# Cuberick-Orion/Candidate-Reranking-CIR

Hardware: AMD Instinct MI355X
Metric: query-candidate triplets scored/sec at K=100 (higher is better)
Workload: dtype f16; 1 GPU; CIRR-val-style K=100 re-rank from pixels (BASELINE configs[2]): ViT-B/16 224px (197 tokens), 32-token captions, 64 queries x (100 candidates + 5 subset members) per step per GPU, skip rate 0, random-init weights; k=100, subset=5, image_size=224, residual_stream=f16

## Files before the change

candidate_reranking_cir_amd/csrc/common.hpp:

```cpp
#pragma once
#include <hip/hip_runtime.h>
#include <stdint.h>

#include "cirrank.h"

namespace cir {

typedef __attribute__((ext_vector_type(8))) __bf16 bf16x8;
typedef __attribute__((ext_vector_type(4))) __bf16 bf16x4;
typedef __attribute__((ext_vector_type(8))) _Float16 f16x8;
typedef __attribute__((ext_vector_type(4))) _Float16 f16x4;
typedef __attribute__((ext_vector_type(4))) float f32x4;
typedef __attribute__((ext_vector_type(16))) float f32x16;
typedef __attribute__((ext_vector_type(4))) short s16x4;
typedef __attribute__((ext_vector_type(8))) short s16x8;
typedef __attribute__((ext_vector_type(4))) unsigned int u32x4;
typedef __attribute__((ext_vector_type(2))) unsigned int u32x2;

constexpr int kWave = 64;

template <typename T> struct Elem;
template <> struct Elem<__bf16> {
    using x8 = bf16x8;
    using x4 = bf16x4;
    static __device__ __forceinline__ f32x4 mfma16(x8 a, x8 b, f32x4 c) {
        return __builtin_amdgcn_mfma_f32_16x16x32_bf16(a, b, c, 0, 0, 0);
    }
    static __device__ __forceinline__ f32x16 mfma32(x8 a, x8 b, f32x16 c) {
        return __builtin_amdgcn_mfma_f32_32x32x16_bf16(a, b, c, 0, 0, 0);
    }
    static __device__ __forceinline__ void mfma16_acc(f32x4& c, x8 a, x8 b) {
        asm("v_mfma_f32_16x16x32_bf16 %0, %1, %2, %0" : "+v"(c) : "v"(a), "v"(b));
    }
};
template <> struct Elem<_Float16> {
    using x8 = f16x8;
    using x4 = f16x4;
    static __device__ __forceinline__ f32x4 mfma16(x8 a, x8 b, f32x4 c) {
        return __builtin_amdgcn_mfma_f32_16x16x32_f16(a, b, c, 0, 0, 0);
    }
    static __device__ __forceinline__ f32x16 mfma32(x8 a, x8 b, f32x16 c) {
        return __builtin_amdgcn_mfma_f32_32x32x16_f16(a, b, c, 0, 0, 0);
    }
    static __device__ __forceinline__ void mfma16_acc(f32x4& c, x8 a, x8 b) {
        asm("v_mfma_f32_16x16x32_f16 %0, %1, %2, %0" : "+v"(c) : "v"(a), "v"(b));
    }
};

template <typename T> __device__ __forceinline__ T from_f32(float x) { return static_cast<T>(x); }
template <typename T> __device__ __forceinline__ float to_f32(T x) { return static_cast<float>(x); }

template <typename T> __device__ __forceinline__ unsigned int pack2(float a, float b) {
    typedef __attribute__((ext_vector_type(2))) T t2;
    t2 v = {static_cast<T>(a), static_cast<T>(b)};
    return __builtin_bit_cast(unsigned int, v);
}

__device__ __forceinline__ float wave_sum(float v) {
#pragma unroll
    for (int o = 32; o > 0; o >>= 1) v += __shfl_xor(v, o, 64);
    return v;
}
__device__ __forceinline__ float wave_max(float v) {
#pragma unroll
    for (int o = 32; o > 0; o >>= 1) v = fmaxf(v, __shfl_xor(v, o, 64));
    return v;
}

__device__ __forceinline__ float fast_erf(float x) {
    const float ax = fabsf(x);
    const float t = __frcp_rn(fmaf(0.3275911f, ax, 1.0f));
    float p = fmaf(1.061405429f, t, -1.453152027f);
    p = fmaf(p, t, 1.421413741f);
    p = fmaf(p, t, -0.284496736f);
    p = fmaf(p, t, 0.254829592f);
    p *= t;
    const float e = 1.0f - p * __expf(-ax * ax);
    return copysignf(e, x);
}
__device__ __forceinline__ float gelu_erf_as(float x) { return 0.5f * x * (1.0f + fast_erf(x * 0.70710678118654752f)); }

__device__ __forceinline__ float gelu_erf(float x) {
    const float xc = __builtin_amdgcn_fmed3f(x, -5.5f, 5.5f);
    const float x2 = xc * xc;
    float p = fmaf(x2, -2.48362952e-05f, -7.36062896e-04f);
    p = fmaf(x2, p, 1.05982735e-01f);
    p = fmaf(x2, p, 2.30164715e+00f);
    const float e = __builtin_amdgcn_exp2f(-(xc * p));
    return x * __builtin_amdgcn_rcpf(1.0f + e);
}

typedef __attribute__((ext_vector_type(2))) float f32x2;
__device__ __forceinline__ f32x2 gelu_erf2(f32x2 x) {
    f32x2 xc;
    xc.x = __builtin_amdgcn_fmed3f(x.x, -5.5f, 5.5f);
    xc.y = __builtin_amdgcn_fmed3f(x.y, -5.5f, 5.5f);
    const f32x2 x2 = xc * xc;
    const f32x2 c3 = {-2.48362952e-05f, -2.48362952e-05f}, c2 = {-7.36062896e-04f, -7.36062896e-04f};
    const f32x2 c1 = {1.05982735e-01f, 1.05982735e-01f}, c0 = {2.30164715e+00f, 2.30164715e+00f};
    f32x2 p = __builtin_elementwise_fma(x2, c3, c2);
    p = __builtin_elementwise_fma(x2, p, c1);
    p = __builtin_elementwise_fma(x2, p, c0);
    const f32x2 q = xc * p;
    f32x2 e;
    e.x = __builtin_amdgcn_exp2f(-q.x);
    e.y = __builtin_amdgcn_exp2f(-q.y);
    const f32x2 d = e + 1.0f;
    f32x2 r;
    r.x = __builtin_amdgcn_rcpf(d.x);
    r.y = __builtin_amdgcn_rcpf(d.y);
    return x * r;
}

__device__ __forceinline__ void gelu_erf8(float (&v)[8]) {
    f32x2 x[4], xc[4], t[4], p[4];
#pragma unroll
    for (int j = 0; j < 4; ++j) x[j] = f32x2{v[2 * j], v[2 * j + 1]};
#pragma unroll
    for (int j = 0; j < 4; ++j) { xc[j].x = __builtin_amdgcn_fmed3f(x[j].x, -5.5f, 5.5f); xc[j].y = __builtin_amdgcn_fmed3f(x[j].y, -5.5f, 5.5f); }
    __builtin_amdgcn_sched_barrier(0);
#pragma unroll
    for (int j = 0; j < 4; ++j) t[j] = xc[j] * xc[j];
    __builtin_amdgcn_sched_barrier(0);
    const f32x2 c3 = {-2.48362952e-05f, -2.48362952e-05f}, c2 = {-7.36062896e-04f, -7.36062896e-04f};
    const f32x2 c1 = {1.05982735e-01f, 1.05982735e-01f}, c0 = {2.30164715e+00f, 2.30164715e+00f};
#pragma unroll
    for (int j = 0; j < 4; ++j) p[j] = __builtin_elementwise_fma(t[j], c3, c2);
    __builtin_amdgcn_sched_barrier(0);
#pragma unroll
    for (int j = 0; j < 4; ++j) p[j] = __builtin_elementwise_fma(t[j], p[j], c1);
    __builtin_amdgcn_sched_barrier(0);
#pragma unroll
    for (int j = 0; j < 4; ++j) p[j] = __builtin_elementwise_fma(t[j], p[j], c0);
    __builtin_amdgcn_sched_barrier(0);
#pragma unroll
    for (int j = 0; j < 4; ++j) t[j] = xc[j] * p[j];
    __builtin_amdgcn_sched_barrier(0);
#pragma unroll
    for (int j = 0; j < 4; ++j) { t[j].x = __builtin_amdgcn_exp2f(-t[j].x); t[j].y = __builtin_amdgcn_exp2f(-t[j].y); }
    __builtin_amdgcn_sched_barrier(0);
#pragma unroll
    for (int j = 0; j < 4; ++j) t[j] = t[j] + 1.0f;
    __builtin_amdgcn_sched_barrier(0);
#pragma unroll
    for (int j = 0; j < 4; ++j) { t[j].x = __builtin_amdgcn_rcpf(t[j].x); t[j].y = __builtin_amdgcn_rcpf(t[j].y); }
    __builtin_amdgcn_sched_barrier(0);
#pragma unroll
    for (int j = 0; j < 4; ++j) { const f32x2 y = x[j] * t[j]; v[2 * j] = y.x; v[2 * j + 1] = y.y; }
}

__device__ __forceinline__ void gelu_erf_as8(float (&v)[8]) {
    f32x2 x[4], t[4], p[4], q[4];
#pragma unroll
    for (int j = 0; j < 4; ++j) x[j] = f32x2{v[2 * j], v[2 * j + 1]};
#pragma unroll
    for (int j = 0; j < 4; ++j) { t[j].x = fmaf(fabsf(x[j].x), 0.3275911f * 0.70710678118654752f, 1.0f); t[j].y = fmaf(fabsf(x[j].y), 0.3275911f * 0.70710678118654752f, 1.0f); }
    __builtin_amdgcn_sched_barrier(0);
#pragma unroll
    for (int j = 0; j < 4; ++j) { t[j].x = __builtin_amdgcn_rcpf(t[j].x); t[j].y = __builtin_amdgcn_rcpf(t[j].y); }
#pragma unroll
    for (int j = 0; j < 4; ++j) q[j] = x[j] * x[j];
    __builtin_amdgcn_sched_barrier(0);
    const f32x2 a5 = {1.061405429f, 1.061405429f}, a4 = {-1.453152027f, -1.453152027f}, a3 = {1.421413741f, 1.421413741f};
    const f32x2 a2 = {-0.284496736f, -0.284496736f}, a1 = {0.254829592f, 0.254829592f};
#pragma unroll
    for (int j = 0; j < 4; ++j) p[j] = __builtin_elementwise_fma(a5, t[j], a4);
#pragma unroll
    for (int j = 0; j < 4; ++j) q[j] = q[j] * f32x2{-0.72134752044448170f, -0.72134752044448170f};
    __builtin_amdgcn_sched_barrier(0);
#pragma unroll
    for (int j = 0; j < 4; ++j) p[j] = __builtin_elementwise_fma(p[j], t[j], a3);
#pragma unroll
    for (int j = 0; j < 4; ++j) { q[j].x = __builtin_amdgcn_exp2f(q[j].x); q[j].y = __builtin_amdgcn_exp2f(q[j].y); }
    __builtin_amdgcn_sched_barrier(0);
#pragma unroll
    for (int j = 0; j < 4; ++j) p[j] = __builtin_elementwise_fma(p[j], t[j], a2);
    __builtin_amdgcn_sched_barrier(0);
#pragma unroll
    for (int j = 0; j < 4; ++j) p[j] = __builtin_elementwise_fma(p[j], t[j], a1);
    __builtin_amdgcn_sched_barrier(0);
#pragma unroll
    for (int j = 0; j < 4; ++j) t[j] = t[j] * q[j];
    __builtin_amdgcn_sched_barrier(0);
#pragma unroll
    for (int j = 0; j < 4; ++j) p[j] = __builtin_elementwise_fma(-p[j], t[j], f32x2{1.0f, 1.0f});
    __builtin_amdgcn_sched_barrier(0);
#pragma unroll
    for (int j = 0; j < 4; ++j) { p[j].x = fmaf(fabsf(x[j].x), p[j].x, x[j].x); p[j].y = fmaf(fabsf(x[j].y), p[j].y, x[j].y); }
    __builtin_amdgcn_sched_barrier(0);
#pragma unroll
    for (int j = 0; j < 4; ++j) { const f32x2 y = p[j] * f32x2{0.5f, 0.5f}; v[2 * j] = y.x; v[2 * j + 1] = y.y; }
}

constexpr float kSplitLoScale = 4096.0f;
constexpr int kSplitLoExp = 12;
__device__ __forceinline__ float clamp_e4m3(float x) { return __builtin_amdgcn_fmed3f(x, -448.0f, 448.0f); }
struct Split4 { unsigned h01, h23, lo8, hi8; };
__device__ __forceinline__ Split4 split8_x4(const float (&y)[4]) {
    float hf[4], lf[4];
    _Float16 hh[4];
#pragma unroll
    for (int j = 0; j < 4; ++j) {
        float v = y[j];
        asm volatile("" : "+v"(v));
        hh[j] = (_Float16)v;
        float f = (float)hh[j];
        asm volatile("" : "+v"(f));
        hf[j] = clamp_e4m3(f);
        lf[j] = clamp_e4m3((v - f) * kSplitLoScale);
    }
    typedef __attribute__((ext_vector_type(2))) _Float16 h2;
    Split4 r;
    r.h01 = __builtin_bit_cast(unsigned, h2{hh[0], hh[1]});
    r.h23 = __builtin_bit_cast(unsigned, h2{hh[2], hh[3]});
    unsigned l = 0, h = 0;
    l = __builtin_amdgcn_cvt_pk_fp8_f32(lf[0], lf[1], l, false);
    l = __builtin_amdgcn_cvt_pk_fp8_f32(lf[2], lf[3], l, true);
    h = __builtin_amdgcn_cvt_pk_fp8_f32(hf[0], hf[1], h, false);
    h = __builtin_amdgcn_cvt_pk_fp8_f32(hf[2], hf[3], h, true);
    r.lo8 = l;
    r.hi8 = h;
    return r;
}
typedef __attribute__((ext_vector_type(8))) int i32x8;
__device__ __forceinline__ void mfma_f8_acc(f32x4& c, i32x8 a, i32x8 b, int sa, int sb) {
    asm("v_mfma_scale_f32_16x16x128_f8f6f4 %0, %1, %2, %0, %3, %4 op_sel_hi:[0,0,0]" : "+v"(c) : "v"(a), "v"(b), "v"(sa), "v"(sb));
}

__device__ __forceinline__ uint32_t hash32(uint32_t x) {
    x ^= x >> 16; x *= 0x7feb352du; x ^= x >> 15; x *= 0x846ca68bu; x ^= x >> 16;
    return x;
}
constexpr uint32_t kDropWeyl = 0x9E3779B9u;
__device__ __forceinline__ uint32_t drop_threshold(float p) { return (uint32_t)(p * 65536.0f + 0.5f); }
__device__ __forceinline__ uint32_t drop_row_key(uint64_t seed, uint64_t row) {
    return (uint32_t)seed + (uint32_t)(seed >> 32) * 0x85EBCA6Bu + (uint32_t)row * kDropWeyl + (uint32_t)(row >> 32) * 0xC2B2AE35u;
}
__device__ __forceinline__ uint32_t drop_bits(uint32_t row_key, uint32_t col) { return hash32(row_key ^ (col >> 1)); }
__device__ __forceinline__ bool drop_kept(uint32_t bits, uint32_t col, uint32_t thr) { return ((col & 1u) ? (bits >> 16) : (bits & 0xffffu)) >= thr; }

__device__ __forceinline__ int xcd_remap(int bid, int nblk) {
    const int q = nblk >> 3, r = nblk & 7, x = bid & 7;
    const int base = (x < r) ? x * (q + 1) : r * (q + 1) + (x - r) * q;
    return base + (bid >> 3);
}

}

namespace cir {
extern int g_tune[3];

constexpr int kOrdRows = 256;
constexpr int kEmbChunk = 512;
struct OrderedDst { float* out[4]; int src[4]; int nout; };
int colsum_ordered_launch(const float* x, int64_t ld, int64_t rows, int seg, const OrderedDst& d, hipStream_t s);
}
#define CIR_CHECK_PTR(p) do { if ((p) == nullptr) return CIR_EINVAL; } while (0)
#define CIR_LAUNCH_RESULT() do { hipError_t e_ = hipGetLastError(); return e_ == hipSuccess ? CIR_OK : (int)e_; } while (0)
static inline bool cir_aligned16(const void* p) { return (reinterpret_cast<uintptr_t>(p) & 15u) == 0; }
```

candidate_reranking_cir_amd/csrc/misc.hip:

```cpp
#include "common.hpp"

namespace cir {

template <typename TI, typename TO>
__global__ __launch_bounds__(256) void patchify_kernel(const TI* img, TO* out, int B, int C, int H, int Wd, int p, int vec) {
    const int gw = Wd / p, gh = H / p;
    const int64_t total = (int64_t)B * gh * gw * C * p;
    const int64_t gid = (int64_t)blockIdx.x * blockDim.x + threadIdx.x;
    if (gid >= total) return;
    int64_t t = gid;
    const int px = (int)(t % gw); t /= gw;
    const int ky = (int)(t % p); t /= p;
    const int py = (int)(t % gh); t /= gh;
    const int c = (int)(t % C);
    const int64_t b = t / C;
    const TI* src = img + ((b * C + c) * H + (py * p + ky)) * (int64_t)Wd + px * p;
    TO* dst = out + ((b * gh + py) * gw + px) * (int64_t)(C * p * p) + (c * p + ky) * p;
    if (vec) {
        if constexpr (sizeof(TO) == 4) {
            const float4* s4 = reinterpret_cast<const float4*>(src);
            float4* d4 = reinterpret_cast<float4*>(dst);
            const float4 a0 = s4[0], a1 = s4[1], a2 = s4[2], a3 = s4[3];
            d4[0] = a0; d4[1] = a1; d4[2] = a2; d4[3] = a3;
        } else if constexpr (sizeof(TI) == 2) {
            const u32x4* s4 = reinterpret_cast<const u32x4*>(src);
            u32x4* d4 = reinterpret_cast<u32x4*>(dst);
            const u32x4 v0 = s4[0], v1 = s4[1];
            d4[0] = v0;
            d4[1] = v1;
        } else {
            const float4* s4 = reinterpret_cast<const float4*>(src);
            const float4 a0 = s4[0], a1 = s4[1], a2 = s4[2], a3 = s4[3];
            u32x4 o0, o1;
            o0.x = pack2<TO>(a0.x, a0.y); o0.y = pack2<TO>(a0.z, a0.w); o0.z = pack2<TO>(a1.x, a1.y); o0.w = pack2<TO>(a1.z, a1.w);
            o1.x = pack2<TO>(a2.x, a2.y); o1.y = pack2<TO>(a2.z, a2.w); o1.z = pack2<TO>(a3.x, a3.y); o1.w = pack2<TO>(a3.z, a3.w);
            u32x4* d4 = reinterpret_cast<u32x4*>(dst);
            d4[0] = o0;
            d4[1] = o1;
        }
        return;
    }
    for (int kx = 0; kx < p; ++kx) dst[kx] = static_cast<TO>(static_cast<float>(src[kx]));
}

template <typename S>
__global__ __launch_bounds__(256) void vit_assemble_kernel(const S* proj, const float* cls, const float* pos, S* x,
                                                           int B, int P, int D) {
    const int d4 = D / 4;
    const int64_t total = (int64_t)B * (P + 1) * d4;
    const int64_t gid = (int64_t)blockIdx.x * blockDim.x + threadIdx.x;
    if (gid >= total) return;
    const int c = (int)(gid % d4);
    const int64_t row = gid / d4;
    const int tok = (int)(row % (P + 1));
    const int64_t b = row / (P + 1);
    const float4 pe = reinterpret_cast<const float4*>(pos + (int64_t)tok * D)[c];
    float4 v;
    if (tok == 0) {
        v = reinterpret_cast<const float4*>(cls)[c];
    } else if constexpr (__is_same(S, float)) {
        v = reinterpret_cast<const float4*>(proj + (b * P + tok - 1) * D)[c];
    } else {
        const f16x4 h = reinterpret_cast<const f16x4*>(proj + (b * P + tok - 1) * D)[c];
        v = make_float4((float)h[0], (float)h[1], (float)h[2], (float)h[3]);
    }
    const float4 o = make_float4(v.x + pe.x, v.y + pe.y, v.z + pe.z, v.w + pe.w);
    if constexpr (__is_same(S, float)) {
        reinterpret_cast<float4*>(x + row * D)[c] = o;
    } else {
        u32x2 pk;
        pk.x = pack2<_Float16>(o.x, o.y);
        pk.y = pack2<_Float16>(o.z, o.w);
        reinterpret_cast<u32x2*>(x + row * D)[c] = pk;
    }
}

template <typename T>
__global__ __launch_bounds__(256) void small_linear_kernel(const T* x, int64_t ldx, const T* W, const float* bias, float* y,
                                                           int64_t M, int N, int K) {
    using X8 = typename Elem<T>::x8;
    const int lane = threadIdx.x & 63;
    const int64_t row = (int64_t)blockIdx.x * 4 + (threadIdx.x >> 6);
    if (row >= M) return;
    float acc[8];
#pragma unroll
    for (int n = 0; n < 8; ++n) acc[n] = 0.f;
    for (int k = lane * 8; k < K; k += 512) {
        const X8 xv = *reinterpret_cast<const X8*>(x + row * ldx + k);
#pragma unroll
        for (int n = 0; n < 8; ++n) {
            if (n < N) {
                const X8 wv = *reinterpret_cast<const X8*>(W + (int64_t)n * K + k);
#pragma unroll
                for (int j = 0; j < 8; ++j) acc[n] = fmaf(static_cast<float>(xv[j]), static_cast<float>(wv[j]), acc[n]);
            }
        }
    }
#pragma unroll
    for (int n = 0; n < 8; ++n) {
        if (n < N) {
            const float s = wave_sum(acc[n]);
            if (lane == 0) y[row * N + n] = s + (bias ? bias[n] : 0.f);
        }
    }
}


template <typename TI, typename TO>
__global__ __launch_bounds__(256) void gather_rows_kernel(const TI* src, const int64_t* index, TO* dst, int64_t n_rows,
                                                          int64_t row_elems, int64_t src_rows) {
    const int64_t vec_per_row = row_elems / 8;
    const int64_t gid = (int64_t)blockIdx.x * blockDim.x + threadIdx.x;
    if (gid >= n_rows * vec_per_row) return;
    const int64_t row = gid / vec_per_row, c = (gid - row * vec_per_row) * 8;
    int64_t sr = index ? index[row] : row;
    sr = sr < 0 ? 0 : (sr >= src_rows ? src_rows - 1 : sr);
    const TI* s = src + sr * row_elems + c;
    TO* d = dst + row * row_elems + c;
    float v[8];
    if constexpr (sizeof(TI) == 4) {
        const float4 a = reinterpret_cast<const float4*>(s)[0], b = reinterpret_cast<const float4*>(s)[1];
        v[0] = a.x; v[1] = a.y; v[2] = a.z; v[3] = a.w; v[4] = b.x; v[5] = b.y; v[6] = b.z; v[7] = b.w;
    } else {
        typedef __attribute__((ext_vector_type(8))) TI ti8;
        const ti8 a = *reinterpret_cast<const ti8*>(s);
#pragma unroll
        for (int j = 0; j < 8; ++j) v[j] = static_cast<float>(a[j]);
    }
    if constexpr (sizeof(TO) == 4) {
        reinterpret_cast<float4*>(d)[0] = make_float4(v[0], v[1], v[2], v[3]);
        reinterpret_cast<float4*>(d)[1] = make_float4(v[4], v[5], v[6], v[7]);
    } else {
        u32x4 o;
        o.x = pack2<TO>(v[0], v[1]); o.y = pack2<TO>(v[2], v[3]); o.z = pack2<TO>(v[4], v[5]); o.w = pack2<TO>(v[6], v[7]);
        *reinterpret_cast<u32x4*>(d) = o;
    }
}


__global__ __launch_bounds__(256) void linear_f32_kernel(const float* x, int64_t ldx, const float* W, const float* bias, float* y,
                                                        int64_t M, int N, int K, int mode) {
    __shared__ float As[16][65], Ws[16][65];
    const int tid = threadIdx.x, tx = tid & 15, ty = tid >> 4;
    const int64_t row0 = (int64_t)blockIdx.y * 64;
    const int col0 = blockIdx.x * 64;
    float acc[4][4];
#pragma unroll
    for (int i = 0; i < 4; ++i)
#pragma unroll
        for (int j = 0; j < 4; ++j) acc[i][j] = 0.f;
    for (int k0 = 0; k0 < K; k0 += 16) {
#pragma unroll
        for (int i = 0; i < 4; ++i) {
            const int e = tid + i * 256, r = e >> 4, kk = e & 15;
            As[kk][r] = (row0 + r < M && k0 + kk < K) ? x[(row0 + r) * ldx + k0 + kk] : 0.f;
            Ws[kk][r] = (col0 + r < N && k0 + kk < K) ? W[(int64_t)(col0 + r) * K + k0 + kk] : 0.f;
        }
        __syncthreads();
#pragma unroll
        for (int kk = 0; kk < 16; ++kk) {
            float av[4], wv[4];
#pragma unroll
            for (int i = 0; i < 4; ++i) { av[i] = As[kk][ty * 4 + i]; wv[i] = Ws[kk][tx * 4 + i]; }
#pragma unroll
            for (int i = 0; i < 4; ++i)
#pragma unroll
                for (int j = 0; j < 4; ++j) acc[i][j] = fmaf(av[i], wv[j], acc[i][j]);
        }
        __syncthreads();
    }
#pragma unroll
    for (int i = 0; i < 4; ++i) {
        const int64_t m = row0 + ty * 4 + i;
        if (m >= M) continue;
#pragma unroll
        for (int j = 0; j < 4; ++j) {
            const int n = col0 + tx * 4 + j;
            if (n >= N) continue;
            const float v = acc[i][j] + (bias ? bias[n] : 0.f);
            y[m * N + n] = mode == 1 ? 1.0f - v : (mode == 2 ? v - 1.0f : v);
        }
    }
}

__global__ __launch_bounds__(256) void l2_normalize_kernel(const float* x, float* y, int64_t rows, int cols) {
    const int lane = threadIdx.x & 63;
    const int64_t row = (int64_t)blockIdx.x * 4 + (threadIdx.x >> 6);
    if (row >= rows) return;
    float s = 0.f;
    for (int c = lane; c < cols; c += 64) { const float v = x[row * cols + c]; s = fmaf(v, v, s); }
    const float inv = 1.0f / fmaxf(sqrtf(wave_sum(s)), 1e-12f);
    for (int c = lane; c < cols; c += 64) y[row * cols + c] = x[row * cols + c] * inv;
}

__global__ __launch_bounds__(256) void topk_desc_kernel(const float* logits, int64_t* idx, int K, int n_pow2) {
    extern __shared__ __attribute__((aligned(16))) char dyn[];
    float* val = reinterpret_cast<float*>(dyn);
    int* ind = reinterpret_cast<int*>(dyn + (size_t)n_pow2 * 4);
    const float* row = logits + (int64_t)blockIdx.x * K;
    for (int i = threadIdx.x; i < n_pow2; i += blockDim.x) {
        float v = i < K ? row[i] : -INFINITY;
        if (v != v) v = -INFINITY;
        val[i] = v;
        ind[i] = i < K ? i : 0x7fffffff;
    }
    __syncthreads();
    for (int size = 2; size <= n_pow2; size <<= 1) {
        for (int stride = size >> 1; stride > 0; stride >>= 1) {
            for (int t = threadIdx.x; t < n_pow2 / 2; t += blockDim.x) {
                const int lo = 2 * t - (t & (stride - 1));
                const int hi = lo + stride;
                const bool asc_block = ((lo & size) != 0);
                const float va = val[lo], vb = val[hi];
                const int ia = ind[lo], ib = ind[hi];
                const bool a_first = (va > vb) || (va == vb && ia < ib);
                const bool swap = asc_block ? a_first : !a_first;
                if (swap) { val[lo] = vb; val[hi] = va; ind[lo] = ib; ind[hi] = ia; }
            }
            __syncthreads();
        }
    }
    for (int i = threadIdx.x; i < K; i += blockDim.x) idx[(int64_t)blockIdx.x * K + i] = ind[i];
}

}

extern "C" int cir_version(void) { return CIR_ABI_VERSION; }

namespace cir { int g_tune[3] = {0, 0, 0}; }

extern "C" int cir_set_tuning(int knob, int value) {
    switch (knob) {
        case CIR_TUNE_GEMM_TILE: if (value != 0 && value != 128 && value != 256) return CIR_EINVAL; break;
        case CIR_TUNE_GEMM_GROUP_W: if (value < 0 || value > 64) return CIR_EINVAL; break;
        case CIR_TUNE_ATTN_SHARED_MAX: if (value != 0 && value != -1 && value != -2 && (value < 32 || value > 608)) return CIR_EINVAL; break;
        default: return CIR_EINVAL;
    }
    cir::g_tune[knob] = value;
    return CIR_OK;
}

extern "C" const char* cir_strerror(int code) {
    switch (code) {
        case CIR_OK: return "ok";
        case CIR_EINVAL: return "invalid argument (null pointer or non-positive extent)";
        case CIR_ESHAPE: return "extent not supported by the gfx950 kernels";
        case CIR_EALIGN: return "pointer or stride not aligned for 16-byte vector access";
        case CIR_EDTYPE: return "dtype code not supported by this entry point";
        default: return code > 0 ? hipGetErrorString((hipError_t)code) : "unknown cirrank error";
    }
}

extern "C" int cir_patchify(const void* image, int img_dtype, void* patches, int dtype16, int B, int C, int H, int Wd,
                            int patch, void* stream) {
    using namespace cir;
    CIR_CHECK_PTR(image); CIR_CHECK_PTR(patches);
    if (B <= 0 || C <= 0 || H <= 0 || Wd <= 0 || patch <= 0) return CIR_EINVAL;
    if (H % patch || Wd % patch) return CIR_ESHAPE;
    if (dtype16 != CIR_BF16 && dtype16 != CIR_F16 && dtype16 != CIR_F32) return CIR_EDTYPE;
    if (img_dtype != CIR_F32 && img_dtype != dtype16) return CIR_EDTYPE;
    const int64_t total = (int64_t)B * C * H * (Wd / patch);
    dim3 grid((unsigned)((total + 255) / 256)), block(256);
    hipStream_t s = reinterpret_cast<hipStream_t>(stream);
    const int vec = patch == 16 && Wd % 16 == 0 && cir_aligned16(image) && cir_aligned16(patches);
    if (dtype16 == CIR_F32) {
        hipLaunchKernelGGL((patchify_kernel<float, float>), grid, block, 0, s, (const float*)image, (float*)patches, B, C, H, Wd, patch, vec);
        CIR_LAUNCH_RESULT();
    }
    if (dtype16 == CIR_BF16) {
        if (img_dtype == CIR_F32) hipLaunchKernelGGL((patchify_kernel<float, __bf16>), grid, block, 0, s, (const float*)image, (__bf16*)patches, B, C, H, Wd, patch, vec);
        else hipLaunchKernelGGL((patchify_kernel<__bf16, __bf16>), grid, block, 0, s, (const __bf16*)image, (__bf16*)patches, B, C, H, Wd, patch, vec);
    } else {
        if (img_dtype == CIR_F32) hipLaunchKernelGGL((patchify_kernel<float, _Float16>), grid, block, 0, s, (const float*)image, (_Float16*)patches, B, C, H, Wd, patch, vec);
        else hipLaunchKernelGGL((patchify_kernel<_Float16, _Float16>), grid, block, 0, s, (const _Float16*)image, (_Float16*)patches, B, C, H, Wd, patch, vec);
    }
    CIR_LAUNCH_RESULT();
}

extern "C" int cir_vit_assemble(const void* proj, const float* cls, const float* pos, void* x, int stream_dtype, int B, int P, int D,
                                void* stream) {
    CIR_CHECK_PTR(proj); CIR_CHECK_PTR(cls); CIR_CHECK_PTR(pos); CIR_CHECK_PTR(x);
    if (B <= 0 || P <= 0 || D <= 0) return CIR_EINVAL;
    if (D % 8) return CIR_ESHAPE;
    if (stream_dtype != CIR_F32 && stream_dtype != CIR_F16) return CIR_EDTYPE;
    if (!cir_aligned16(proj) || !cir_aligned16(cls) || !cir_aligned16(pos) || !cir_aligned16(x)) return CIR_EALIGN;
    const int64_t total = (int64_t)B * (P + 1) * (D / 4);
    dim3 grid((unsigned)((total + 255) / 256)), block(256);
    hipStream_t s = reinterpret_cast<hipStream_t>(stream);
    if (stream_dtype == CIR_F32)
        hipLaunchKernelGGL(cir::vit_assemble_kernel<float>, grid, block, 0, s, reinterpret_cast<const float*>(proj), cls, pos, reinterpret_cast<float*>(x), B, P, D);
    else
        hipLaunchKernelGGL(cir::vit_assemble_kernel<_Float16>, grid, block, 0, s, reinterpret_cast<const _Float16*>(proj), cls, pos, reinterpret_cast<_Float16*>(x), B, P, D);
    CIR_LAUNCH_RESULT();
}

extern "C" int cir_small_linear(const void* x, int64_t ldx, const void* W, const float* bias, float* y, int64_t M, int N,
                                int K, int dtype, void* stream) {
    using namespace cir;
    CIR_CHECK_PTR(x); CIR_CHECK_PTR(W); CIR_CHECK_PTR(y);
    if (M <= 0 || N <= 0 || K <= 0) return CIR_EINVAL;
    if (N > 8 || K % 8) return CIR_ESHAPE;
    if (dtype != CIR_BF16 && dtype != CIR_F16) return CIR_EDTYPE;
    if (!cir_aligned16(x) || !cir_aligned16(W) || ldx % 8) return CIR_EALIGN;
    if ((M + 3) / 4 > 0x7fffffffLL) return CIR_ESHAPE;
    dim3 grid((unsigned)((M + 3) / 4)), block(256);
    hipStream_t s = reinterpret_cast<hipStream_t>(stream);
    if (dtype == CIR_BF16) hipLaunchKernelGGL((small_linear_kernel<__bf16>), grid, block, 0, s, (const __bf16*)x, ldx, (const __bf16*)W, bias, y, M, N, K);
    else hipLaunchKernelGGL((small_linear_kernel<_Float16>), grid, block, 0, s, (const _Float16*)x, ldx, (const _Float16*)W, bias, y, M, N, K);
    CIR_LAUNCH_RESULT();
}

extern "C" int cir_topk_desc(const float* logits, int64_t* idx, int Q, int K, void* stream) {
    CIR_CHECK_PTR(logits); CIR_CHECK_PTR(idx);
    if (Q <= 0 || K <= 0) return CIR_EINVAL;
    if (K > 8192) return CIR_ESHAPE;
    int n = 2;
    while (n < K) n <<= 1;
    dim3 grid((unsigned)Q), block(256);
    hipLaunchKernelGGL(cir::topk_desc_kernel, grid, block, (size_t)n * 8, reinterpret_cast<hipStream_t>(stream), logits, idx, K, n);
    CIR_LAUNCH_RESULT();
}

namespace cir {
template <typename TI, typename TO>
static void launch_gather(const void* src, const int64_t* index, void* dst, int64_t n_rows, int64_t row_elems, int64_t src_rows, hipStream_t s) {
    const int64_t total = n_rows * (row_elems / 8);
    dim3 grid((unsigned)((total + 255) / 256)), block(256);
    hipLaunchKernelGGL((gather_rows_kernel<TI, TO>), grid, block, 0, s, (const TI*)src, index, (TO*)dst, n_rows, row_elems, src_rows);
}
}

extern "C" int cir_gather_rows(const void* src, int src_dtype, const int64_t* index, void* dst, int dst_dtype, int64_t n_rows,
                               int64_t row_elems, int64_t src_rows, void* stream) {
    using namespace cir;
    CIR_CHECK_PTR(src); CIR_CHECK_PTR(dst);
    if (n_rows <= 0 || row_elems <= 0 || src_rows <= 0) return CIR_EINVAL;
    if (row_elems % 8) return CIR_ESHAPE;
    if (!cir_aligned16(src) || !cir_aligned16(dst)) return CIR_EALIGN;
    if (n_rows * (row_elems / 8) > 0x7fffffffLL * 256) return CIR_ESHAPE;
    hipStream_t s = reinterpret_cast<hipStream_t>(stream);
#define CIR_G(SD, DD, TI, TO) if (src_dtype == SD && dst_dtype == DD) { launch_gather<TI, TO>(src, index, dst, n_rows, row_elems, src_rows, s); CIR_LAUNCH_RESULT(); }
    CIR_G(CIR_F32, CIR_F32, float, float)
    CIR_G(CIR_F32, CIR_BF16, float, __bf16)
    CIR_G(CIR_F32, CIR_F16, float, _Float16)
    CIR_G(CIR_BF16, CIR_BF16, __bf16, __bf16)
    CIR_G(CIR_F16, CIR_F16, _Float16, _Float16)
    CIR_G(CIR_BF16, CIR_F32, __bf16, float)
    CIR_G(CIR_F16, CIR_F32, _Float16, float)
    CIR_G(CIR_BF16, CIR_F16, __bf16, _Float16)
    CIR_G(CIR_F16, CIR_BF16, _Float16, __bf16)
#undef CIR_G
    return CIR_EDTYPE;
}

namespace cir {
template <int ACT>
__global__ __launch_bounds__(256) void split16_kernel(const float* __restrict__ x, int64_t ldx, _Float16* __restrict__ hi, _Float16* __restrict__ lo,
                                                      _Float16* __restrict__ hi2, int64_t ldo, int64_t rows, int cols) {
    const int64_t per_row = cols >> 3;
    const int64_t i = (int64_t)blockIdx.x * 256 + threadIdx.x;
    if (i >= rows * per_row) return;
    const int64_t r = i / per_row;
    const int c = (int)(i - r * per_row) * 8;
    const float4 v0 = *reinterpret_cast<const float4*>(x + r * ldx + c), v1 = *reinterpret_cast<const float4*>(x + r * ldx + c + 4);
    float v[8] = {v0.x, v0.y, v0.z, v0.w, v1.x, v1.y, v1.z, v1.w};
    f16x8 h, l;
#pragma unroll
    for (int j = 0; j < 8; ++j) {
        float y = v[j];
        if (ACT == CIR_ACT_GELU) y = 0.5f * y * (1.0f + erff(y * 0.70710678118654752f));
        else if (ACT == CIR_ACT_RELU) y = fmaxf(y, 0.f);
        asm volatile("" : "+v"(y));
        const _Float16 hj = (_Float16)y;
        float hf = (float)hj;
        asm volatile("" : "+v"(hf));
        h[j] = hj;
        l[j] = (_Float16)(y - hf);
    }
    *reinterpret_cast<f16x8*>(hi + r * ldo + c) = h;
    *reinterpret_cast<f16x8*>(lo + r * ldo + c) = l;
    if (hi2 != nullptr) *reinterpret_cast<f16x8*>(hi2 + r * ldo + c) = h;
}
template <int ACT>
__global__ __launch_bounds__(256) void split8_kernel(const float* __restrict__ x, int64_t ldx, char* __restrict__ out, int64_t ldo, int64_t rows, int cols) {
    const int64_t per_row = cols >> 3;
    const int64_t i = (int64_t)blockIdx.x * 256 + threadIdx.x;
    if (i >= rows * per_row) return;
    const int64_t r = i / per_row;
    const int c = (int)(i - r * per_row) * 8;
    const float4 v0 = *reinterpret_cast<const float4*>(x + r * ldx + c), v1 = *reinterpret_cast<const float4*>(x + r * ldx + c + 4);
    float v[8] = {v0.x, v0.y, v0.z, v0.w, v1.x, v1.y, v1.z, v1.w};
    if (ACT == CIR_ACT_GELU) gelu_erf_as8(v);
    else if (ACT == CIR_ACT_RELU) {
#pragma unroll
        for (int j = 0; j < 8; ++j) v[j] = fmaxf(v[j], 0.f);
    }
    const float a[4] = {v[0], v[1], v[2], v[3]}, b[4] = {v[4], v[5], v[6], v[7]};
    const Split4 sa = split8_x4(a), sb = split8_x4(b);
    const u32x4 h = {sa.h01, sa.h23, sb.h01, sb.h23};
    const u32x2 l8 = {sa.lo8, sb.lo8}, h8 = {sa.hi8, sb.hi8};
    char* row = out + r * ldo;
    *reinterpret_cast<u32x4*>(row + 2 * c) = h;
    *reinterpret_cast<u32x2*>(row + 2 * cols + c) = l8;
    *reinterpret_cast<u32x2*>(row + 3 * cols + c) = h8;
}
}


extern "C" int cir_split16(const float* x, int64_t ldx, void* hi, void* lo, void* hi2, int64_t ldo, int64_t rows, int cols, int act, void* stream) {
    using namespace cir;
    CIR_CHECK_PTR(x); CIR_CHECK_PTR(hi); CIR_CHECK_PTR(lo);
    if (rows <= 0 || cols <= 0) return CIR_EINVAL;
    if (cols % 8 || ldx % 4 || ldo % 8 || ldo < cols) return CIR_ESHAPE;
    if (act < CIR_ACT_NONE || act > CIR_ACT_RELU) return CIR_EINVAL;
    if (!cir_aligned16(x) || !cir_aligned16(hi) || !cir_aligned16(lo) || (hi2 && !cir_aligned16(hi2))) return CIR_EALIGN;
    const int64_t n = rows * (cols / 8);
    if (n > 0x7fffffffLL * 256) return CIR_ESHAPE;
    dim3 grid((unsigned)((n + 255) / 256)), block(256);
    hipStream_t s = reinterpret_cast<hipStream_t>(stream);
    _Float16* h = reinterpret_cast<_Float16*>(hi);
    _Float16* l = reinterpret_cast<_Float16*>(lo);
    _Float16* h2 = reinterpret_cast<_Float16*>(hi2);
    if (act == CIR_ACT_GELU) hipLaunchKernelGGL((split16_kernel<CIR_ACT_GELU>), grid, block, 0, s, x, ldx, h, l, h2, ldo, rows, cols);
    else if (act == CIR_ACT_RELU) hipLaunchKernelGGL((split16_kernel<CIR_ACT_RELU>), grid, block, 0, s, x, ldx, h, l, h2, ldo, rows, cols);
    else hipLaunchKernelGGL((split16_kernel<CIR_ACT_NONE>), grid, block, 0, s, x, ldx, h, l, h2, ldo, rows, cols);
    CIR_LAUNCH_RESULT();
}

extern "C" int cir_split8(const float* x, int64_t ldx, void* out, int64_t ldo_bytes, int64_t rows, int cols, int act, void* stream) {
    using namespace cir;
    CIR_CHECK_PTR(x); CIR_CHECK_PTR(out);
    if (rows <= 0 || cols <= 0) return CIR_EINVAL;
    if (cols % 8 || ldx % 4 || ldo_bytes % 16 || ldo_bytes < 4 * (int64_t)cols) return CIR_ESHAPE;
    if (act < CIR_ACT_NONE || act > CIR_ACT_RELU) return CIR_EINVAL;
    if (!cir_aligned16(x) || !cir_aligned16(out) || cols % 16) return CIR_EALIGN;
    const int64_t n = rows * (cols / 8);
    if (n > 0x7fffffffLL * 256) return CIR_ESHAPE;
    dim3 grid((unsigned)((n + 255) / 256)), block(256);
    hipStream_t s = reinterpret_cast<hipStream_t>(stream);
    char* o = reinterpret_cast<char*>(out);
    if (act == CIR_ACT_GELU) hipLaunchKernelGGL((split8_kernel<CIR_ACT_GELU>), grid, block, 0, s, x, ldx, o, ldo_bytes, rows, cols);
    else if (act == CIR_ACT_RELU) hipLaunchKernelGGL((split8_kernel<CIR_ACT_RELU>), grid, block, 0, s, x, ldx, o, ldo_bytes, rows, cols);
    else hipLaunchKernelGGL((split8_kernel<CIR_ACT_NONE>), grid, block, 0, s, x, ldx, o, ldo_bytes, rows, cols);
    CIR_LAUNCH_RESULT();
}

extern "C" int cir_linear_f32(const float* x, int64_t ldx, const float* W, const float* bias, float* y, int64_t M, int N, int K,
                              int mode, void* stream) {
    CIR_CHECK_PTR(x); CIR_CHECK_PTR(W); CIR_CHECK_PTR(y);
    if (M <= 0 || N <= 0 || K <= 0) return CIR_EINVAL;
    if (mode < 0 || mode > 2) return CIR_EINVAL;
    dim3 grid((unsigned)((N + 63) / 64), (unsigned)((M + 63) / 64)), block(256);
    if (grid.y > 65535u) return CIR_ESHAPE;
    hipLaunchKernelGGL(cir::linear_f32_kernel, grid, block, 0, reinterpret_cast<hipStream_t>(stream), x, ldx, W, bias, y, M, N, K, mode);
    CIR_LAUNCH_RESULT();
}

extern "C" int cir_l2_normalize(const float* x, float* y, int64_t rows, int cols, void* stream) {
    CIR_CHECK_PTR(x); CIR_CHECK_PTR(y);
    if (rows <= 0 || cols <= 0) return CIR_EINVAL;
    if ((rows + 3) / 4 > 0x7fffffffLL) return CIR_ESHAPE;
    dim3 grid((unsigned)((rows + 3) / 4)), block(256);
    hipLaunchKernelGGL(cir::l2_normalize_kernel, grid, block, 0, reinterpret_cast<hipStream_t>(stream), x, y, rows, cols);
    CIR_LAUNCH_RESULT();
}
```

candidate_reranking_cir_amd/csrc/xattn_fold.hip:

```cpp

#include "xattn_fold.hpp"

#ifndef FOLD_DBG
#define FOLD_DBG 0
#endif

namespace cir {

#if FOLD_DBG & 8
__device__ unsigned long long g_fold_stamps[8 * 64];
#define FOLD_STAMP(K)                                                                                          \
    do { if (blockIdx.x < 4 && (wave & 3) == 0 && lane == 0 && (K) < 64) {                                      \
             unsigned long long t_; __builtin_amdgcn_sched_barrier(0);                                         \
             asm volatile("s_memtime %0\n\ts_waitcnt lgkmcnt(0)" : "=s"(t_) :: "memory");                       \
             __builtin_amdgcn_sched_barrier(0);                                                                 \
             g_fold_stamps[(blockIdx.x * 2 + (wave >> 2)) * 64 + (K)] = t_; } } while (0)
#else
#define FOLD_STAMP(K) do {} while (0)
#endif

template <typename T, bool MASKED = false>
__global__ __launch_bounds__(512, 2) void xattn_fold_kernel(const FoldArgs a) {
    using X8 = typename Elem<T>::x8;
    extern __shared__ __attribute__((aligned(16))) char smem[];

    const int tid = threadIdx.x;
    const int lane = tid & 63;
    const int wave = __builtin_amdgcn_readfirstlane(tid >> 6);
    const int l16 = lane & 15, g = lane >> 4;
    const int b = (blockIdx.x >> 2) & 1;
    const int t = (blockIdx.x >> 3) * 4 + (blockIdx.x & 3);
    if (t >= a.T) return;

    const T* X = reinterpret_cast<const T*>(a.x) + (int64_t)t * a.x_s1;
    const T* Wk = reinterpret_cast<const T*>(a.wkt) + (int64_t)b * a.w_sb;
    const T* Wv = reinterpret_cast<const T*>(a.wvp) + (int64_t)b * a.w_sb;

    const int pair = wave >> 1, odd = wave & 1;
    const int hA = 3 * pair + 2 * odd, hC = 3 * pair + 1;
    int hq[3], tok[3];
    hq[0] = hA; hq[1] = hA; hq[2] = hC;
    tok[0] = l16; tok[1] = 16 + l16; tok[2] = 16 * odd + l16;
    char* const qs = smem + 2 * kFoldBuf;
    {
        const T* qb_ = reinterpret_cast<const T*>(a.q) + (int64_t)b * a.q_sb + (int64_t)t * a.L * a.q_rs;
#pragma unroll
        for (int i = 0; i < 6; ++i) {
            const int c = tid + i * 512;
            const int row = c / 96, ch = c - row * 96;
            X8 v;
#pragma unroll
            for (int j = 0; j < 8; ++j) v[j] = static_cast<T>(0.f);
            if (row < a.L) v = *reinterpret_cast<const X8*>(qb_ + (int64_t)row * a.q_rs + ch * 8);
            *reinterpret_cast<X8*>(qs + row * kStrideQ + ch * 16) = v;
        }
    }
    int qoff[3];
#pragma unroll
    for (int qb = 0; qb < 3; ++qb) qoff[qb] = tok[qb] * kStrideQ + (hq[qb] * 64 + 8 * g) * 2;

    int xoff1[4];
#pragma unroll
    for (int j = 0; j < 4; ++j) {
        const int s = (wave * 4 + j) * 64 + lane;
        const int row = s >> 3, c = (s & 7) ^ (row & 7);
        xoff1[j] = (min(row, a.N - 1) * kFoldD + c * 8) * 2;
    }
    const __amdgpu_buffer_rsrc_t rs_x = __builtin_amdgcn_make_buffer_rsrc(const_cast<T*>(X), 0, a.N * kFoldD * 2, 0x00020000);
    auto stage1 = [&](int chunk, int buf) {
        char* base = smem + buf * kFoldBuf + wave * 4 * 1024;
#pragma unroll
        for (int j = 0; j < 4; ++j) FOLD_DMA(rs_x, xoff1[j], chunk * 128, base + j * 1024);
    };

    f32x4 S[kFoldKB][3];
#pragma unroll
    for (int kb = 0; kb < kFoldKB; ++kb)
#pragma unroll
        for (int qb = 0; qb < 3; ++qb) S[kb][qb] = f32x4{0.f, 0.f, 0.f, 0.f};

    X8 w[2][2][2];
    const int wlane = lane * 16;
    const __amdgpu_buffer_rsrc_t rs_k = __builtin_amdgcn_make_buffer_rsrc(const_cast<T*>(Wk), 0, kFoldD * kFoldD * 2, 0x00020000);
    const __amdgpu_buffer_rsrc_t rs_v = __builtin_amdgcn_make_buffer_rsrc(const_cast<T*>(Wv), 0, kFoldD * kFoldD * 2, 0x00020000);
    auto load_wk = [&](int unit) {
#pragma unroll
        for (int fbh = 0; fbh < 2; ++fbh) {
#pragma unroll
            for (int ks = 0; ks < 2; ++ks) {
                w[fbh][ks][0] = wload<X8>(rs_k, wlane, (((unit * 2 + fbh) * 12 + hA) * 2 + ks) * 1024);
                w[fbh][ks][1] = wload<X8>(rs_k, wlane, (((unit * 2 + fbh) * 12 + hC) * 2 + ks) * 1024);
            }
        }
    };
    FOLD_STAMP(0);
    stage1(0, 0);
    load_wk(0);
    for (int kc = 0; kc < kFoldChunks; ++kc) {
        if (kc < 4) FOLD_STAMP(1 + 6 * kc);
        asm volatile("s_waitcnt vmcnt(0)" ::: "memory");
        if (kc < 4) FOLD_STAMP(2 + 6 * kc);
        if (!(FOLD_DBG & 4) || kc == 0) __syncthreads();
        if (kc < 4) FOLD_STAMP(3 + 6 * kc);
        const char* xs = smem + (kc & 1) * kFoldBuf;
#pragma unroll
        for (int half = 0; half < 2; ++half) {
            f32x4 a1[2][3];
#pragma unroll
            for (int fbh = 0; fbh < 2; ++fbh)
#pragma unroll
                for (int qb = 0; qb < 3; ++qb) a1[fbh][qb] = f32x4{0.f, 0.f, 0.f, 0.f};
#pragma unroll
            for (int ks = 0; ks < 2; ++ks) {
                X8 qf[3];
#pragma unroll
                for (int qb = 0; qb < 3; ++qb) qf[qb] = *reinterpret_cast<const X8*>(qs + qoff[qb] + 64 * ks);
#pragma unroll
                for (int fbh = 0; fbh < 2; ++fbh) {
                    a1[fbh][0] = Elem<T>::mfma16(w[fbh][ks][0], qf[0], a1[fbh][0]);
                    a1[fbh][1] = Elem<T>::mfma16(w[fbh][ks][0], qf[1], a1[fbh][1]);
                    a1[fbh][2] = Elem<T>::mfma16(w[fbh][ks][1], qf[2], a1[fbh][2]);
                }
            }
            X8 bq[3];
#pragma unroll
            for (int qb = 0; qb < 3; ++qb) bq[qb] = pack_acc2<T>(a1[0][qb], a1[1][qb]);
            if (kc < 4 && half == 0) FOLD_STAMP(4 + 6 * kc);
            __builtin_amdgcn_sched_barrier(0);
            const int nu = 2 * kc + half + 1;
            const bool more_w = nu < 2 * kFoldChunks && !(FOLD_DBG & 1), more_x = half == 0 && kc + 1 < kFoldChunks && !(FOLD_DBG & 4);
            auto mem_op = [&](int j) {
                if (j < 8) {
                    if (more_w) {
                        const int fbh = j >> 2, ks = (j >> 1) & 1, hc = j & 1;
                        w[fbh][ks][hc] = wload<X8>(rs_k, wlane, (((nu * 2 + fbh) * 12 + (hc ? hC : hA)) * 2 + ks) * 1024);
                    }
                } else if (j < 12) {
                    if (more_x) FOLD_DMA(rs_x, xoff1[j - 8], (kc + 1) * 128, smem + ((kc + 1) & 1) * kFoldBuf + (wave * 4 + j - 8) * 1024);
                }
            };
            const char* xr = xs + l16 * 128 + (((4 * half + g) ^ (l16 & 7)) << 4);
            auto rd = [&](int kb) { return *reinterpret_cast<const X8*>(xr + kb * 16 * 128); };
            X8 xa[3];
            xa[0] = rd(0);
            xa[1] = rd(1);
#pragma unroll
            for (int kb = 0; kb < kFoldKB; ++kb) {
                if (kb + 2 < kFoldKB && !(FOLD_DBG & 2)) xa[(kb + 2) % 3] = rd(kb + 2);
                mem_op(kb);
                __builtin_amdgcn_sched_barrier(0);
#pragma unroll
                for (int qb = 0; qb < 3; ++qb) S[kb][qb] = Elem<T>::mfma16(xa[kb % 3], bq[qb], S[kb][qb]);
                __builtin_amdgcn_sched_barrier(0);
            }
            if (kc < 4) FOLD_STAMP(5 + 6 * kc + half);
        }
    }
    FOLD_STAMP(25);

    const float sl = a.scale * 1.4426950408889634f;
    float rinv[3];
    X8 P[7][3];
#pragma unroll
    for (int qb = 0; qb < 3; ++qb) {
        float m = -INFINITY;
#pragma unroll
        for (int kb = 0; kb < kFoldKB; ++kb)
#pragma unroll
            for (int r = 0; r < 4; ++r) {
                const int key = 16 * kb + 4 * g + r;
                float v = key < a.N ? S[kb][qb][r] : -INFINITY;
                if constexpr (MASKED) {
                    const float mk = a.mask[(int64_t)t * a.m_st + min(key, a.N - 1)];
                    v = key < a.N ? fmaf(fmaxf(mk, -2.0e38f), 1.4426950408889634f, S[kb][qb][r] * sl) : -INFINITY;
                }
                S[kb][qb][r] = v;
                m = fmaxf(m, v);
            }
        m = fmaxf(m, __shfl_xor(m, 16, 64));
        m = fmaxf(m, __shfl_xor(m, 32, 64));
        const float ms = MASKED ? m : m * sl;
        float sum = 0.f;
#pragma unroll
        for (int kb = 0; kb < kFoldKB; ++kb)
#pragma unroll
            for (int r = 0; r < 4; ++r) {
                const float p = MASKED ? __builtin_amdgcn_exp2f(S[kb][qb][r] - ms) : __builtin_amdgcn_exp2f(fmaf(S[kb][qb][r], sl, -ms));
                S[kb][qb][r] = p;
                sum += p;
            }
        sum += __shfl_xor(sum, 16, 64);
        sum += __shfl_xor(sum, 32, 64);
        rinv[qb] = 1.0f / sum;
#pragma unroll
        for (int p = 0; p < 7; ++p) P[p][qb] = pack_acc2<T>(S[2 * p][qb], S[2 * p + 1][qb]);
    }

    f32x4 c4[4][3];
#pragma unroll
    for (int db = 0; db < 4; ++db)
#pragma unroll
        for (int qb = 0; qb < 3; ++qb) c4[db][qb] = f32x4{0.f, 0.f, 0.f, 0.f};
    X8 wv[4][2];
    int xoff2[5];
#pragma unroll
    for (int j = 0; j < 5; ++j) {
        const int s = (wave * 5 + j) * 64 + lane;
        const int row = min(s / 10, a.N - 1), c = min(s % 10, 7);
        xoff2[j] = (row * kFoldD + c * 8) * 2;
    }
    auto stage2 = [&](int chunk, int buf) {
        char* base = smem + buf * kFoldBuf + wave * 5 * 1024;
#pragma unroll
        for (int j = 0; j < 5; ++j) FOLD_DMA(rs_x, xoff2[j], chunk * 128, base + j * 1024);
    };
    FOLD_STAMP(26);
    __syncthreads();
    stage2(0, 0);
    const int troff = (4 * g + (l16 >> 2)) * kStride2 + (4 * (l16 & 3)) * 2;
    for (int nc = 0; nc < kFoldChunks; ++nc) {
        if (nc < 4) FOLD_STAMP(27 + 6 * nc);
        asm volatile("s_waitcnt vmcnt(0)" ::: "memory");
        if (nc < 4) FOLD_STAMP(28 + 6 * nc);
        if (!(FOLD_DBG & 4) || nc == 0) __syncthreads();
        if (nc < 4) FOLD_STAMP(29 + 6 * nc);
        const char* xs = smem + (nc & 1) * kFoldBuf + troff;
#pragma unroll
        for (int half = 0; half < 2; ++half) {
            f32x4 a3[2][3];
#pragma unroll
            for (int fbh = 0; fbh < 2; ++fbh)
#pragma unroll
                for (int qb = 0; qb < 3; ++qb) a3[fbh][qb] = f32x4{0.f, 0.f, 0.f, 0.f};
            const int cu = 2 * nc + half;
            const bool more_x = half == 0 && nc + 1 < kFoldChunks && !(FOLD_DBG & 4);
            auto mem_op = [&](int j) {
                if (j < 8) {
                    if (!(FOLD_DBG & 1) || cu == 0) {
                        const int db = j >> 1, hc = j & 1;
                        wv[db][hc] = wload<X8>(rs_v, wlane, ((cu * 4 + db) * 12 + (hc ? hC : hA)) * 1024);
                    }
                } else if (j < 13) {
                    if (more_x) FOLD_DMA(rs_x, xoff2[j - 8], (nc + 1) * 128, smem + ((nc + 1) & 1) * kFoldBuf + (wave * 5 + j - 8) * 1024);
                }
            };
            const unsigned xaddr = (unsigned)(size_t)(lptr_t)(xs) + (32 * half) * 2;
            u32x2 lo[3], hi[3];
#define FOLD_TR(SLOT, I)                                                                                                        \
            asm volatile("ds_read_b64_tr_b16 %0, %2 offset:%3\n\tds_read_b64_tr_b16 %1, %2 offset:%4"                             \
                         : "=&v"(lo[SLOT]), "=&v"(hi[SLOT]) : "v"(xaddr), "n"((32 * ((I) >> 1)) * kStride2 + (16 * ((I) & 1)) * 2),  \
                           "n"((32 * ((I) >> 1) + 16) * kStride2 + (16 * ((I) & 1)) * 2) : "memory")
            FOLD_TR(0, 0);
            FOLD_TR(1, 1);
#pragma unroll
            for (int i = 0; i < 14; ++i) {
                if (i + 2 < 14 && !(FOLD_DBG & 2)) {
                    switch (i + 2) {
                        case 2: FOLD_TR(2, 2); break; case 3: FOLD_TR(0, 3); break; case 4: FOLD_TR(1, 4); break; case 5: FOLD_TR(2, 5); break;
                        case 6: FOLD_TR(0, 6); break; case 7: FOLD_TR(1, 7); break; case 8: FOLD_TR(2, 8); break; case 9: FOLD_TR(0, 9); break;
                        case 10: FOLD_TR(1, 10); break; case 11: FOLD_TR(2, 11); break; case 12: FOLD_TR(0, 12); break; default: FOLD_TR(1, 13); break;
                    }
                }
                mem_op(i);
                if (FOLD_DBG & 2) asm volatile("s_waitcnt lgkmcnt(0)" : "+v"(lo[i % 3]), "+v"(hi[i % 3]));
                else if (i + 2 < 14) asm volatile("s_waitcnt lgkmcnt(4)" : "+v"(lo[i % 3]), "+v"(hi[i % 3]));
                else if (i + 1 < 14) asm volatile("s_waitcnt lgkmcnt(2)" : "+v"(lo[i % 3]), "+v"(hi[i % 3]));
                else asm volatile("s_waitcnt lgkmcnt(0)" : "+v"(lo[i % 3]), "+v"(hi[i % 3]));
                __builtin_amdgcn_sched_barrier(0);
                const u32x4 both = {lo[i % 3].x, lo[i % 3].y, hi[i % 3].x, hi[i % 3].y};
                const X8 xa = __builtin_bit_cast(X8, both);
#pragma unroll
                for (int qb = 0; qb < 3; ++qb) a3[i & 1][qb] = Elem<T>::mfma16(xa, P[i >> 1][qb], a3[i & 1][qb]);
                __builtin_amdgcn_sched_barrier(0);
            }
#undef FOLD_TR
            if (nc < 4 && half == 0) FOLD_STAMP(30 + 6 * nc);
            X8 bq[3];
#pragma unroll
            for (int qb = 0; qb < 3; ++qb) bq[qb] = pack_acc2<T>(a3[0][qb], a3[1][qb]);
#pragma unroll
            for (int db = 0; db < 4; ++db) {
                c4[db][0] = Elem<T>::mfma16(wv[db][0], bq[0], c4[db][0]);
                c4[db][1] = Elem<T>::mfma16(wv[db][0], bq[1], c4[db][1]);
                c4[db][2] = Elem<T>::mfma16(wv[db][1], bq[2], c4[db][2]);
            }
            __builtin_amdgcn_sched_barrier(0);
            if (nc < 4) FOLD_STAMP(31 + 6 * nc + half);
        }
    }

    FOLD_STAMP(51);
    T* ob = reinterpret_cast<T*>(a.out) + (int64_t)t * a.o_st + (int64_t)b * a.o_sb;
    const float* bvb = a.bv + b * kFoldD;
#pragma unroll
    for (int qb = 0; qb < 3; ++qb) {
        if (tok[qb] >= a.L) continue;
        T* orow = ob + (int64_t)tok[qb] * a.o_sr + hq[qb] * 64 + 4 * g;
        const float* brow = bvb + hq[qb] * 64 + 4 * g;
#pragma unroll
        for (int db = 0; db < 4; ++db) {
            const float4 b4 = *reinterpret_cast<const float4*>(brow + 16 * db);
            u32x2 o;
            o.x = pack2<T>(fmaf(c4[db][qb][0], rinv[qb], b4.x), fmaf(c4[db][qb][1], rinv[qb], b4.y));
            o.y = pack2<T>(fmaf(c4[db][qb][2], rinv[qb], b4.z), fmaf(c4[db][qb][3], rinv[qb], b4.w));
            *reinterpret_cast<u32x2*>(orow + 16 * db) = o;
        }
    }
}

}

extern "C" int cir_cross_attention_folded(const void* q, int64_t q_sb, int64_t q_rs, const void* x, int64_t x_s1, const void* wkt, const void* wvp,
                                          int64_t w_sb, const float* bv, const float* key_mask, int64_t mask_stride, void* out, int64_t o_st, int64_t o_sr,
                                          int64_t o_sb, int T, int L, int N, int D, int H, float scale, int dtype, void* stream) {
    using namespace cir;
    FoldArgs a;
    const int rc = fold_args(a, q, q_sb, q_rs, x, x_s1, wkt, wvp, w_sb, bv, key_mask, mask_stride, out, o_st, o_sr, o_sb, T, L, N, D, H, scale, dtype,
                             32, 608, (int64_t)T * 2);
    if (rc != CIR_OK) return rc;
    hipStream_t s = reinterpret_cast<hipStream_t>(stream);
    if (N > 16 * kFoldKB) return launch_fold16(a, dtype, s);
    const FoldKernel k = dtype == CIR_BF16 ? (key_mask ? xattn_fold_kernel<__bf16, true> : xattn_fold_kernel<__bf16, false>)
                                           : (key_mask ? xattn_fold_kernel<_Float16, true> : xattn_fold_kernel<_Float16, false>);
    return fold_launch(k, dim3((unsigned)(8 * ((T + 3) / 4))), dim3(512), 2 * kFoldBuf + 32 * kStrideQ, s, a);
}

#if FOLD_DBG & 8
extern "C" int cir_debug_fold_stamps(unsigned long long* host) {
    return (int)hipMemcpyFromSymbol(host, HIP_SYMBOL(cir::g_fold_stamps), sizeof(unsigned long long) * 8 * 64);
}
#endif
```

candidate_reranking_cir_amd/csrc/xattn_fold.hpp:

```cpp
#pragma once
#include "common.hpp"
#include "gemm_args.hpp"

namespace cir {

struct FoldArgs {
    const void* q; int64_t q_sb, q_rs;
    const void* x; int64_t x_s1;
    const void* wkt; const void* wvp; int64_t w_sb;
    const float* bv;
    void* out; int64_t o_st, o_sr, o_sb;
    int T, L, N;
    float scale;
    const float* mask = nullptr; int64_t m_st = 0;
};

typedef __attribute__((address_space(3))) s16x4* lds_s16x4_ptr_f;
constexpr int kFoldD = 768, kFoldChunks = 12, kFoldKB = 14;
constexpr int kFoldBuf = 2560 * 16;
constexpr int kStride2 = 160;
constexpr int kStrideQ = 1568;

#define FOLD_DMA(RS, VOFF, SOFF, LDS_DST) __builtin_amdgcn_raw_ptr_buffer_load_lds(RS, (lptr_t)(LDS_DST), 16, VOFF, SOFF, 0, 0)

template <typename X8>
__device__ __forceinline__ X8 wload(__amdgpu_buffer_rsrc_t rs, int voff, int soff) {
    return __builtin_bit_cast(X8, __builtin_amdgcn_raw_buffer_load_b128(rs, voff, soff, 0));
}

template <typename T>
__device__ __forceinline__ typename Elem<T>::x8 pack_acc2(const f32x4& lo, const f32x4& hi) {
    typename Elem<T>::x8 r;
#pragma unroll
    for (int j = 0; j < 4; ++j) { r[j] = static_cast<T>(lo[j]); r[4 + j] = static_cast<T>(hi[j]); }
    return r;
}


inline int fold_args(FoldArgs& a, const void* q, int64_t q_sb, int64_t q_rs, const void* x, int64_t x_s1, const void* wkt, const void* wvp, int64_t w_sb,
                     const float* bv, const float* key_mask, int64_t mask_stride, void* out, int64_t o_st, int64_t o_sr, int64_t o_sb, int T, int L, int N,
                     int D, int H, float scale, int dtype, int max_l, int max_n, int64_t grid_bound, int min_l = 1, int min_n = 1) {
    CIR_CHECK_PTR(q); CIR_CHECK_PTR(x); CIR_CHECK_PTR(wkt); CIR_CHECK_PTR(wvp); CIR_CHECK_PTR(bv); CIR_CHECK_PTR(out);
    if (T <= 0 || L <= 0 || N <= 0) return CIR_EINVAL;
    if (D != kFoldD || H != 12 || L > max_l || N > max_n || L < min_l || N < min_n) return CIR_ESHAPE;
    if (dtype != CIR_BF16 && dtype != CIR_F16) return CIR_EDTYPE;
    if (!cir_aligned16(q) || !cir_aligned16(x) || !cir_aligned16(wkt) || !cir_aligned16(wvp) || !cir_aligned16(bv) || (reinterpret_cast<uintptr_t>(out) & 7) ||
        q_sb % 8 || q_rs % 8 || x_s1 % 8 || w_sb % 8 || o_st % 4 || o_sr % 4 || o_sb % 4)
        return CIR_EALIGN;
    if (grid_bound > 0x7fffffff) return CIR_ESHAPE;
    if (key_mask && mask_stride < N) return CIR_ESHAPE;
    a.q = q; a.q_sb = q_sb; a.q_rs = q_rs; a.x = x; a.x_s1 = x_s1; a.wkt = wkt; a.wvp = wvp; a.w_sb = w_sb; a.bv = bv;
    a.out = out; a.o_st = o_st; a.o_sr = o_sr; a.o_sb = o_sb; a.T = T; a.L = L; a.N = N; a.scale = scale;
    a.mask = key_mask; a.m_st = mask_stride;
    return CIR_OK;
}

using FoldKernel = void (*)(const FoldArgs);
inline int fold_launch(FoldKernel kernel, dim3 grid, dim3 block, size_t lds, hipStream_t s, const FoldArgs& a) {
    const hipError_t e = hipFuncSetAttribute(reinterpret_cast<const void*>(kernel), hipFuncAttributeMaxDynamicSharedMemorySize, (int)lds);
    if (e != hipSuccess) return (int)e;
    hipLaunchKernelGGL(kernel, grid, block, lds, s, a);
    CIR_LAUNCH_RESULT();
}

int launch_fold16(const FoldArgs& a, int dtype, hipStream_t s);

}
```

candidate_reranking_cir_amd/engine.py:

```python
from __future__ import annotations

import warnings
import weakref
from typing import Dict, NamedTuple, Optional, Tuple

import torch

from . import ops
from .config import BertGeometry, VitGeometry

SD = Dict[str, torch.Tensor]

LN_FOLD_DEFAULT = 1


def _w16(t: torch.Tensor, dtype, device) -> torch.Tensor:
    return t.detach().to(device=device, dtype=torch.float32).to(dtype).contiguous()


def _f32(t: torch.Tensor, device) -> torch.Tensor:
    return t.detach().to(device=device, dtype=torch.float32).contiguous()


def _mark_split(mode: int, layers, *extra):
    mark = ops.split_weight8 if mode == 8 else ops.split_weight
    for ly in layers:
        for k, v in ly.items():
            if k.startswith("w") and torch.is_tensor(v) and v.dtype == torch.float32 and v.dim() >= 2:
                mark(v)
    for w in extra:
        mark(w)


def _split_mode(split3, dtype, geo=None) -> int:
    if dtype != torch.float32 or not split3:
        return 0
    if split3 == 8 and geo is not None and (geo.hidden_size % 256 or geo.intermediate_size % 256):
        return 3
    return 8 if split3 == 8 else 3


def _auto_stream(dtype: torch.dtype, stream_dtype: Optional[torch.dtype]) -> torch.dtype:
    return stream_dtype if stream_dtype is not None else torch.float16


def _ln(x, gamma, beta, eps, dt, sdt, residual=None, need_stream=True, split8=False):
    if split8:
        return ops.layernorm_split8(x, gamma, beta, eps, residual=residual)
    if (dt == sdt and need_stream) or dt == torch.float32:
        y, _ = ops.layernorm(x, gamma, beta, eps, residual=residual, want32=True, dtype16=None, stream_dtype=sdt)
        return y, y
    return ops.layernorm(x, gamma, beta, eps, residual=residual, want32=need_stream, dtype16=dt, stream_dtype=sdt)


def _attend(q, k, v, scale, mask, dt, split8, lead):
    if split8:
        return ops.attention_split8(q, k, v, scale, mask).view(*lead)
    ctx = torch.empty(q.shape, dtype=dt, device=q.device)
    ops.attention(q, k, v, ctx, scale, mask)
    return ctx.view(*lead, q.shape[-1])


def additive_self_mask(attention_mask: torch.Tensor) -> torch.Tensor:
    return ((1.0 - attention_mask.to(torch.float32)) * -10000.0).contiguous()


def additive_encoder_mask(attention_mask: torch.Tensor) -> torch.Tensor:
    return ((1.0 - attention_mask.to(torch.float32)) * torch.finfo(torch.float32).min).contiguous()


class VitEngine:

    def __init__(self, sd: SD, geo: VitGeometry, dtype: torch.dtype, device, prefix: str = "visual_encoder.",
                 stream_dtype: Optional[torch.dtype] = None):
        geo.validate()
        self.geo, self.dtype, self.device, self.stream_dtype = geo, dtype, device, _auto_stream(dtype, stream_dtype)
        d = geo.width
        p = prefix
        self.w_patch = _w16(sd[p + "patch_embed.proj.weight"].reshape(d, -1), dtype, device)
        self.b_patch = _f32(sd[p + "patch_embed.proj.bias"], device)
        self.cls = _f32(sd[p + "cls_token"].reshape(d), device)
        self.pos = _f32(sd[p + "pos_embed"].reshape(-1, d), device)
        self.blocks = []
        for i in range(geo.depth):
            b = f"{p}blocks.{i}."
            self.blocks.append(dict(
                g1=_f32(sd[b + "norm1.weight"], device), b1=_f32(sd[b + "norm1.bias"], device),
                wqkv=_w16(sd[b + "attn.qkv.weight"], dtype, device), bqkv=_f32(sd[b + "attn.qkv.bias"], device),
                wo=_w16(sd[b + "attn.proj.weight"], dtype, device), bo=_f32(sd[b + "attn.proj.bias"], device),
                g2=_f32(sd[b + "norm2.weight"], device), b2=_f32(sd[b + "norm2.bias"], device),
                w1=_w16(sd[b + "mlp.fc1.weight"], dtype, device), c1=_f32(sd[b + "mlp.fc1.bias"], device),
                w2=_w16(sd[b + "mlp.fc2.weight"], dtype, device), c2=_f32(sd[b + "mlp.fc2.bias"], device)))
        self.gf, self.bf = _f32(sd[p + "norm.weight"], device), _f32(sd[p + "norm.bias"], device)
        self.ln_fold = 0
        if dtype == torch.float16 and self.stream_dtype == torch.float16 and d % 128 == 0:
            self.ln_fold = LN_FOLD_DEFAULT
            for i, blk in enumerate(self.blocks):
                b = f"{p}blocks.{i}."
                blk["qkv_f"] = ops.ln_fold_pack(sd[b + "attn.qkv.weight"].to(device), sd[b + "attn.qkv.bias"].to(device), blk["g1"], blk["b1"])
                if self.ln_fold >= 2:
                    blk["fc1_f"] = ops.ln_fold_pack(sd[b + "mlp.fc1.weight"].to(device), sd[b + "mlp.fc1.bias"].to(device), blk["g2"], blk["b2"])

    def forward(self, image: torch.Tensor, want32: bool = False, chunk: int = 4096, out32: Optional[torch.Tensor] = None,
                out16: Optional[torch.Tensor] = None):
        geo, dt = self.geo, self.dtype
        bsz, d, n = image.shape[0], geo.width, geo.num_tokens
        if bsz > chunk:
            n_parts = -(-bsz // chunk)
            size = -(-bsz // n_parts)
            y16 = torch.empty((bsz, n, d), dtype=dt, device=image.device) if out16 is None else out16
            if dt == torch.float32 and want32 and out32 is None:
                y32 = y16
            else:
                y32 = (torch.empty((bsz, n, d), dtype=torch.float32, device=image.device) if out32 is None else out32) if want32 else None
            for i in range(0, bsz, size):
                self.forward(image[i:i + size], want32, chunk, out32=None if y32 is None else y32[i:i + size], out16=y16[i:i + size])
            return y32, y16
        if image.shape[-1] != geo.image_size or image.shape[-2] != geo.image_size:
            raise ValueError(f"image size {tuple(image.shape[-2:])} != model image_size {geo.image_size}")
        if image.dtype not in (torch.float32, dt):
            image = image.float()
        scale = 64 ** -0.5
        sdt = self.stream_dtype
        patches = ops.patchify(image, geo.patch_size, dt)
        proj = ops.gemm(patches, self.w_patch, self.b_patch, out_dtype=sdt)
        x = ops.vit_assemble(proj, self.cls, self.pos, bsz).view(bsz * n, d)
        ctx = torch.empty((bsz, n, d), dtype=dt, device=x.device)
        for blk in self.blocks:
            if self.ln_fold >= 1:
                qkv = ops.gemm_ln(x, *blk["qkv_f"], geo.layer_norm_eps).view(bsz, n, 3, d)
            else:
                _, xb = _ln(x, blk["g1"], blk["b1"], geo.layer_norm_eps, dt, sdt, need_stream=False)
                qkv = ops.gemm(xb, blk["wqkv"], blk["bqkv"]).view(bsz, n, 3, d)
            ops.attention(qkv[:, :, 0].unsqueeze(1), qkv[:, :, 1].unsqueeze(1), qkv[:, :, 2].unsqueeze(1),
                          ctx.unsqueeze(1), scale)
            ops.gemm(ctx.view(bsz * n, d), blk["wo"], blk["bo"], residual=x, out_dtype=sdt, out=x)
            if self.ln_fold >= 2 and "fc1_f" in blk:
                f = ops.gemm_ln(x, *blk["fc1_f"], geo.layer_norm_eps, act=ops.ACT_GELU)
            else:
                _, xb = _ln(x, blk["g2"], blk["b2"], geo.layer_norm_eps, dt, sdt, need_stream=False)
                f = ops.gemm(xb, blk["w1"], blk["c1"], act=ops.ACT_GELU)
            ops.gemm(f, blk["w2"], blk["c2"], residual=x, out_dtype=sdt, out=x)
        if dt == torch.float32:
            o = out16 if out16 is not None else out32
            y32, _ = ops.layernorm(x, self.gf, self.bf, geo.layer_norm_eps, want32=True, dtype16=None, stream_dtype=torch.float32,
                                   out32=None if o is None else o.view(bsz * n, d))
            if out16 is not None and out32 is not None and out32.data_ptr() != out16.data_ptr():
                out32.copy_(out16)
            return (y32.view(bsz, n, d) if want32 else None), y32.view(bsz, n, d)
        y32, y16 = ops.layernorm(x, self.gf, self.bf, geo.layer_norm_eps, want32=want32, dtype16=dt, stream_dtype=torch.float32,
                                 out32=None if (out32 is None or not want32) else out32.view(bsz * n, d),
                                 out16=None if out16 is None else out16.view(bsz * n, d))
        return (y32.view(bsz, n, d) if want32 else None), y16.view(bsz, n, d)


    @torch.no_grad()
    def forward_drop_path(self, image: torch.Tensor, scales: torch.Tensor) -> torch.Tensor:
        from . import train_ops as T
        geo, dt = self.geo, self.dtype
        if dt == torch.float32:
            raise RuntimeError("DropPath embeds run on 16-bit operands: leave the exact mode for training")
        bsz, d, n = image.shape[0], geo.width, geo.num_tokens
        assert tuple(scales.shape) == (geo.depth, 2, bsz) and scales.dtype == torch.float32
        if image.dtype not in (torch.float32, dt):
            image = image.float()
        f32 = torch.float32
        patches = ops.patchify(image.contiguous(), geo.patch_size, dt)
        x = ops.vit_assemble(ops.gemm(patches, self.w_patch, self.b_patch, out_dtype=f32), self.cls, self.pos, bsz).view(bsz * n, d)
        ctx = torch.empty((bsz, n, d), dtype=dt, device=x.device)
        for i, blk in enumerate(self.blocks):
            _, xb = ops.layernorm(x, blk["g1"], blk["b1"], geo.layer_norm_eps, want32=False, dtype16=dt, stream_dtype=f32)
            qkv = ops.gemm(xb, blk["wqkv"], blk["bqkv"]).view(bsz, n, 3, d)
            ops.attention(qkv[:, :, 0].unsqueeze(1), qkv[:, :, 1].unsqueeze(1), qkv[:, :, 2].unsqueeze(1), ctx.unsqueeze(1), 64 ** -0.5)
            x = T.rows_scale_add(x, ops.gemm(ctx.view(bsz * n, d), blk["wo"], blk["bo"], out_dtype=f32), scales[i, 0].contiguous(), n)
            _, xb = ops.layernorm(x, blk["g2"], blk["b2"], geo.layer_norm_eps, want32=False, dtype16=dt, stream_dtype=f32)
            f = ops.gemm(xb, blk["w1"], blk["c1"], act=ops.ACT_GELU)
            x = T.rows_scale_add(x, ops.gemm(f, blk["w2"], blk["c2"], out_dtype=f32), scales[i, 1].contiguous(), n)
        y32, _ = ops.layernorm(x, self.gf, self.bf, geo.layer_norm_eps, want32=True, dtype16=None, stream_dtype=f32)
        return y32.view(bsz, n, d)


class KVBank(list):
    tokens: Optional[torch.Tensor] = None
    engine = None


def _cat(sd: SD, keys, suffix: str) -> torch.Tensor:
    return torch.cat([sd[k + suffix].detach().float() for k in keys], dim=0)


class MedEngine:

    def __init__(self, sd: SD, geo: BertGeometry, dtype: torch.dtype, device, prefix: str = "text_encoder.",
                 stream_dtype: Optional[torch.dtype] = None, cross_dtype: Optional[torch.dtype] = None, split3: bool = False):
        geo.validate()
        self.geo, self.dtype, self.device, self.stream_dtype = geo, dtype, device, _auto_stream(dtype, stream_dtype)
        self.split = _split_mode(split3, dtype, geo)
        self.split3 = self.split != 0
        self.xdtype = xdt = cross_dtype or dtype
        e = prefix + "embeddings."
        self.word, self.posemb = _f32(sd[e + "word_embeddings.weight"], device), _f32(sd[e + "position_embeddings.weight"], device)
        self.ge, self.be = _f32(sd[e + "LayerNorm.weight"], device), _f32(sd[e + "LayerNorm.bias"], device)
        self.layers = []
        for i in range(geo.num_hidden_layers):
            p = f"{prefix}encoder.layer.{i}."
            sa, ca = p + "attention.self.", p + "crossattention.self."
            self.layers.append(dict(
                wqkv=_w16(_cat(sd, [sa + "query", sa + "key", sa + "value"], ".weight"), dtype, device),
                bqkv=_f32(_cat(sd, [sa + "query", sa + "key", sa + "value"], ".bias"), device),
                wo=_w16(sd[p + "attention.output.dense.weight"], dtype, device), bo=_f32(sd[p + "attention.output.dense.bias"], device),
                g1=_f32(sd[p + "attention.output.LayerNorm.weight"], device), b1=_f32(sd[p + "attention.output.LayerNorm.bias"], device),
                wq=_w16(sd[ca + "query.weight"], xdt, device), bq=_f32(sd[ca + "query.bias"], device),
                wkv=_w16(_cat(sd, [ca + "key", ca + "value"], ".weight"), xdt, device),
                bkv=_f32(_cat(sd, [ca + "key", ca + "value"], ".bias"), device),
                wco=_w16(sd[p + "crossattention.output.dense.weight"], xdt, device), bco=_f32(sd[p + "crossattention.output.dense.bias"], device),
                g2=_f32(sd[p + "crossattention.output.LayerNorm.weight"], device), b2=_f32(sd[p + "crossattention.output.LayerNorm.bias"], device),
                w1=_w16(sd[p + "intermediate.dense.weight"], dtype, device), c1=_f32(sd[p + "intermediate.dense.bias"], device),
                w2=_w16(sd[p + "output.dense.weight"], dtype, device), c2=_f32(sd[p + "output.dense.bias"], device),
                g3=_f32(sd[p + "output.LayerNorm.weight"], device), b3=_f32(sd[p + "output.LayerNorm.bias"], device)))
        if self.split:
            _mark_split(self.split, self.layers)

    def forward(self, input_ids: torch.Tensor, attention_mask: torch.Tensor, enc16: torch.Tensor,
                enc_mask: Optional[torch.Tensor] = None):
        geo, dt, sdt, xdt = self.geo, self.dtype, self.stream_dtype, self.xdtype
        q_n, l = input_ids.shape
        d, n = geo.hidden_size, enc16.shape[1]
        r = q_n * l
        eps, scale = geo.layer_norm_eps, 64 ** -0.5
        hs, h16 = ops.embed_layernorm(input_ids, self.word, self.posemb, self.ge, self.be, eps, dt, stream_dtype=sdt)
        hs, h16 = hs.view(r, d), h16.view(r, d)
        smask = additive_self_mask(attention_mask).view(q_n, 1, l)
        emask = additive_encoder_mask(enc_mask).view(q_n, 1, n) if enc_mask is not None else None
        enc2 = enc16.reshape(q_n * n, enc16.shape[2])
        s8 = self.split == 8
        ctx_x = torch.empty((q_n, 1, l, d), dtype=xdt, device=hs.device)
        for ly in self.layers:
            qkv = ops.gemm(h16, ly["wqkv"], ly["bqkv"]).view(q_n, 1, l, 3 * d)
            ctx_op = _attend(qkv[..., :d], qkv[..., d:2 * d], qkv[..., 2 * d:], scale, smask, dt, s8, (r,))
            t = ops.gemm(ctx_op, ly["wo"], ly["bo"], residual=hs, out_dtype=sdt)
            a_s, a16 = _ln(t, ly["g1"], ly["b1"], eps, xdt, sdt)
            qc = ops.gemm(a16, ly["wq"], ly["bq"]).view(q_n, 1, l, d)
            kv = ops.gemm(enc2, ly["wkv"], ly["bkv"]).view(q_n, 1, n, 2 * d)
            ops.attention(qc, kv[..., :d], kv[..., d:], ctx_x, scale, emask)
            t = ops.gemm(ctx_x.view(r, d), ly["wco"], ly["bco"], residual=a_s, out_dtype=sdt)
            c_s, c16 = _ln(t, ly["g2"], ly["b2"], eps, dt, sdt, split8=s8)
            f = ops.gemm(c16, ly["w1"], ly["c1"], act=ops.ACT_GELU)
            t = ops.gemm(f, ly["w2"], ly["c2"], residual=c_s, out_dtype=sdt)
            hs, h16 = _ln(t, ly["g3"], ly["b3"], eps, dt, sdt, split8=s8)
        if s8:
            h16 = hs
        h32 = hs if hs.dtype == torch.float32 else ops.gather_rows(hs, None, torch.float32)
        return h32.view(q_n, l, d), h16.view(q_n, l, d)


class LayerPlan(NamedTuple):
    cls_only: bool
    cross: str
    sdt: torch.dtype
    sdt_out: torch.dtype


class Plan(NamedTuple):
    layers: Tuple[LayerPlan, ...]
    kv_chunk: int
    fallback: bool


SCALE = 64 ** -0.5


class NlvrEngine:

    def __init__(self, sd: SD, geo: BertGeometry, dtype: torch.dtype, device, prefix: str = "text_encoder.", fold_merge: bool = True,
                 stream_dtype: Optional[torch.dtype] = None, cross_dtype: Optional[torch.dtype] = None, split3: bool = False):
        geo.validate()
        self.geo, self.dtype, self.device, self.fold_merge, self.stream_dtype = geo, dtype, device, fold_merge, _auto_stream(dtype, stream_dtype)
        self.split = _split_mode(split3, dtype, geo)
        self.split3 = self.split != 0
        self.xdtype = xdt = cross_dtype or dtype
        self.trim_last = True
        self.kv_chunk = 0
        self.fold_cls_kv = xdt != torch.float32
        self.fold_cross_kv = xdt != torch.float32 and geo.hidden_size == 768 and geo.encoder_width == 768 and geo.num_attention_heads == 12
        self.fold_fallbacks = 0
        self.fold_long = False
        self.fold_short = False
        self.fold_long_wide = False
        self.stream32_from = None
        self._graphs = {}
        e = prefix + "embeddings."
        self.word, self.posemb = _f32(sd[e + "word_embeddings.weight"], device), _f32(sd[e + "position_embeddings.weight"], device)
        self.ge, self.be = _f32(sd[e + "LayerNorm.weight"], device), _f32(sd[e + "LayerNorm.bias"], device)
        d = geo.hidden_size
        self.layers = []
        for i in range(geo.num_hidden_layers):
            p = f"{prefix}encoder.layer.{i}."
            ly = {}
            sa = [p + f"attention.self{b}." for b in (0, 1)]
            ca = [p + f"crossattention.self{b}." for b in (0, 1)]
            ly["wqkv"] = _w16(torch.stack([_cat(sd, [s + "query", s + "key", s + "value"], ".weight") for s in sa]), dtype, device)
            ly["bqkv"] = _f32(torch.stack([_cat(sd, [s + "query", s + "key", s + "value"], ".bias") for s in sa]), device)
            ly["wo"] = _w16(torch.stack([sd[p + f"attention.output.dense{b}.weight"].float() for b in (0, 1)]), dtype, device)
            ly["bo"] = _f32(torch.stack([sd[p + f"attention.output.dense{b}.bias"].float() for b in (0, 1)]), device)
            ly["g1"] = _f32(torch.stack([sd[p + f"attention.output.LayerNorm{c}.weight"] for c in "AB"]), device)
            ly["b1"] = _f32(torch.stack([sd[p + f"attention.output.LayerNorm{c}.bias"] for c in "AB"]), device)
            ly["wq"] = _w16(torch.stack([sd[c + "query.weight"].float() for c in ca]), xdt, device)
            ly["bq"] = _f32(torch.stack([sd[c + "query.bias"].float() for c in ca]), device)
            kv_keys = [ca[0] + "key", ca[0] + "value", ca[1] + "key", ca[1] + "value"]
            ly["wkv"] = _w16(_cat(sd, kv_keys, ".weight"), xdt, device)
            ly["bkv"] = _f32(_cat(sd, kv_keys, ".bias"), device)
            if self.fold_cross_kv:
                ly["wkt"] = ops.fold_pack_key(_w16(torch.stack([sd[c + "key.weight"].detach().float() for c in ca]), xdt, device))
                ly["wvp"] = ops.fold_pack_value(_w16(torch.stack([sd[c + "value.weight"].detach().float() for c in ca]), xdt, device))
                ly["bvf"] = _f32(torch.stack([sd[c + "value.bias"].detach().float() for c in ca]), device)
            w0 = sd[p + "crossattention.output.dense0.weight"].detach().cpu().double()
            w1 = sd[p + "crossattention.output.dense1.weight"].detach().cpu().double()
            c0 = sd[p + "crossattention.output.dense0.bias"].detach().cpu().double()
            c1 = sd[p + "crossattention.output.dense1.bias"].detach().cpu().double()
            mk = p + "crossattention.output.merge_layer"
            if mk + ".weight" in sd:
                wm, bm = sd[mk + ".weight"].detach().cpu().double(), sd[mk + ".bias"].detach().cpu().double()
                if fold_merge:
                    ly["wm"] = _w16(torch.cat([wm[:, :d] @ w0, wm[:, d:] @ w1], dim=1).float(), xdt, device)
                    ly["bm"] = _f32((wm[:, :d] @ c0 + wm[:, d:] @ c1 + bm).float(), device)
                else:
                    ly["wd"] = _w16(torch.stack([w0, w1]).float(), xdt, device)
                    ly["bd"] = _f32(torch.stack([c0, c1]).float(), device)
                    ly["wm"] = _w16(wm.float(), xdt, device)
                    ly["bm"] = _f32(bm.float(), device)
            else:
                ly["wm"] = _w16(torch.cat([0.5 * w0, 0.5 * w1], dim=1).float(), xdt, device)
                ly["bm"] = _f32((0.5 * (c0 + c1)).float(), device)
            ly["g2"] = _f32(torch.stack([sd[p + f"crossattention.output.LayerNorm{c}.weight"] for c in "AB"]), device)
            ly["b2"] = _f32(torch.stack([sd[p + f"crossattention.output.LayerNorm{c}.bias"] for c in "AB"]), device)
            ly["w1"] = _w16(sd[p + "intermediate.dense.weight"], dtype, device)
            ly["c1"] = _f32(sd[p + "intermediate.dense.bias"], device)
            ly["w2"] = _w16(sd[p + "output.dense.weight"], dtype, device)
            ly["c2"] = _f32(sd[p + "output.dense.bias"], device)
            ly["g3"] = _f32(sd[p + "output.LayerNorm.weight"], device)
            ly["b3"] = _f32(sd[p + "output.LayerNorm.bias"], device)
            self.layers.append(ly)
        h_n, dv = geo.num_attention_heads, geo.encoder_width
        self.cls_fold = None
        if geo.num_hidden_layers > 1 and 2 * h_n <= 32 and dv % 128 == 0 and dv <= 768 and d == h_n * 64:
            p = f"{prefix}encoder.layer.{geo.num_hidden_layers - 1}.crossattention."
            wk = [sd[p + f"self{b}.key.weight"].detach().float() for b in (0, 1)]
            wv = [sd[p + f"self{b}.value.weight"].detach().float() for b in (0, 1)]
            bv = [sd[p + f"self{b}.value.bias"].detach().float() for b in (0, 1)]
            self.cls_fold = dict(
                wkt=[_w16(w.view(h_n, 64, dv).transpose(1, 2).contiguous(), xdt, device) for w in wk],
                wv=_w16(torch.cat(wv).view(2 * h_n, 64, dv), xdt, device),
                bv=_f32(torch.cat(bv).view(2 * h_n, 64), device), qp={})
        self.wc0, self.bc0 = _w16(sd["cls_head.0.weight"], dtype, device), _f32(sd["cls_head.0.bias"], device)
        self.wc2, self.bc2 = _w16(sd["cls_head.2.weight"], dtype, device), _f32(sd["cls_head.2.bias"], device)
        if self.split:
            _mark_split(self.split, self.layers, self.wc0)

    def plan(self, l: int, n: int, dv: int, masked: bool, bank: Optional[Tuple[bool, ...]] = None) -> Plan:
        d, dt, s32, last = self.geo.hidden_size, self.dtype, self.stream32_from, len(self.layers) - 1
        sd = lambda i: torch.float32 if (s32 is not None and i >= s32 and dt != torch.float32) else self.stream_dtype
        layers = []
        for i, ly in enumerate(self.layers):
            cls_only = self.trim_last and i == last and i > 0
            no_kv = bank is not None and bank[i]
            foldable = bank is None and self.fold_cross_kv and "wkt" in ly and not cls_only and dv == d
            if cls_only and not masked and self.cls_fold is not None and self.fold_cls_kv and (bank is None or no_kv):
                cross = "cls_fold"
            elif no_kv:
                raise ValueError("this K/V bank was built with the last layer folded (no K|V of that layer): rebuild it with fold_cls_kv = False")
            elif foldable and self.fold_short and l <= 16 and n <= 608:
                cross = "fold_short"
            elif foldable and l <= 32 and n <= 608:
                cross = "fold32"
            elif foldable and self.fold_long and 33 <= l <= 64 and n <= 224:
                cross = "fold_long"
            elif foldable and self.fold_long_wide and 33 <= l <= 64 and 225 <= n <= 608:
                cross = "fold_long_wide"
            else:
                cross = "projected" if bank is None else "bank"
            layers.append(LayerPlan(cls_only, cross, sd(i), sd(i + 1)))
        fallback = last >= 1 and layers[1].cross == "projected" and self.fold_cross_kv and "wkt" in self.layers[1] and l > 32
        return Plan(tuple(layers), self.kv_chunk, fallback)

    def graph_key(self, ids_shape, cand_shape, cand_dtype) -> tuple:
        return (tuple(ids_shape), tuple(cand_shape), cand_dtype, self.plan(ids_shape[1], cand_shape[1], cand_shape[2], False))

    @torch.no_grad()
    def build_kv_bank(self, bank16: torch.Tensor, chunk: int = 512) -> list:
        n_idx, n, dv = bank16.shape
        d = self.geo.hidden_size
        out = KVBank()
        out.tokens = bank16
        out.engine = weakref.ref(self)
        last = len(self.layers) - 1
        for i, ly in enumerate(self.layers):
            if i == last and self.trim_last and last > 0 and self.cls_fold is not None and self.fold_cls_kv:
                out.append(None)
                continue
            kv = torch.empty((n_idx, n, 4 * d), dtype=self.xdtype, device=bank16.device)
            for i0 in range(0, n_idx, chunk):
                rows = bank16[i0:i0 + chunk].reshape(-1, dv)
                ops.gemm(rows, ly["wkv"], ly["bkv"], out=kv[i0:i0 + chunk].view(-1, 4 * d))
            out.append(kv)
        return out

    def forward_graphed(self, input_ids, attention_mask, z_t32, cand16, qidx) -> torch.Tensor:
        if ops.PROFILE_GEMM is not None or ops.PROFILE_ATTN is not None:
            return self.forward(input_ids, attention_mask, z_t32, cand16, qidx)
        graphs = self._graphs
        z_t32 = z_t32.float().contiguous()
        key = self.graph_key(input_ids.shape, cand16.shape, cand16.dtype)
        g = graphs.pop(key, None)
        if g is None:
            if len(graphs) >= 8:
                graphs.pop(next(iter(graphs)))
            g = ScoreGraph(self, input_ids.contiguous(), attention_mask.contiguous(), z_t32, cand16.contiguous(), qidx.contiguous())
        graphs[key] = g
        return g(input_ids, attention_mask, z_t32, cand16, qidx)

    def _self_block(self, ly, h32, h16, items, l, smask, sdt, lq=None):
        d, eps, lq = self.geo.hidden_size, self.geo.layer_norm_eps, lq or l
        qkv = ops.gemm(h16, ly["wqkv"], ly["bqkv"]).view(2, items, l, 3 * d)
        ctx_op = _attend(qkv[:, :, :lq, :d], qkv[..., d:2 * d], qkv[..., 2 * d:], SCALE, smask.unsqueeze(0).expand(2, items, l), self.dtype,
                         self.split == 8, (2, items * lq))
        t = ops.gemm(ctx_op, ly["wo"], ly["bo"], residual=h32 if lq == l else h32.view(2, items, l, d)[:, :, 0, :], out_dtype=sdt)
        return _ln(t, ly["g1"], ly["b1"], eps, self.xdtype, sdt)

    def _query_block(self, input_ids, attention_mask, z_t32, qidx, t_n, sdt):
        geo, dt, xdt = self.geo, self.dtype, self.xdtype
        (q_n, l), d = input_ids.shape, geo.hidden_size
        emb32, _ = ops.embed_layernorm(input_ids, self.word, self.posemb, self.ge, self.be, geo.layer_norm_eps, dt)
        if tuple(z_t32.shape) != tuple(emb32.shape):
            raise AssertionError("left and right inputs shall be the same shape")
        hq32 = torch.stack([z_t32.reshape(q_n * l, d).float(), emb32.view(q_n * l, d)])
        hq_s = hq32 if sdt == torch.float32 else ops.gather_rows(hq32.view(2 * q_n * l, d), None, sdt).view(2, q_n * l, d)
        hq16 = hq_s if dt == sdt else ops.gather_rows(hq32.view(2 * q_n * l, d), None, dt).view(2, q_n * l, d)
        smask_q = additive_self_mask(attention_mask)
        a_sq, a16q = self._self_block(self.layers[0], hq_s, hq16, q_n, l, smask_q, sdt)
        both = torch.cat([qidx, qidx + q_n])
        a32 = ops.gather_rows(a_sq.view(2 * q_n, l * d), both, sdt).view(2, t_n * l, d)
        a16 = a32 if xdt == sdt else ops.gather_rows(a16q.view(2 * q_n, l * d), both, xdt).view(2, t_n * l, d)
        return a32, a16, ops.gather_rows(_pad8(smask_q), qidx, torch.float32)[:, :l]

    def _cross_block(self, ly, lp: LayerPlan, a16, cc, tok, emask2d, rows, kv, kv_chunk):
        d, (t_n, l), n = self.geo.hidden_size, cc.shape[:2], tok.shape[1]
        qraw = ops.gemm(a16, ly["wq"], ly["bq"])
        qc = qraw.view(2, t_n, -1, d).permute(1, 0, 2, 3)
        ccl = cc if not lp.cls_only else torch.empty((t_n, 1, 2, d), dtype=self.xdtype, device=cc.device)
        emask = None if emask2d is None else emask2d.view(t_n, 1, n).expand(t_n, 2, n)
        if lp.cross == "cls_fold":
            self._cross_cls_fold(qc, ccl, tok, rows)
        elif lp.cross in ("fold_short", "fold32", "fold_long", "fold_long_wide"):
            fold = getattr(ops, {"fold_short": "cross_attention_folded_short", "fold32": "cross_attention_folded", "fold_long": "cross_attention_folded_long",
                                 "fold_long_wide": "cross_attention_folded_long_wide"}[lp.cross])
            fold(qraw, tok, ly["wkt"], ly["wvp"], ly["bvf"], ccl, l, SCALE, heads=self.geo.num_attention_heads, mask=emask2d)
        elif lp.cross == "projected":
            self._cross_projected(ly, qc, ccl, tok, emask, kv_chunk)
        else:
            kv = kv.view(-1, n, 4, d)
            ops.attention(qc, kv[:, :, 0::2].permute(0, 2, 1, 3), kv[:, :, 1::2].permute(0, 2, 1, 3), ccl.permute(0, 2, 1, 3), SCALE, emask,
                          kv_index=rows)
        return ccl

    def _cross_cls_fold(self, qc, ccl, tok, rows):
        f, h_n, t_n, dv = self.cls_fold, self.geo.num_attention_heads, ccl.shape[0], tok.shape[2]
        qp = f["qp"].get(t_n)
        if qp is None:
            qp = f["qp"][t_n] = torch.zeros((t_n, 32, dv), dtype=self.xdtype, device=ccl.device)
        q2 = qc.permute(1, 0, 2, 3).reshape(2, t_n, h_n, 64)
        for b in (0, 1):
            ops.gemm(q2[b].permute(1, 0, 2), f["wkt"][b], None, out=qp[:, b * h_n:(b + 1) * h_n, :].permute(1, 0, 2))
        o = ops.cls_cross_attention(tok, qp, SCALE, x_index=rows)
        ops.gemm(o[:, :2 * h_n, :].permute(1, 0, 2), f["wv"], f["bv"], out=ccl.view(t_n, 2 * h_n, 64).permute(1, 0, 2))

    def _cross_projected(self, ly, qc, ccl, tok, emask, kv_chunk):
        d, (t_n, n, dv) = self.geo.hidden_size, tok.shape
        cand2 = tok.reshape(t_n * n, dv)
        step_c = kv_chunk if kv_chunk > 0 else t_n
        for c0 in range(0, t_n, step_c):
            c1 = min(c0 + step_c, t_n)
            kv = ops.gemm(cand2[c0 * n:c1 * n], ly["wkv"], ly["bkv"]).view(c1 - c0, n, 4, d)
            ops.attention(qc[c0:c1], kv[:, :, 0::2].permute(0, 2, 1, 3), kv[:, :, 1::2].permute(0, 2, 1, 3),
                          ccl[c0:c1].permute(0, 2, 1, 3), SCALE, None if emask is None else emask[c0:c1])

    def _merge_ffn(self, ly, lp: LayerPlan, ccl, a32, rq):
        d, dt, eps, xdt, s8 = self.geo.hidden_size, self.dtype, self.geo.layer_norm_eps, self.xdtype, self.split == 8
        if "wd" in ly:
            dd = torch.empty((rq, 2, d), dtype=xdt, device=ccl.device)
            ops.gemm(ccl.view(rq, 2, d).permute(1, 0, 2), ly["wd"], ly["bd"], out=dd.permute(1, 0, 2))
            m = ops.gemm(dd.view(rq, 2 * d), ly["wm"], ly["bm"], out_dtype=lp.sdt)
        else:
            m = ops.gemm(ccl.view(rq, 2 * d), ly["wm"], ly["bm"], out_dtype=lp.sdt)
        x32, x16 = _ln(m, ly["g2"], ly["b2"], eps, dt, lp.sdt, residual=a32, split8=s8)
        f = ops.gemm(x16.view(2 * rq, d) if not s8 else x16.view(2 * rq), ly["w1"], ly["c1"], act=ops.ACT_GELU)
        t = ops.gemm(f, ly["w2"], ly["c2"], residual=x32.view(2 * rq, d), out_dtype=lp.sdt)
        h32, h16 = _ln(t, ly["g3"], ly["b3"], eps, dt, lp.sdt_out, split8=s8)
        return h32.view(2, rq, d), (h16.view(2, rq, d) if not s8 else h16.view(2, rq))

    def forward(self, input_ids: torch.Tensor, attention_mask: torch.Tensor, z_t32: torch.Tensor, cand16: Optional[torch.Tensor],
                qidx: torch.Tensor, cand_mask: Optional[torch.Tensor] = None, taps: Optional[list] = None,
                kv_bank: Optional[list] = None, cand_rows: Optional[torch.Tensor] = None) -> torch.Tensor:
        d, l = self.geo.hidden_size, input_ids.shape[1]
        if kv_bank is not None:
            if getattr(kv_bank, "engine", None) is None or kv_bank.engine() is not self:
                raise RuntimeError("kv_bank was not built by this engine: the model's parameters were written (or its precision changed) since "
                                   "build_kv_bank - its K/V are projections of the old weights; build the bank again")
            bank, tok, cand_rows = tuple(kv is None for kv in kv_bank), kv_bank.tokens, cand_rows.to(torch.int64).contiguous()
            t_n, n = cand_rows.shape[0], kv_bank[0].shape[1]
        else:
            bank, tok, cand_rows, (t_n, n), kv_bank = None, cand16, None, cand16.shape[:2], [None] * len(self.layers)
        plan = self.plan(l, n, tok.shape[2], cand_mask is not None, bank)
        a32, a16, smask = self._query_block(input_ids, attention_mask, z_t32, qidx, t_n, plan.layers[0].sdt)
        self.fold_fallbacks += plan.fallback
        if plan.fallback and self.fold_fallbacks == 1:
            warnings.warn(f"captions of {l} tokens (> 32): the cross-attention runs the projected K|V path for this batch (~8 % of a step slower than "
                          "the query-side fold at 224 px); NlvrEngine.fold_fallbacks counts such calls; 33-64 tokens against <= 224 keys can take the "
                          "long-caption fold instead: BLIP_NLVR.set_long_caption_fold(); against 225-608 keys (384 px) its key-split form: "
                          "BLIP_NLVR.set_long_caption_fold_wide()", stacklevel=3)
        emask2d = additive_encoder_mask(cand_mask).view(t_n, n) if cand_mask is not None else None
        cc = torch.empty((t_n, l, 2, d), dtype=self.xdtype, device=z_t32.device)
        h32 = h16 = None
        for ly, lp, kv in zip(self.layers, plan.layers, kv_bank):
            lq = 1 if lp.cls_only else l
            if h32 is not None:
                a32, a16 = self._self_block(ly, h32, h16, t_n, l, smask, lp.sdt, lq)
            ccl = self._cross_block(ly, lp, a16, cc, tok, emask2d, cand_rows, kv, plan.kv_chunk)
            h32, h16 = self._merge_ffn(ly, lp, ccl, a32, t_n * lq)
            if taps is not None:
                hv = h32.view(2, t_n, lq, d)
                taps.append((hv[0, :, 0, :8].float(), hv[1, :, 0, :8].float()))
        lq = 1 if plan.layers[-1].cls_only else l
        hcls = h32 if self.split == 8 else h16
        hid = hcls.view(2, t_n, lq, d)[:, :, 0, :].permute(1, 0, 2).reshape(t_n, 2 * d)
        y = ops.gemm(hid, self.wc0, self.bc0, act=ops.ACT_RELU)
        return ops.small_linear(y, self.wc2, self.bc2)


class ScoreGraph:

    def __init__(self, eng: "NlvrEngine", ids, mask, z32, cand16, qidx):
        self.ids, self.mask, self.z, self.cand, self.qidx = (t.clone() for t in (ids, mask, z32, cand16, qidx))
        side = torch.cuda.Stream()
        side.wait_stream(torch.cuda.current_stream())
        with torch.cuda.stream(side):
            for _ in range(2):
                eng.forward(self.ids, self.mask, self.z, self.cand, self.qidx)
        torch.cuda.current_stream().wait_stream(side)
        self.graph = torch.cuda.CUDAGraph()
        with torch.cuda.graph(self.graph):
            self.out = eng.forward(self.ids, self.mask, self.z, self.cand, self.qidx)

    def __call__(self, ids, mask, z32, cand16, qidx) -> torch.Tensor:
        self.ids.copy_(ids); self.mask.copy_(mask); self.z.copy_(z32); self.cand.copy_(cand16); self.qidx.copy_(qidx)
        self.graph.replay()
        return self.out.clone()


def _pad8(m: torch.Tensor) -> torch.Tensor:
    pad = (-m.shape[1]) % 8
    if pad == 0:
        return m.contiguous()
    return torch.cat([m, m.new_zeros((m.shape[0], pad))], dim=1).contiguous()
```

candidate_reranking_cir_amd/lib.py:

```python
from __future__ import annotations

import ctypes
import os
from ctypes import c_uint64, c_char_p, c_float, c_int, c_int64, c_void_p

_HERE = os.path.dirname(os.path.abspath(__file__))
LIB_PATH = os.environ.get("CIR_LIB", os.path.join(_HERE, "libcirrank.so"))

CIR_BF16, CIR_F16, CIR_F32 = 0, 1, 2
TUNE_GEMM_TILE, TUNE_GEMM_GROUP_W, TUNE_ATTN_SHARED_MAX = 0, 1, 2
ACT_NONE, ACT_GELU, ACT_RELU = 0, 1, 2

class WgradDesc(ctypes.Structure):
    _fields_ = [("dy", c_void_p), ("ldy", c_int64), ("x", c_void_p), ("ldx", c_int64), ("dw", c_void_p), ("ldw", c_int64), ("rows", c_int64),
                ("N", c_int), ("K", c_int), ("splits", c_int)]


SIGNATURES = {
    "cir_version": (c_int, []),
    "cir_strerror": (c_char_p, [c_int]),
    "cir_set_tuning": (c_int, [c_int, c_int]),
    "cir_gemm_bias_act": (c_int, [c_void_p, c_int64, c_int64, c_void_p, c_int64, c_int64, c_void_p, c_int64,
                                  c_void_p, c_int, c_int64, c_int64, c_void_p, c_int64, c_int64,
                                  c_int64, c_int, c_int, c_int, c_int, c_int, c_int, c_void_p]),
    "cir_gemm_ln_bias_act": (c_int, [c_void_p, c_int64, c_void_p, c_int64, c_void_p, c_void_p, c_void_p, c_int64,
                                     c_int64, c_int, c_int, c_float, c_int, c_int, c_void_p]),
    "cir_split16": (c_int, [c_void_p, c_int64, c_void_p, c_void_p, c_void_p, c_int64, c_int64, c_int, c_int, c_void_p]),
    "cir_split8": (c_int, [c_void_p, c_int64, c_void_p, c_int64, c_int64, c_int, c_int, c_void_p]),
    "cir_gemm_split8": (c_int, [c_void_p, c_int64, c_int64, c_void_p, c_int64, c_int64, c_void_p, c_int64, c_void_p, c_int64, c_int64,
                                c_void_p, c_int64, c_int64, c_int64, c_int, c_int, c_int, c_int, c_int, c_int, c_int, c_void_p]),
    "cir_layernorm_split8": (c_int, [c_void_p, c_int64, c_void_p, c_int64, c_void_p, c_void_p, c_int64, c_void_p, c_int64, c_void_p, c_int64, c_int64,
                                     c_int64, c_int, c_int, c_float, c_void_p]),
    "cir_layernorm": (c_int, [c_void_p, c_int, c_int64, c_void_p, c_int64, c_void_p, c_void_p, c_int64, c_void_p, c_int, c_void_p,
                              c_int64, c_int64, c_int, c_int, c_float, c_int, c_void_p]),
    "cir_attention": (c_int, [c_void_p, c_int64, c_int64, c_int64, c_void_p, c_int64, c_int64, c_int64,
                              c_void_p, c_int64, c_int64, c_int64, c_void_p, c_int64, c_int64, c_void_p,
                              c_void_p, c_int64, c_int64, c_int64,
                              c_int, c_int, c_int, c_int, c_int, c_float, c_int, c_void_p]),
    "cir_attention_split8": (c_int, [c_void_p, c_int64, c_int64, c_int64, c_void_p, c_int64, c_int64, c_int64, c_void_p, c_int64, c_int64, c_int64,
                                     c_void_p, c_int64, c_int64, c_void_p, c_int64, c_int64, c_int64, c_int, c_int, c_int, c_int, c_int, c_float, c_void_p]),
    "cir_cls_cross_attention": (c_int, [c_void_p, c_int64, c_void_p, c_void_p, c_void_p, c_int, c_int, c_int, c_float, c_int, c_void_p]),
    "cir_cross_attention_folded": (c_int, [c_void_p, c_int64, c_int64, c_void_p, c_int64, c_void_p, c_void_p, c_int64, c_void_p, c_void_p, c_int64, c_void_p, c_int64, c_int64,
                                           c_int64, c_int, c_int, c_int, c_int, c_int, c_float, c_int, c_void_p]),
    "cir_cross_attention_folded_long": (c_int, [c_void_p, c_int64, c_int64, c_void_p, c_int64, c_void_p, c_void_p, c_int64, c_void_p, c_void_p, c_int64, c_void_p, c_int64,
                                                c_int64, c_int64, c_int, c_int, c_int, c_int, c_int, c_float, c_int, c_void_p]),
    "cir_cross_attention_folded_short": (c_int, [c_void_p, c_int64, c_int64, c_void_p, c_int64, c_void_p, c_void_p, c_int64, c_void_p, c_void_p, c_int64, c_void_p, c_int64,
                                                 c_int64, c_int64, c_int, c_int, c_int, c_int, c_int, c_float, c_int, c_void_p]),
    "cir_cross_attention_folded_long_wide": (c_int, [c_void_p, c_int64, c_int64, c_void_p, c_int64, c_void_p, c_void_p, c_int64, c_void_p, c_void_p, c_int64, c_void_p,
                                                     c_int64, c_int64, c_int64, c_int, c_int, c_int, c_int, c_int, c_float, c_int, c_void_p]),
    "cir_embed_layernorm": (c_int, [c_void_p, c_void_p, c_void_p, c_void_p, c_void_p, c_void_p, c_int, c_void_p,
                                    c_int64, c_int, c_int, c_int, c_float, c_int, c_void_p]),
    "cir_patchify": (c_int, [c_void_p, c_int, c_void_p, c_int, c_int, c_int, c_int, c_int, c_int, c_void_p]),
    "cir_vit_assemble": (c_int, [c_void_p, c_void_p, c_void_p, c_void_p, c_int, c_int, c_int, c_int, c_void_p]),
    "cir_small_linear": (c_int, [c_void_p, c_int64, c_void_p, c_void_p, c_void_p, c_int64, c_int, c_int, c_int, c_void_p]),
    "cir_gather_rows": (c_int, [c_void_p, c_int, c_void_p, c_void_p, c_int, c_int64, c_int64, c_int64, c_void_p]),
    "cir_topk_desc": (c_int, [c_void_p, c_void_p, c_int, c_int, c_void_p]),
    "cir_topk_select_workspace": (c_int64, [c_int, c_int, c_int]),
    "cir_topk_select": (c_int, [c_void_p, c_int64, c_void_p, c_void_p, c_void_p, c_int, c_int, c_int, c_void_p, c_int64, c_void_p]),
    "cir_rank_of": (c_int, [c_void_p, c_int64, c_void_p, c_void_p, c_void_p, c_int, c_int, c_int, c_void_p]),
    "cir_linear_f32": (c_int, [c_void_p, c_int64, c_void_p, c_void_p, c_void_p, c_int64, c_int, c_int, c_int, c_void_p]),
    "cir_l2_normalize": (c_int, [c_void_p, c_void_p, c_int64, c_int, c_void_p]),
    "cir_transpose16": (c_int, [c_void_p, c_void_p, c_int, c_int, c_int64, c_int64, c_int, c_int64, c_int64, c_int, c_void_p]),
    "cir_bmm": (c_int, [c_void_p, c_void_p, c_void_p, c_int, c_int, c_int, c_int64, c_int64, c_int64, c_int, c_int, c_int, c_int,
                        c_int64, c_int64, c_int64, c_int64, c_int64, c_int64, c_float, c_int, c_int, c_int, c_void_p]),
    "cir_softmax_dropout": (c_int, [c_void_p, c_int64, c_void_p, c_int64, c_int64, c_void_p, c_void_p, c_int64, c_int64, c_int, c_float, c_float,
                                    c_uint64, c_int, c_void_p]),
    "cir_softmax_dropout_bwd": (c_int, [c_void_p, c_int64, c_void_p, c_int64, c_void_p, c_int64, c_int64, c_int, c_float, c_float, c_uint64, c_int,
                                        c_void_p]),
    "cir_attention_train_fwd": (c_int, [c_void_p, c_int64, c_int64, c_int64, c_void_p, c_int64, c_int64, c_int64, c_void_p, c_int64, c_int64, c_int64,
                                        c_void_p, c_void_p, c_int64, c_int64, c_int64, c_void_p, c_void_p, c_int, c_int, c_int, c_int, c_float, c_float, c_uint64,
                                        c_int, c_void_p]),
    "cir_attention_train_bwd": (c_int, [c_void_p, c_int64, c_int64, c_int64, c_void_p, c_int64, c_int64, c_int64, c_void_p, c_int64, c_int64, c_int64,
                                        c_void_p, c_void_p, c_void_p, c_int64, c_int64, c_int64, c_void_p, c_void_p, c_void_p,
                                        c_void_p, c_int64, c_int64, c_int64, c_void_p, c_int64, c_int64, c_int64, c_void_p, c_int64, c_int64, c_int64,
                                        c_int, c_int, c_int, c_int, c_int, c_float, c_float, c_uint64, c_int, c_void_p]),
    "cir_residual_layernorm_train": (c_int, [c_void_p, c_void_p, c_void_p, c_void_p, c_void_p, c_void_p, c_void_p, c_void_p, c_int64, c_int, c_float,
                                             c_float, c_float, c_uint64, c_int, c_void_p]),
    "cir_layernorm_bwd_fused": (c_int, [c_void_p, c_void_p, c_void_p, c_void_p, c_void_p, c_void_p, c_void_p, c_void_p, c_void_p, c_void_p, c_int64,
                                        c_int, c_float, c_float, c_float, c_uint64, c_int, c_void_p]),
    "cir_rows16_colsum": (c_int, [c_void_p, c_int64, c_void_p, c_int64, c_void_p, c_int64, c_void_p, c_int64, c_int, c_int, c_int, c_void_p]),
    "cir_transpose16_multi": (c_int, [c_void_p, c_void_p, c_void_p, c_int, c_int64, c_int, c_void_p]),
    "cir_wgrad_grouped": (c_int, [c_void_p, c_int, c_int, c_void_p]),
    "cir_wgrad": (c_int, [c_void_p, c_int64, c_void_p, c_int64, c_void_p, c_int64, c_int64, c_int, c_int, c_int, c_int, c_void_p]),
    "cir_rows_scale_add": (c_int, [c_void_p, c_void_p, c_void_p, c_void_p, c_int64, c_int, c_int64, c_int, c_void_p]),
    "cir_layernorm_bwd": (c_int, [c_void_p, c_void_p, c_void_p, c_void_p, c_void_p, c_void_p, c_int64, c_int, c_float, c_void_p]),
    "cir_eltwise": (c_int, [c_void_p, c_int, c_void_p, c_void_p, c_int, c_int64, c_int, c_float, c_uint64, c_void_p]),
    "cir_colsum": (c_int, [c_void_p, c_int64, c_void_p, c_int64, c_int, c_void_p]),
    "cir_embed_bwd": (c_int, [c_void_p, c_void_p, c_void_p, c_void_p, c_int64, c_int, c_int, c_void_p]),
    "cir_colsum_ordered": (c_int, [c_void_p, c_int64, c_void_p, c_int64, c_int, c_void_p, c_int64, c_void_p]),
    "cir_layernorm_bwd_ordered": (c_int, [c_void_p, c_void_p, c_void_p, c_void_p, c_void_p, c_void_p, c_int64, c_int, c_float, c_void_p, c_int64, c_void_p]),
    "cir_layernorm_bwd_fused_ordered": (c_int, [c_void_p, c_void_p, c_void_p, c_void_p, c_void_p, c_void_p, c_void_p, c_void_p, c_void_p, c_void_p, c_int64,
                                                c_int, c_float, c_float, c_float, c_uint64, c_int, c_void_p, c_int64, c_void_p]),
    "cir_rows16_colsum_ordered": (c_int, [c_void_p, c_int64, c_void_p, c_int64, c_void_p, c_int64, c_void_p, c_int64, c_int, c_int, c_int, c_void_p, c_int64,
                                          c_void_p]),
    "cir_embed_bwd_ordered": (c_int, [c_void_p, c_void_p, c_void_p, c_void_p, c_int64, c_int, c_int, c_int64, c_void_p, c_int64, c_void_p, c_int64, c_void_p]),
    "cir_adamw_step": (c_int, [c_void_p, c_void_p, c_void_p, c_void_p, c_int64, c_float, c_float, c_float, c_float, c_float, c_int, c_void_p]),
    "cir_grads_check": (c_int, [c_void_p, c_int64, c_float, c_void_p, c_void_p]),
    "cir_adamw_begin": (c_int, [c_void_p, c_float, c_float, c_void_p]),
    "cir_adamw_step_dev": (c_int, [c_void_p, c_void_p, c_void_p, c_void_p, c_int64, c_float, c_float, c_float, c_float, c_float, c_void_p, c_void_p, c_int, c_void_p]),
    "cir_contrastive_fwd": (c_int, [c_void_p, c_void_p, c_void_p, c_void_p, c_void_p, c_void_p, c_int, c_int, c_int, c_int, c_void_p]),
    "cir_contrastive_bwd": (c_int, [c_void_p, c_void_p, c_void_p, c_void_p, c_void_p, c_void_p, c_void_p, c_void_p, c_void_p, c_int64, c_void_p,
                                    c_void_p, c_int64, c_void_p, c_void_p, c_int, c_int, c_int, c_int, c_int, c_void_p]),
}

_lib = None
TUNING = {}
PARAM_EPOCH = [0]


class CirrankError(RuntimeError):
    pass


def load() -> ctypes.CDLL:
    global _lib
    if _lib is not None:
        return _lib
    if not os.path.exists(LIB_PATH):
        raise ImportError(
            f"{LIB_PATH} is missing: build the gfx950 kernels first "
            f"(`python -c 'import __graft_entry__ as g; g.build()'` or `make -C candidate_reranking_cir_amd/csrc`). "
            f"There is no CPU/PyTorch fallback for this path.")
    import torch
    lib = ctypes.CDLL(LIB_PATH)
    for name, (restype, argtypes) in SIGNATURES.items():
        fn = getattr(lib, name)
        fn.restype = restype
        fn.argtypes = argtypes
    from . import ABI_VERSION
    if lib.cir_version() != ABI_VERSION:
        raise ImportError(f"libcirrank.so ABI {lib.cir_version()} != expected {ABI_VERSION}: rebuild")
    _lib = lib
    return lib


def set_tuning(knob: int, value: int):
    check(load().cir_set_tuning(knob, value), "cir_set_tuning")
    TUNING[knob] = value


def check(code: int, what: str):
    if code != 0:
        msg = load().cir_strerror(code).decode()
        raise CirrankError(f"{what} failed: {msg} (code {code})")
```

candidate_reranking_cir_amd/ops.py:

```python
from __future__ import annotations

from typing import Optional

import torch

from . import lib as _lib
from .lib import ACT_GELU, ACT_NONE, ACT_RELU, CIR_BF16, CIR_F16, CIR_F32

_DT = {torch.bfloat16: CIR_BF16, torch.float16: CIR_F16, torch.float32: CIR_F32}


PROFILE_GEMM = None
PROFILE_ATTN = None


def gemm_kernel_name(m: int, n: int, k: int, nb: int, has_residual: bool, act: int, out_dtype, in_dtype: torch.dtype, tile: int = 0,
                     res_dtype=None, lda: int = 0, ldw: int = 0, form: str = "gemm") -> str:
    if form == "ln":
        return f"cir::gemm256_kernel<_Float16,false,false,float,{act},true>"
    split8 = form == "split8"
    if in_dtype == torch.float32 and not split8:
        return "cir::gemm_kernel<float,1>"
    if isinstance(out_dtype, bool):
        out_dtype = torch.float32 if out_dtype else in_dtype
    t = "__bf16" if in_dtype == torch.bfloat16 else "_Float16"
    stream16 = out_dtype == torch.float16 and (in_dtype != torch.float16 or (has_residual and res_dtype == torch.float16))
    kind = 1 if out_dtype == torch.float32 else (2 if stream16 else 0)
    nblk256 = -(-m // 256) * -(-n // 256) * nb
    use256 = n >= 256 and nblk256 >= 192
    can256 = split8 or (not (has_residual and (act != ACT_NONE or kind == 0)) and k % 128 == 0)
    if tile == 128:
        use256 = False
    elif tile == 256:
        use256 = True
    if not (use256 and can256 and lda < (1 << 21) and ldw < (1 << 21)):
        return "cir::gemm_split8_kernel" if split8 else f"cir::gemm_kernel<{t},{kind}>"
    if split8:
        return "cir::gemm256_kernel<split8%s>" % (",split8-out" if out_dtype == torch.uint8 else (",residual" if has_residual else ""))
    name = f"cir::gemm256_kernel<{t},{'true' if kind == 1 else 'false'},{'true' if has_residual else 'false'}"
    if kind == 2:
        return name + (",_Float16,0>" if act == ACT_NONE else ",_Float16>")
    if kind == 0 and act in (ACT_NONE, ACT_GELU):
        return name + f",float,{act}>"
    return name + ">"


def _events():
    e0, e1 = torch.cuda.Event(enable_timing=True), torch.cuda.Event(enable_timing=True)
    e0.record()
    return e0, e1


def _stream() -> int:
    return torch._C._cuda_getCurrentRawStream(torch._C._cuda_getDevice())


def _need_cuda(*tensors):
    for t in tensors:
        if t is not None and not t.is_cuda:
            raise _lib.CirrankError("cirrank ops need device tensors (no CPU fallback exists)")


def _ptr(t: Optional[torch.Tensor]) -> Optional[int]:
    return None if t is None else t.data_ptr()


def _rows2d(x: torch.Tensor) -> torch.Tensor:
    k = x.shape[-1]
    if x.dim() == 2:
        return x
    if x.is_contiguous():
        return x.reshape(-1, k)
    if x.dim() == 3 and x.stride(0) == x.shape[1] * x.stride(1):
        return x.as_strided((x.shape[0] * x.shape[1], k), (x.stride(1), 1))
    return x.contiguous().view(-1, k)


def _gemm_views(a: torch.Tensor, w: torch.Tensor, bias, residual, out, out_dtype: torch.dtype, out_per_n: int = 1):
    batched = a.dim() == 3
    a3 = a if batched else a.unsqueeze(0)
    w3 = w if w.dim() == 3 else w.unsqueeze(0)
    nb, m, kk = a3.shape
    wb, n, wk = w3.shape
    out_cols = n * out_per_n
    assert wb == nb and wk == kk and a3.stride(2) == 1 and w3.stride(2) == 1
    if out is None:
        out = torch.empty((nb, m, out_cols) if batched else (m, out_cols), dtype=out_dtype, device=a.device)
    o3 = out if out.dim() == 3 else out.unsqueeze(0)
    assert o3.shape == (nb, m, out_cols) and o3.stride(2) == 1 and o3.dtype == out_dtype
    sb = 0
    if bias is not None:
        assert bias.dtype == torch.float32 and bias.stride(-1) == 1
        sb = bias.stride(0) if bias.dim() == 2 else 0
    ldr = sr = 0
    if residual is not None:
        r3 = residual if residual.dim() == 3 else residual.unsqueeze(0)
        assert r3.shape == (nb, m, n) and r3.stride(2) == 1
        ldr, sr = r3.stride(1), r3.stride(0)
    return a3, w3, out, o3, nb, m, n, kk, sb, ldr, sr


class SplitOperand:
    dtype = torch.float32

    def __init__(self, cat: torch.Tensor, k: int):
        self.cat, self.k, self.shape, self.device = cat, k, cat.shape[:-1] + (k,), cat.device

    @property
    def hi(self):
        return self.cat[..., :self.k]

    @property
    def lo(self):
        return self.cat[..., self.k:2 * self.k]

    def dim(self):
        return self.cat.dim()


def split16(x: torch.Tensor, act: int = ACT_NONE) -> SplitOperand:
    _need_cuda(x)
    assert x.dtype == torch.float32 and x.stride(-1) == 1
    k = x.shape[-1]
    x2 = _rows2d(x)
    cat = torch.empty(x.shape[:-1] + (3 * k,), dtype=torch.float16, device=x.device)
    p = cat.data_ptr()
    _lib.check(_lib.load().cir_split16(x2.data_ptr(), x2.stride(0), p, p + 2 * k, p + 4 * k, 3 * k, x2.shape[0], k, act, _stream()), "cir_split16")
    return SplitOperand(cat, k)


def split_weight(w32: torch.Tensor) -> torch.Tensor:
    hi = w32.to(torch.float16)
    lo = (w32 - hi.float()).to(torch.float16)
    w32._split3 = torch.cat([hi, hi, lo], dim=-1).contiguous()
    return w32


def _gemm_split3(a, w_cat, bias, residual, act, out):
    sa = a if isinstance(a, SplitOperand) else split16(a)
    assert act == ACT_NONE or residual is None, "activation and residual do not meet on this path"
    n_rec = len(PROFILE_GEMM) if PROFILE_GEMM is not None else 0
    s_ = gemm(sa.cat, w_cat, bias, residual=residual, out_dtype=torch.float32, out=out)
    if PROFILE_GEMM is not None and len(PROFILE_GEMM) > n_rec:
        fl, e0, e1, nbytes, name = PROFILE_GEMM[-1]
        PROFILE_GEMM[-1] = (fl / 3.0, e0, e1, nbytes, name.replace("cir::", "cir::split3:"))
    if act == ACT_GELU:
        return split16(s_, ACT_GELU)
    if act == ACT_RELU:
        s_.relu_()
    return s_


class Split8Operand:
    dtype = torch.float32

    def __init__(self, rows: torch.Tensor, k: int):
        assert rows.dtype == torch.uint8 and rows.shape[-1] == 4 * k and rows.stride(-1) == 1
        self.rows, self.k, self.shape, self.device = rows, k, rows.shape[:-1] + (k,), rows.device

    def dim(self):
        return self.rows.dim()

    def view(self, *lead) -> "Split8Operand":
        return Split8Operand(self.rows.view(*lead, 4 * self.k), self.k)

    def float(self) -> torch.Tensor:
        k = self.k
        hi = self.rows[..., :2 * k].contiguous().view(torch.float16).float()
        lo = self.rows[..., 2 * k:3 * k].contiguous().view(torch.float8_e4m3fn).float() * 2.0 ** -12
        return hi + lo


def split8(x: torch.Tensor, act: int = ACT_NONE, out: Optional[torch.Tensor] = None) -> Split8Operand:
    _need_cuda(x, out)
    assert x.dtype == torch.float32 and x.stride(-1) == 1
    k = x.shape[-1]
    x2 = _rows2d(x)
    if out is None:
        out = torch.empty(x.shape[:-1] + (4 * k,), dtype=torch.uint8, device=x.device)
    assert out.is_contiguous() and out.dtype == torch.uint8 and out.numel() == x2.shape[0] * 4 * k
    _lib.check(_lib.load().cir_split8(x2.data_ptr(), x2.stride(0), out.data_ptr(), 4 * k, x2.shape[0], k, act, _stream()), "cir_split8")
    return Split8Operand(out, k)


def _e4m3(x: torch.Tensor) -> torch.Tensor:
    x = x.clamp(-448.0, 448.0)
    try:
        return x.to(torch.float8_e4m3fn).view(torch.uint8)
    except (RuntimeError, TypeError):
        return x.cpu().to(torch.float8_e4m3fn).view(torch.uint8).to(x.device)


def split_weight8(w32: torch.Tensor) -> torch.Tensor:
    import math
    hi = w32.to(torch.float16)
    lo = w32 - hi.float()
    e1 = int(math.floor(math.log2(224.0 / max(float(hi.float().abs().max()), 1e-30))))
    e2 = int(math.floor(math.log2(224.0 / max(float(lo.abs().max()), 1e-30))))
    e1, e2 = max(min(e1, 60), -60), max(min(e2, 60), -60)
    rows = torch.cat([hi.contiguous().view(torch.uint8), _e4m3(hi.float() * 2.0 ** e1), _e4m3(lo * 2.0 ** e2)], dim=-1).contiguous()
    w32._split8 = (rows, e1, e2)
    return w32


def _gemm_split8(a, wpack, bias, residual, act, out):
    rows_w, e1, e2 = wpack
    sa = a if isinstance(a, Split8Operand) else split8(a)
    _need_cuda(sa.rows, rows_w, bias, residual, out)
    assert act == ACT_NONE or residual is None, "activation and residual do not meet on this path"
    assert residual is None or residual.dtype == torch.float32
    out_split = act == ACT_GELU
    assert out is None or not out_split
    k = sa.k
    a3, w3, res, o3, nb, m, n, _, sb, ldr, sr = _gemm_views(sa.rows, rows_w, bias, residual, out, *((torch.uint8, 4) if out_split else (torch.float32, 1)))
    ev = _events() if PROFILE_GEMM is not None else None
    code = _lib.load().cir_gemm_split8(a3.data_ptr(), a3.stride(1), a3.stride(0), w3.data_ptr(), w3.stride(1), w3.stride(0), _ptr(bias), sb,
                                       _ptr(residual), ldr, sr, o3.data_ptr(), o3.stride(1), o3.stride(0), m, n, k, nb, act, int(out_split),
                                       e1, e2, _stream())
    if ev is not None:
        ev[1].record()
        alg_bytes = nb * ((m * k + n * k) * 4 + m * n * 4 + (m * n * 4 if residual is not None else 0) + (n * 4 if bias is not None else 0))
        PROFILE_GEMM.append((2.0 * nb * m * n * k, *ev, float(alg_bytes),
                             gemm_kernel_name(m, n, k, nb, residual is not None, act, o3.dtype, torch.float32, _lib.TUNING.get(_lib.TUNE_GEMM_TILE, 0),
                                              lda=a3.stride(1) // 2, ldw=w3.stride(1) // 2, form="split8")))
    _lib.check(code, "cir_gemm_split8")
    return Split8Operand(res, n) if out_split else res


def gemm(a: torch.Tensor, w: torch.Tensor, bias: Optional[torch.Tensor] = None, residual: Optional[torch.Tensor] = None,
         act: int = ACT_NONE, out_dtype: Optional[torch.dtype] = None, out: Optional[torch.Tensor] = None) -> torch.Tensor:
    if isinstance(a, Split8Operand) or (not isinstance(a, SplitOperand) and a.dtype == torch.float32 and getattr(w, "_split8", None) is not None):
        assert out_dtype in (None, torch.float32) and getattr(w, "_split8", None) is not None
        return _gemm_split8(a, w._split8, bias, residual, act, out)
    if isinstance(a, SplitOperand) or (a.dtype == torch.float32 and getattr(w, "_split3", None) is not None):
        assert out_dtype in (None, torch.float32) and getattr(w, "_split3", None) is not None
        return _gemm_split3(a, w._split3, bias, residual, act, out)
    _need_cuda(a, w, bias, residual, out)
    assert w.dtype == a.dtype, "operands of one type (16-bit, or fp32 for the exact mode)"
    out_dtype = out_dtype or a.dtype
    if residual is not None:
        assert residual.dtype == torch.float32 or (residual.dtype == torch.float16 and out_dtype == torch.float16), \
            "residual: fp32, or fp16 with an fp16 out"
        assert not (out_dtype == torch.float16 and a.dtype != torch.float16 and residual.dtype != torch.float16), \
            "an fp16 out from bf16 operands (residual stream) takes an fp16 residual"
    a3, w3, out, o3, nb, m, n, k, sb, ldr, sr = _gemm_views(a, w, bias, residual, out, out_dtype)
    ev = _events() if PROFILE_GEMM is not None else None
    code = _lib.load().cir_gemm_bias_act(
        a3.data_ptr(), a3.stride(1), a3.stride(0), w3.data_ptr(), w3.stride(1), w3.stride(0),
        _ptr(bias), sb, _ptr(residual), _DT[residual.dtype] if residual is not None else CIR_F32, ldr, sr,
        o3.data_ptr(), o3.stride(1), o3.stride(0), m, n, k, nb, act, _DT[a.dtype], _DT[out_dtype], _stream())
    if ev is not None:
        ev[1].record()
        alg_bytes = nb * ((m * k + n * k) * a.element_size() + m * n * o3.element_size()
                          + (m * n * residual.element_size() if residual is not None else 0) + (n * 4 if bias is not None else 0))
        PROFILE_GEMM.append((2.0 * nb * m * n * k, *ev, float(alg_bytes),
                             gemm_kernel_name(m, n, k, nb, residual is not None, act, out_dtype, a.dtype, _lib.TUNING.get(_lib.TUNE_GEMM_TILE, 0),
                                              residual.dtype if residual is not None else None, a3.stride(1), w3.stride(1))))
    _lib.check(code, "cir_gemm_bias_act")
    return out


def ln_fold_pack(w: torch.Tensor, b: torch.Tensor, gamma: torch.Tensor, beta: torch.Tensor, dtype=torch.float16):
    w32, g32 = w.detach().float(), gamma.detach().float()
    wg = (w32 * g32[None, :]).to(dtype).contiguous()
    colsum = wg.double().sum(dim=1).float().contiguous()
    bias = (b.detach().double() + w32.double() @ beta.detach().double()).float().contiguous()
    return wg, colsum, bias


def gemm_ln(x: torch.Tensor, wg: torch.Tensor, colsum: torch.Tensor, bias: torch.Tensor, eps: float, act: int = ACT_NONE,
            out: Optional[torch.Tensor] = None) -> torch.Tensor:
    _need_cuda(x, wg, colsum, bias, out)
    m, k = x.shape
    n = wg.shape[0]
    assert x.dtype == torch.float16 and wg.dtype == torch.float16 and x.stride(1) == 1 and wg.stride(1) == 1 and wg.shape[1] == k
    assert colsum.dtype == torch.float32 and bias.dtype == torch.float32 and colsum.shape == (n,) and bias.shape == (n,)
    if out is None:
        out = torch.empty((m, n), dtype=torch.float16, device=x.device)
    assert out.shape == (m, n) and out.dtype == torch.float16 and out.stride(1) == 1
    ev = _events() if PROFILE_GEMM is not None else None
    code = _lib.load().cir_gemm_ln_bias_act(x.data_ptr(), x.stride(0), wg.data_ptr(), wg.stride(0), colsum.data_ptr(), bias.data_ptr(),
                                            out.data_ptr(), out.stride(0), m, n, k, float(eps), act, CIR_F16, _stream())
    if ev is not None:
        ev[1].record()
        PROFILE_GEMM.append((2.0 * m * n * k, *ev, float((m * k + n * k + m * n) * 2 + n * 8),
                             gemm_kernel_name(m, n, k, 1, False, act, torch.float16, torch.float16, form="ln")))
    _lib.check(code, "cir_gemm_ln_bias_act")
    return out


def _ln_views(x: torch.Tensor, gamma: torch.Tensor, residual: Optional[torch.Tensor], dtypes):
    x3 = x if x.dim() == 3 else x.unsqueeze(0)
    nb = max(x3.shape[0], gamma.shape[0] if gamma.dim() == 2 else 1, (residual.shape[0] if residual is not None and residual.dim() == 3 else 1))
    rows, cols = x3.shape[1], x3.shape[2]
    assert x3.dtype in dtypes and x3.stride(2) == 1 and x3.stride(1) == cols
    sx = x3.stride(0) if x3.shape[0] > 1 else 0
    sr = 0
    if residual is not None:
        r3 = residual if residual.dim() == 3 else residual.unsqueeze(0)
        assert r3.dtype == x3.dtype and r3.stride(2) == 1 and r3.stride(1) == cols
        sr = r3.stride(0) if r3.shape[0] > 1 else 0
    sg = gamma.stride(0) if gamma.dim() == 2 else 0
    return x3, nb, rows, cols, ((nb, rows) if (x.dim() == 3 or nb > 1) else (rows,)), sx, sr, sg


def layernorm(x: torch.Tensor, gamma: torch.Tensor, beta: torch.Tensor, eps: float, residual: Optional[torch.Tensor] = None,
              out32: Optional[torch.Tensor] = None, out16: Optional[torch.Tensor] = None, want32: bool = True,
              dtype16: Optional[torch.dtype] = torch.bfloat16, stream_dtype: Optional[torch.dtype] = None):
    _need_cuda(x, gamma, beta, residual)
    x3, nb, rows, cols, lead, sx, sr, sg = _ln_views(x, gamma, residual, (torch.float32, torch.float16))
    stream_dtype = stream_dtype or (out32.dtype if out32 is not None else x3.dtype)
    assert stream_dtype in (torch.float32, torch.float16)
    if out32 is None and want32:
        out32 = torch.empty(lead + (cols,), dtype=stream_dtype, device=x.device)
    if out16 is None and dtype16 is not None:
        out16 = torch.empty(lead + (cols,), dtype=dtype16, device=x.device)
    d16 = _DT[out16.dtype] if out16 is not None else CIR_BF16
    code = _lib.load().cir_layernorm(x3.data_ptr(), _DT[x3.dtype], sx, _ptr(residual), sr, gamma.data_ptr(), beta.data_ptr(), sg,
                                     _ptr(out32), _DT[out32.dtype] if out32 is not None else CIR_F32, _ptr(out16), rows * cols, rows, cols, nb,
                                     float(eps), d16, _stream())
    _lib.check(code, "cir_layernorm")
    return out32, out16


def layernorm_split8(x: torch.Tensor, gamma: torch.Tensor, beta: torch.Tensor, eps: float, residual: Optional[torch.Tensor] = None,
                     want_stream: bool = True):
    _need_cuda(x, gamma, beta, residual)
    x3, nb, rows, cols, lead, sx, sr, sg = _ln_views(x, gamma, residual, (torch.float32,))
    ys = torch.empty(lead + (cols,), dtype=torch.float32, device=x.device) if want_stream else None
    sp = torch.empty(lead + (4 * cols,), dtype=torch.uint8, device=x.device)
    code = _lib.load().cir_layernorm_split8(x3.data_ptr(), sx, _ptr(residual), sr, gamma.data_ptr(), beta.data_ptr(), sg, _ptr(ys), rows * cols,
                                            sp.data_ptr(), 4 * cols, rows * 4 * cols, rows, cols, nb, float(eps), _stream())
    _lib.check(code, "cir_layernorm_split8")
    return ys, Split8Operand(sp, cols)


def attention_split8(q: torch.Tensor, k: torch.Tensor, v: torch.Tensor, scale: float, mask: Optional[torch.Tensor] = None) -> Split8Operand:
    _need_cuda(q, k, v, mask)
    b1, b0, lq, d = q.shape
    lk = k.shape[2]
    assert k.shape == (b1, b0, lk, d) and v.shape == k.shape and d % 64 == 0
    assert q.dtype == k.dtype == v.dtype == torch.float32 and q.stride(3) == 1 and k.stride(3) == 1 and v.stride(3) == 1
    out = torch.empty((b1, b0, lq, 4 * d), dtype=torch.uint8, device=q.device)
    _attention_launch("cir_attention_split8", q, k, v, mask, (), out, (float(scale),))
    return Split8Operand(out, d)


def _attention_launch(entry: str, q: torch.Tensor, k: torch.Tensor, v: torch.Tensor, mask: Optional[torch.Tensor], extra: tuple, out: torch.Tensor,
                      tail: tuple):
    b1, b0, lq, d = q.shape
    lk = k.shape[2]
    ms1 = ms0 = 0
    if mask is not None:
        assert mask.dtype == torch.float32 and mask.shape == (b1, b0, lk) and mask.stride(2) == 1
        ms1, ms0 = mask.stride(0), mask.stride(1)
    ev = _events() if PROFILE_ATTN is not None else None
    code = getattr(_lib.load(), entry)(
        q.data_ptr(), q.stride(0), q.stride(1), q.stride(2), k.data_ptr(), k.stride(0), k.stride(1), k.stride(2),
        v.data_ptr(), v.stride(0), v.stride(1), v.stride(2), _ptr(mask), ms1, ms0, *extra,
        out.data_ptr(), out.stride(0), out.stride(1), out.stride(2), b1, b0, d // 64, lq, lk, *tail, _stream())
    if ev is not None:
        ev[1].record()
        PROFILE_ATTN.append((4.0 * b1 * b0 * lq * lk * d, *ev, (lq, lk)))
    _lib.check(code, entry)


def attention(q: torch.Tensor, k: torch.Tensor, v: torch.Tensor, out: torch.Tensor, scale: float,
              mask: Optional[torch.Tensor] = None, kv_index: Optional[torch.Tensor] = None) -> torch.Tensor:
    _need_cuda(q, k, v, out, mask, kv_index)
    b1, b0, lq, d = q.shape
    lk = k.shape[2]
    if kv_index is None:
        assert k.shape == (b1, b0, lk, d)
    else:
        assert kv_index.dtype == torch.int64 and kv_index.shape == (b1,) and kv_index.is_contiguous() and k.shape[1:] == (b0, lk, d)
    assert d % 64 == 0 and v.shape == k.shape and out.shape == q.shape
    assert q.stride(3) == 1 and k.stride(3) == 1 and v.stride(3) == 1 and out.stride(3) == 1
    assert q.dtype == k.dtype == v.dtype == out.dtype
    _attention_launch("cir_attention", q, k, v, mask, (_ptr(kv_index),), out, (float(scale), _DT[q.dtype]))
    return out


def cls_cross_attention(x: torch.Tensor, qp: torch.Tensor, scale: float, out: Optional[torch.Tensor] = None,
                        x_index: Optional[torch.Tensor] = None) -> torch.Tensor:
    _need_cuda(x, qp, out, x_index)
    lk, d = x.shape[1], x.shape[2]
    t_n = qp.shape[0]
    assert x_index is not None or x.shape[0] == t_n
    assert x_index is None or (x_index.dtype == torch.int64 and x_index.shape == (t_n,) and x_index.is_contiguous())
    assert x.stride(2) == 1 and x.stride(1) == d and qp.shape == (t_n, 32, d) and qp.is_contiguous() and qp.dtype == x.dtype
    if out is None:
        out = torch.empty((t_n, 32, d), dtype=x.dtype, device=x.device)
    assert out.shape == (t_n, 32, d) and out.is_contiguous() and out.dtype == x.dtype
    _lib.check(_lib.load().cir_cls_cross_attention(x.data_ptr(), x.stride(0), _ptr(x_index), qp.data_ptr(), out.data_ptr(), t_n, lk, d,
                                                   float(scale), _DT[x.dtype], _stream()), "cir_cls_cross_attention")
    return out


def fold_pack_key(wk: torch.Tensor) -> torch.Tensor:
    b, d, _ = wk.shape
    h = d // 64
    w = wk.view(b, h, 2, 4, 8, d // 32, 4, 2, 4)
    return w.permute(0, 5, 7, 1, 2, 3, 6, 8, 4).contiguous().view(b, d, d)


def fold_pack_value(wv: torch.Tensor) -> torch.Tensor:
    b, d, _ = wv.shape
    h = d // 64
    w = wv.view(b, h, 4, 16, d // 32, 2, 4, 4)
    return w.permute(0, 4, 2, 1, 6, 3, 5, 7).contiguous().view(b, d, d)


def _cross_attention_folded(entry: str, q: torch.Tensor, x: torch.Tensor, wkt: torch.Tensor, wvp: torch.Tensor, bv: torch.Tensor, out: torch.Tensor, l: int,
                            scale: float, heads: int, mask: Optional[torch.Tensor]) -> torch.Tensor:
    _need_cuda(q, x, wkt, wvp, bv, out)
    t_n, n, d = x.shape
    assert q.shape == (2, t_n * l, d) and q.stride(2) == 1 and x.stride(2) == 1 and x.stride(1) == d
    assert wkt.shape == (2, d, d) and wvp.shape == (2, d, d) and wkt.is_contiguous() and wvp.is_contiguous() and bv.shape == (2, d) and bv.is_contiguous()
    assert out.shape == (t_n, l, 2, d) and out.stride(3) == 1 and q.dtype == x.dtype == wkt.dtype == wvp.dtype == out.dtype and bv.dtype == torch.float32
    if mask is not None:
        _need_cuda(mask)
        assert mask.dtype == torch.float32 and mask.shape == (t_n, n) and mask.stride(1) == 1
    ev = _events() if PROFILE_ATTN is not None else None
    code = getattr(_lib.load(), entry)(q.data_ptr(), q.stride(0), q.stride(1), x.data_ptr(), x.stride(0), wkt.data_ptr(), wvp.data_ptr(), d * d,
                                       bv.data_ptr(), _ptr(mask), mask.stride(0) if mask is not None else 0,
                                       out.data_ptr(), out.stride(0), out.stride(1), out.stride(2), t_n, l, n, d, heads,
                                       float(scale), _DT[x.dtype], _stream())
    if ev is not None:
        ev[1].record()
        PROFILE_ATTN.append((2.0 * t_n * 2 * (2 * heads * l * 64 * d + 2 * heads * l * d * n), *ev, ("folded", l, n)))
    _lib.check(code, entry)
    return out


def cross_attention_folded(q: torch.Tensor, x: torch.Tensor, wkt: torch.Tensor, wvp: torch.Tensor, bv: torch.Tensor, out: torch.Tensor, l: int,
                           scale: float, heads: int = 12, mask: Optional[torch.Tensor] = None) -> torch.Tensor:
    return _cross_attention_folded("cir_cross_attention_folded", q, x, wkt, wvp, bv, out, l, scale, heads, mask)


def cross_attention_folded_long(q: torch.Tensor, x: torch.Tensor, wkt: torch.Tensor, wvp: torch.Tensor, bv: torch.Tensor, out: torch.Tensor, l: int,
                                scale: float, heads: int = 12, mask: Optional[torch.Tensor] = None) -> torch.Tensor:
    return _cross_attention_folded("cir_cross_attention_folded_long", q, x, wkt, wvp, bv, out, l, scale, heads, mask)


def cross_attention_folded_short(q: torch.Tensor, x: torch.Tensor, wkt: torch.Tensor, wvp: torch.Tensor, bv: torch.Tensor, out: torch.Tensor, l: int,
                                 scale: float, heads: int = 12, mask: Optional[torch.Tensor] = None) -> torch.Tensor:
    return _cross_attention_folded("cir_cross_attention_folded_short", q, x, wkt, wvp, bv, out, l, scale, heads, mask)


def cross_attention_folded_long_wide(q: torch.Tensor, x: torch.Tensor, wkt: torch.Tensor, wvp: torch.Tensor, bv: torch.Tensor, out: torch.Tensor, l: int,
                                     scale: float, heads: int = 12, mask: Optional[torch.Tensor] = None) -> torch.Tensor:
    return _cross_attention_folded("cir_cross_attention_folded_long_wide", q, x, wkt, wvp, bv, out, l, scale, heads, mask)


def embed_layernorm(ids: torch.Tensor, word: torch.Tensor, pos: torch.Tensor, gamma: torch.Tensor, beta: torch.Tensor,
                    eps: float, dtype16: torch.dtype = torch.bfloat16, stream_dtype: torch.dtype = torch.float32):
    _need_cuda(ids, word, pos, gamma, beta)
    r, l = ids.shape
    cols = word.shape[1]
    if l > pos.shape[0]:
        raise IndexError(f"caption of {l} tokens exceeds the {pos.shape[0]}-row position-embedding table")
    ids = ids.contiguous()
    y32 = torch.empty((r, l, cols), dtype=stream_dtype, device=ids.device)
    if dtype16 == torch.float32:
        assert stream_dtype == torch.float32
        y16 = None
    else:
        y16 = torch.empty((r, l, cols), dtype=dtype16, device=ids.device)
    code = _lib.load().cir_embed_layernorm(ids.data_ptr(), word.data_ptr(), pos.data_ptr(), gamma.data_ptr(), beta.data_ptr(),
                                           y32.data_ptr(), _DT[stream_dtype], _ptr(y16), r * l, l, cols, word.shape[0], float(eps),
                                           CIR_F16 if y16 is None else _DT[dtype16], _stream())
    _lib.check(code, "cir_embed_layernorm")
    return y32, (y32 if y16 is None else y16)


def patchify(image: torch.Tensor, patch: int, dtype16: torch.dtype = torch.bfloat16) -> torch.Tensor:
    _need_cuda(image)
    image = image.contiguous()
    b, c, h, w = image.shape
    out = torch.empty((b * (h // patch) * (w // patch), c * patch * patch), dtype=dtype16, device=image.device)
    code = _lib.load().cir_patchify(image.data_ptr(), _DT[image.dtype], out.data_ptr(), _DT[dtype16], b, c, h, w, patch, _stream())
    _lib.check(code, "cir_patchify")
    return out


def vit_assemble(proj: torch.Tensor, cls: torch.Tensor, pos: torch.Tensor, batch: int) -> torch.Tensor:
    _need_cuda(proj, cls, pos)
    assert proj.dtype in (torch.float32, torch.float16) and proj.is_contiguous()
    p = proj.shape[0] // batch
    d = proj.shape[1]
    x = torch.empty((batch, p + 1, d), dtype=proj.dtype, device=proj.device)
    code = _lib.load().cir_vit_assemble(proj.data_ptr(), cls.data_ptr(), pos.data_ptr(), x.data_ptr(), _DT[proj.dtype], batch, p, d, _stream())
    _lib.check(code, "cir_vit_assemble")
    return x


def small_linear(x: torch.Tensor, w: torch.Tensor, bias: Optional[torch.Tensor]) -> torch.Tensor:
    _need_cuda(x, w, bias)
    if x.dtype == torch.float32:
        return linear_f32(x, w, bias)
    m, k = x.shape
    n = w.shape[0]
    assert x.stride(1) == 1 and w.is_contiguous()
    y = torch.empty((m, n), dtype=torch.float32, device=x.device)
    code = _lib.load().cir_small_linear(x.data_ptr(), x.stride(0), w.data_ptr(), _ptr(bias), y.data_ptr(), m, n, k, _DT[x.dtype], _stream())
    _lib.check(code, "cir_small_linear")
    return y


def argsort_desc(logits: torch.Tensor) -> torch.Tensor:
    _need_cuda(logits)
    logits = logits.contiguous()
    q, k = logits.shape
    idx = torch.empty((q, k), dtype=torch.int64, device=logits.device)
    code = _lib.load().cir_topk_desc(logits.data_ptr(), idx.data_ptr(), q, k, _stream())
    _lib.check(code, "cir_topk_desc")
    return idx


def _rank_rows(values: torch.Tensor, exclude: Optional[torch.Tensor]):
    _need_cuda(values, exclude)
    assert values.dim() == 2 and values.dtype == torch.float32 and values.shape[0] < 2 ** 31 and values.shape[1] < 2 ** 31
    if values.stride(1) != 1 or values.stride(0) < values.shape[1]:
        values = values.contiguous()
    if exclude is not None:
        exclude = exclude.to(torch.int64).contiguous()
        assert exclude.shape == (values.shape[0],)
    return values, exclude


def topk_desc(values: torch.Tensor, k: int, exclude: Optional[torch.Tensor] = None, return_values: bool = False):
    values, exclude = _rank_rows(values, exclude)
    q, n = values.shape
    c = _lib.load()
    need = c.cir_topk_select_workspace(q, n, k)
    if need < 0:
        _lib.check(int(need), "cir_topk_select_workspace")
    work = torch.empty(need, dtype=torch.uint8, device=values.device)
    idx = torch.empty((q, k), dtype=torch.int64, device=values.device)
    val = torch.empty((q, k), dtype=torch.float32, device=values.device) if return_values else None
    code = c.cir_topk_select(values.data_ptr(), values.stride(0), _ptr(exclude), idx.data_ptr(), _ptr(val), q, n, k, work.data_ptr(), need, _stream())
    _lib.check(code, "cir_topk_select")
    return (idx, val) if return_values else idx


def rank_of(values: torch.Tensor, cols: torch.Tensor, exclude: Optional[torch.Tensor] = None) -> torch.Tensor:
    values, exclude = _rank_rows(values, exclude)
    _need_cuda(cols)
    cols = cols.to(torch.int64).contiguous()
    q, n = values.shape
    assert cols.dim() == 2 and cols.shape[0] == q
    rank = torch.empty_like(cols)
    code = _lib.load().cir_rank_of(values.data_ptr(), values.stride(0), cols.data_ptr(), _ptr(exclude), rank.data_ptr(), q, n, cols.shape[1], _stream())
    _lib.check(code, "cir_rank_of")
    return rank


def gather_rows(src: torch.Tensor, index: Optional[torch.Tensor], dtype: Optional[torch.dtype] = None) -> torch.Tensor:
    _need_cuda(src, index)
    src = src.contiguous()
    dtype = dtype or src.dtype
    row_elems = src[0].numel()
    n = src.shape[0] if index is None else index.numel()
    dst = torch.empty((n,) + tuple(src.shape[1:]), dtype=dtype, device=src.device)
    if index is not None:
        index = index.to(torch.int64).contiguous()
    code = _lib.load().cir_gather_rows(src.data_ptr(), _DT[src.dtype], _ptr(index), dst.data_ptr(), _DT[dtype], n, row_elems,
                                       src.shape[0], _stream())
    _lib.check(code, "cir_gather_rows")
    return dst


def linear_f32(x: torch.Tensor, w: torch.Tensor, bias: Optional[torch.Tensor] = None, mode: int = 0) -> torch.Tensor:
    _need_cuda(x, w, bias)
    assert x.dtype == torch.float32 and w.dtype == torch.float32 and x.stride(1) == 1 and w.is_contiguous()
    m, k = x.shape
    n = w.shape[0]
    y = torch.empty((m, n), dtype=torch.float32, device=x.device)
    code = _lib.load().cir_linear_f32(x.data_ptr(), x.stride(0), w.data_ptr(), _ptr(bias), y.data_ptr(), m, n, k, mode, _stream())
    _lib.check(code, "cir_linear_f32")
    return y


def l2_normalize(x: torch.Tensor) -> torch.Tensor:
    _need_cuda(x)
    x = x.contiguous()
    y = torch.empty_like(x)
    code = _lib.load().cir_l2_normalize(x.data_ptr(), y.data_ptr(), x.shape[0], x.shape[1], _stream())
    _lib.check(code, "cir_l2_normalize")
    return y
```

include/cirrank.h:

```cpp
#ifndef CIRRANK_H
#define CIRRANK_H

#include <stdint.h>

#ifdef __cplusplus
extern "C" {
#endif

#define CIR_ABI_VERSION 15

enum { CIR_BF16 = 0, CIR_F16 = 1, CIR_F32 = 2 };
enum { CIR_ACT_NONE = 0, CIR_ACT_GELU = 1, CIR_ACT_RELU = 2 };
enum {
    CIR_OK = 0,
    CIR_EINVAL = -1,
    CIR_ESHAPE = -2,
    CIR_EALIGN = -3,
    CIR_EDTYPE = -4
};

int cir_version(void);
const char* cir_strerror(int code);

enum { CIR_TUNE_GEMM_TILE = 0, CIR_TUNE_GEMM_GROUP_W = 1, CIR_TUNE_ATTN_SHARED_MAX = 2 };
int cir_set_tuning(int knob, int value);

int cir_gemm_bias_act(const void* A, int64_t lda, int64_t strideA,
                      const void* W, int64_t ldw, int64_t strideW,
                      const float* bias, int64_t strideBias,
                      const void* residual, int res_dtype, int64_t ldr, int64_t strideR,
                      void* C, int64_t ldc, int64_t strideC,
                      int64_t M, int N, int K, int batch,
                      int act, int in_dtype, int out_dtype, void* stream);

int cir_gemm_ln_bias_act(const void* X, int64_t ldx, const void* Wg, int64_t ldw, const float* colsum, const float* bias,
                         void* C, int64_t ldc, int64_t M, int N, int K, float eps, int act, int dtype, void* stream);

int cir_split16(const float* x, int64_t ldx, void* hi, void* lo, void* hi2, int64_t ldo, int64_t rows, int cols, int act, void* stream);

int cir_split8(const float* x, int64_t ldx, void* out, int64_t ldo_bytes, int64_t rows, int cols, int act, void* stream);

int cir_attention_split8(const float* q, int64_t q_s1, int64_t q_s0, int64_t q_rs, const float* k, int64_t k_s1, int64_t k_s0, int64_t k_rs,
                         const float* v, int64_t v_s1, int64_t v_s0, int64_t v_rs, const float* mask, int64_t m_s1, int64_t m_s0,
                         void* out, int64_t o_s1_bytes, int64_t o_s0_bytes, int64_t o_rs_bytes, int B1, int B0, int H, int Lq, int Lk,
                         float scale, void* stream);

int cir_layernorm_split8(const float* x, int64_t strideX, const float* residual, int64_t strideR, const float* gamma, const float* beta,
                         int64_t strideG, float* y_stream, int64_t strideY, void* y_split, int64_t ld_split_bytes, int64_t stride_split_bytes,
                         int64_t rows, int cols, int batch, float eps, void* stream);

int cir_gemm_split8(const void* A, int64_t lda_bytes, int64_t strideA_bytes, const void* W, int64_t ldw_bytes, int64_t strideW_bytes,
                    const float* bias, int64_t strideBias, const float* residual, int64_t ldr, int64_t strideR,
                    void* C, int64_t ldc, int64_t strideC, int64_t M, int N, int K, int batch, int act, int out_split,
                    int w_exp_hi, int w_exp_lo, void* stream);

int cir_layernorm(const void* x, int x_dtype, int64_t strideX, const void* residual, int64_t strideR,
                  const float* gamma, const float* beta, int64_t strideG,
                  void* y_stream, int y_stream_dtype, void* y16, int64_t strideY,
                  int64_t rows, int cols, int batch, float eps, int dtype16, void* stream);

int cir_attention(const void* q, int64_t q_s1, int64_t q_s0, int64_t q_rs,
                  const void* k, int64_t k_s1, int64_t k_s0, int64_t k_rs,
                  const void* v, int64_t v_s1, int64_t v_s0, int64_t v_rs,
                  const float* mask, int64_t m_s1, int64_t m_s0, const int64_t* kv_index,
                  void* out, int64_t o_s1, int64_t o_s0, int64_t o_rs,
                  int B1, int B0, int H, int Lq, int Lk, float scale, int dtype, void* stream);

int cir_cls_cross_attention(const void* x, int64_t x_s1, const int64_t* x_index, const void* qp, void* out, int T, int Lk, int D,
                            float scale, int dtype, void* stream);

int cir_cross_attention_folded(const void* q, int64_t q_sb, int64_t q_rs, const void* x, int64_t x_s1, const void* wkt, const void* wvp, int64_t w_sb,
                               const float* bv, const float* key_mask, int64_t mask_stride, void* out, int64_t o_st, int64_t o_sr, int64_t o_sb,
                               int T, int L, int N, int D, int H, float scale, int dtype, void* stream);

int cir_cross_attention_folded_long(const void* q, int64_t q_sb, int64_t q_rs, const void* x, int64_t x_s1, const void* wkt, const void* wvp, int64_t w_sb,
                                    const float* bv, const float* key_mask, int64_t mask_stride, void* out, int64_t o_st, int64_t o_sr, int64_t o_sb,
                                    int T, int L, int N, int D, int H, float scale, int dtype, void* stream);

int cir_cross_attention_folded_short(const void* q, int64_t q_sb, int64_t q_rs, const void* x, int64_t x_s1, const void* wkt, const void* wvp, int64_t w_sb,
                                     const float* bv, const float* key_mask, int64_t mask_stride, void* out, int64_t o_st, int64_t o_sr, int64_t o_sb,
                                     int T, int L, int N, int D, int H, float scale, int dtype, void* stream);

int cir_cross_attention_folded_long_wide(const void* q, int64_t q_sb, int64_t q_rs, const void* x, int64_t x_s1, const void* wkt, const void* wvp, int64_t w_sb,
                                         const float* bv, const float* key_mask, int64_t mask_stride, void* out, int64_t o_st, int64_t o_sr, int64_t o_sb,
                                         int T, int L, int N, int D, int H, float scale, int dtype, void* stream);

int cir_embed_layernorm(const int64_t* ids, const float* word, const float* pos,
                        const float* gamma, const float* beta, void* y_stream, int y_stream_dtype, void* y16,
                        int64_t rows, int L, int cols, int vocab, float eps, int dtype16, void* stream);

int cir_patchify(const void* image, int img_dtype, void* patches, int dtype16,
                 int B, int C, int H, int Wd, int patch, void* stream);

int cir_vit_assemble(const void* proj, const float* cls, const float* pos, void* x, int stream_dtype,
                     int B, int P, int D, void* stream);

int cir_small_linear(const void* x, int64_t ldx, const void* W, const float* bias, float* y,
                     int64_t M, int N, int K, int dtype, void* stream);

int cir_gather_rows(const void* src, int src_dtype, const int64_t* index, void* dst, int dst_dtype,
                    int64_t n_rows, int64_t row_elems, int64_t src_rows, void* stream);

int cir_topk_desc(const float* logits, int64_t* idx, int Q, int K, void* stream);

int64_t cir_topk_select_workspace(int Q, int n, int k);
int cir_topk_select(const float* values, int64_t ld, const int64_t* exclude, int64_t* idx, float* val, int Q, int n, int k,
                    void* workspace, int64_t workspace_bytes, void* stream);
int cir_rank_of(const float* values, int64_t ld, const int64_t* cols, const int64_t* exclude, int64_t* rank, int Q, int n, int m, void* stream);

int cir_linear_f32(const float* x, int64_t ldx, const float* W, const float* bias, float* y,
                   int64_t M, int N, int K, int mode, void* stream);

int cir_l2_normalize(const float* x, float* y, int64_t rows, int cols, void* stream);


int cir_transpose16(const void* src, void* dst, int rows, int cols, int64_t ld_src, int64_t ld_dst, int batch, int64_t s_src, int64_t s_dst,
                    int dtype, void* stream);
int cir_transpose16_multi(const void* src, void* dst, const int64_t* table, int count, int64_t total_tiles, int dtype, void* stream);
int cir_bmm(const void* A, const void* B, void* C, int M, int N, int K, int64_t lda, int64_t ldb, int64_t ldc, int trans_a, int trans_b,
            int nb1, int nb2, int64_t sA1, int64_t sA2, int64_t sB1, int64_t sB2, int64_t sC1, int64_t sC2, float alpha, int accumulate,
            int in_dtype, int out_dtype, void* stream);
int cir_wgrad(const void* dy, int64_t ldy, const void* x, int64_t ldx, float* dw, int64_t ldw, int64_t rows, int N, int K, int splits, int in_dtype,
              void* stream);
typedef struct { const void* dy; int64_t ldy; const void* x; int64_t ldx; float* dw; int64_t ldw; int64_t rows; int N, K, splits; } cir_wgrad_desc;
int cir_wgrad_grouped(const cir_wgrad_desc* problems, int count, int in_dtype, void* stream);
int cir_softmax_dropout(const float* S, int64_t ld_s, const float* mask, int64_t rows_per_mask, int64_t ld_mask, void* P, void* Pd, int64_t ld_p,
                        int64_t rows, int cols, float scale, float p_drop, uint64_t seed, int dtype, void* stream);
int cir_softmax_dropout_bwd(const void* P, int64_t ld_p, const float* dPd, int64_t ld_d, void* dS, int64_t ld_ds, int64_t rows, int cols,
                            float scale, float p_drop, uint64_t seed, int dtype, void* stream);
int cir_attention_train_fwd(const void* q, int64_t q_sg, int64_t q_sh, int64_t q_sr, const void* k, int64_t k_sg, int64_t k_sh, int64_t k_sr,
                            const void* v, int64_t v_sg, int64_t v_sh, int64_t v_sr, const float* mask, void* out, int64_t o_sg, int64_t o_sh,
                            int64_t o_sr, float* out32, float* lse, int G, int H, int Lq, int Lk, float scale, float p_drop, uint64_t seed,
                            int dtype, void* stream);
int cir_attention_train_bwd(const void* q, int64_t q_sg, int64_t q_sh, int64_t q_sr, const void* k, int64_t k_sg, int64_t k_sh, int64_t k_sr,
                            const void* v, int64_t v_sg, int64_t v_sh, int64_t v_sr, const float* mask, const void* out, const void* d_out,
                            int64_t o_sg, int64_t o_sh, int64_t o_sr, const float* out32, const float* lse,
                            float* dsum_scratch, void* dq, int64_t dq_sg,
                            int64_t dq_sh, int64_t dq_sr, void* dk, int64_t dk_sg, int64_t dk_sh, int64_t dk_sr, void* dv, int64_t dv_sg,
                            int64_t dv_sh, int64_t dv_sr, int grad_dtype, int G, int H, int Lq, int Lk, float scale, float p_drop, uint64_t seed,
                            int dtype, void* stream);
int cir_layernorm_bwd(const float* x, const float* gamma, const float* dy, float* dx, float* dgamma, float* dbeta, int64_t rows, int cols,
                      float eps, void* stream);
int cir_residual_layernorm_train(const float* t0, const float* t1, const float* residual, const float* gamma, const float* beta, float* pre,
                                 float* y32, void* y16, int64_t rows, int cols, float eps, float alpha, float p_drop, uint64_t seed, int dtype16,
                                 void* stream);
int cir_layernorm_bwd_fused(const float* x, const float* gamma, const float* dy, float* dx, float* dgamma, float* dbeta, const float* t_add,
                            void* dt16, float* dbias, float* dbias2, int64_t rows, int cols, float eps, float alpha, float p_drop, uint64_t seed,
                            int dtype16, void* stream);
int cir_rows16_colsum(const void* a, int64_t lda, const void* z, int64_t ldz, void* out, int64_t ldo, float* sums, int64_t rows, int cols, int mode,
                      int dtype, void* stream);
int cir_rows_scale_add(const float* a, const float* b, const float* scale, void* out, int64_t rows, int cols, int64_t rows_per_group, int out_dtype,
                       void* stream);
int cir_eltwise(const void* z, int z_dtype, const float* dy, void* out, int out_dtype, int64_t n, int mode, float p_drop, uint64_t seed, void* stream);
int cir_colsum(const float* x, int64_t ld, float* out, int64_t rows, int cols, void* stream);
int cir_embed_bwd(const int64_t* ids, const float* dy, float* dword, float* dpos, int64_t rows, int L, int cols, void* stream);
int cir_colsum_ordered(const float* x, int64_t ld, float* out, int64_t rows, int cols, float* partials, int64_t partial_elems, void* stream);
int cir_layernorm_bwd_ordered(const float* x, const float* gamma, const float* dy, float* dx, float* dgamma, float* dbeta, int64_t rows, int cols,
                              float eps, float* partials, int64_t partial_elems, void* stream);
int cir_layernorm_bwd_fused_ordered(const float* x, const float* gamma, const float* dy, float* dx, float* dgamma, float* dbeta, const float* t_add,
                                    void* dt16, float* dbias, float* dbias2, int64_t rows, int cols, float eps, float alpha, float p_drop,
                                    uint64_t seed, int dtype16, float* partials, int64_t partial_elems, void* stream);
int cir_rows16_colsum_ordered(const void* a, int64_t lda, const void* z, int64_t ldz, void* out, int64_t ldo, float* sums, int64_t rows, int cols,
                              int mode, int dtype, float* partials, int64_t partial_elems, void* stream);
int cir_embed_bwd_ordered(const int64_t* ids, const float* dy, float* dword, float* dpos, int64_t rows, int L, int cols, int64_t table_rows,
                          float* partials, int64_t partial_elems, int32_t* index, int64_t index_elems, void* stream);
int cir_adamw_step(float* p, const float* g, float* m, float* v, int64_t n, float lr, float beta1, float beta2, float eps, float weight_decay,
                   int step, void* stream);
int cir_grads_check(float* g, int64_t n, float scale, int32_t* state, void* stream);
int cir_adamw_begin(int32_t* state, float beta1, float beta2, void* stream);
int cir_adamw_step_dev(float* p, const float* g, float* m, float* v, int64_t n, float lr, float beta1, float beta2, float eps, float weight_decay,
                       const int32_t* state, void* p16, int dtype16, void* stream);
int cir_contrastive_fwd(const float* p, const float* target, const float* temp, float* p_hat, float* inv_norm, float* logits, int B, int Bt, int E,
                        int dtype, void* stream);
int cir_contrastive_bwd(const float* dlogits, const float* target, const float* temp, const float* p_hat, const float* inv_norm, float* dp,
                        float* row_scratch, float* dtemp, const float* x, int64_t ldx, const float* W, float* dx, int64_t lddx, float* dW, float* db,
                        int D, int B, int Bt, int E, int dtype, void* stream);

#ifdef __cplusplus
}
#endif
#endif
```

Before: 18370 triplets/s.

## Add KB=13 fold kernel variant, indexed query entry, and CLS-only split QKV

The folded cross-attention kernel gains a KB template (13 or 14 key blocks), chosen when N fits in 208 keys, which drops one block of score MFMAs and registers for N=197. Query loads are issued early into registers and written to LDS after the first DMA. Masking is hoisted into a per-block pass, and the value bias is prefetched during the last unit. A new indexed entry point lets queries be gathered by index. In the Python engine, the last CLS-only self-attention layer computes Q for the CLS token only and K/V for all tokens, instead of full QKV. These changes add template variants and a new API, and the split GEMM adds one extra launch.

Measured after the change: 18470 triplets/s, median of 6. Within noise of the previous version (+0.6%).

```diff
diff --git a/candidate_reranking_cir_amd/csrc/common.hpp b/candidate_reranking_cir_amd/csrc/common.hpp
--- a/candidate_reranking_cir_amd/csrc/common.hpp
+++ b/candidate_reranking_cir_amd/csrc/common.hpp
@@ -248,7 +248,7 @@
 }
 
 namespace cir {
-extern int g_tune[3];
+extern int g_tune[4];
 
 constexpr int kOrdRows = 256;
 constexpr int kEmbChunk = 512;
diff --git a/candidate_reranking_cir_amd/csrc/misc.hip b/candidate_reranking_cir_amd/csrc/misc.hip
--- a/candidate_reranking_cir_amd/csrc/misc.hip
+++ b/candidate_reranking_cir_amd/csrc/misc.hip
@@ -227,13 +227,14 @@
 
 extern "C" int cir_version(void) { return CIR_ABI_VERSION; }
 
-namespace cir { int g_tune[3] = {0, 0, 0}; }
+namespace cir { int g_tune[4] = {0, 0, 0, 0}; }
 
 extern "C" int cir_set_tuning(int knob, int value) {
     switch (knob) {
         case CIR_TUNE_GEMM_TILE: if (value != 0 && value != 128 && value != 256) return CIR_EINVAL; break;
         case CIR_TUNE_GEMM_GROUP_W: if (value < 0 || value > 64) return CIR_EINVAL; break;
         case CIR_TUNE_ATTN_SHARED_MAX: if (value != 0 && value != -1 && value != -2 && (value < 32 || value > 608)) return CIR_EINVAL; break;
+        case CIR_TUNE_FOLD_KB: if (value != 0 && value != 14) return CIR_EINVAL; break;
         default: return CIR_EINVAL;
     }
     cir::g_tune[knob] = value;
diff --git a/candidate_reranking_cir_amd/csrc/xattn_fold.hip b/candidate_reranking_cir_amd/csrc/xattn_fold.hip
--- a/candidate_reranking_cir_amd/csrc/xattn_fold.hip
+++ b/candidate_reranking_cir_amd/csrc/xattn_fold.hip
@@ -19,8 +19,9 @@
 #define FOLD_STAMP(K) do {} while (0)
 #endif
 
-template <typename T, bool MASKED = false>
+template <typename T, bool MASKED = false, int KB = kFoldKB>
 __global__ __launch_bounds__(512, 2) void xattn_fold_kernel(const FoldArgs a) {
+    static_assert(KB == 13 || KB == 14, "7 key pairs in G3; four request slots behind the 8 weight fragments of a unit in G2");
     using X8 = typename Elem<T>::x8;
     extern __shared__ __attribute__((aligned(16))) char smem[];
 
@@ -42,19 +43,22 @@
     hq[0] = hA; hq[1] = hA; hq[2] = hC;
     tok[0] = l16; tok[1] = 16 + l16; tok[2] = 16 * odd + l16;
     char* const qs = smem + 2 * kFoldBuf;
+    X8 qv[6];
     {
-        const T* qb_ = reinterpret_cast<const T*>(a.q) + (int64_t)b * a.q_sb + (int64_t)t * a.L * a.q_rs;
+        int64_t tq = t;
+        if (a.q_index) {
+            tq = a.q_index[t];
+            tq = tq < 0 ? 0 : (tq > a.Q - 1 ? a.Q - 1 : tq);
+        }
+        const T* qb_ = reinterpret_cast<const T*>(a.q) + (int64_t)b * a.q_sb + tq * a.L * a.q_rs;
 #pragma unroll
         for (int i = 0; i < 6; ++i) {
             const int c = tid + i * 512;
             const int row = c / 96, ch = c - row * 96;
-            X8 v;
-#pragma unroll
-            for (int j = 0; j < 8; ++j) v[j] = static_cast<T>(0.f);
-            if (row < a.L) v = *reinterpret_cast<const X8*>(qb_ + (int64_t)row * a.q_rs + ch * 8);
-            *reinterpret_cast<X8*>(qs + row * kStrideQ + ch * 16) = v;
-        }
-    }
+            qv[i] = *reinterpret_cast<const X8*>(qb_ + (int64_t)min(row, a.L - 1) * a.q_rs + ch * 8);
+        }
+    }
+    __builtin_amdgcn_sched_barrier(0);
     int qoff[3];
 #pragma unroll
     for (int qb = 0; qb < 3; ++qb) qoff[qb] = tok[qb] * kStrideQ + (hq[qb] * 64 + 8 * g) * 2;
@@ -73,9 +77,9 @@
         for (int j = 0; j < 4; ++j) FOLD_DMA(rs_x, xoff1[j], chunk * 128, base + j * 1024);
     };
 
-    f32x4 S[kFoldKB][3];
-#pragma unroll
-    for (int kb = 0; kb < kFoldKB; ++kb)
+    f32x4 S[KB][3];
+#pragma unroll
+    for (int kb = 0; kb < KB; ++kb)
 #pragma unroll
         for (int qb = 0; qb < 3; ++qb) S[kb][qb] = f32x4{0.f, 0.f, 0.f, 0.f};
 
@@ -96,6 +100,25 @@
     FOLD_STAMP(0);
     stage1(0, 0);
     load_wk(0);
+    __builtin_amdgcn_sched_barrier(0);
+#pragma unroll
+    for (int i = 0; i < 6; ++i) {
+        const int c = tid + i * 512;
+        const int row = c / 96, ch = c - row * 96;
+        X8 v = qv[i];
+        if (row >= a.L) {
+#pragma unroll
+            for (int j = 0; j < 8; ++j) v[j] = static_cast<T>(0.f);
+        }
+        *reinterpret_cast<X8*>(qs + row * kStrideQ + ch * 16) = v;
+    }
+    int xoff2[5];
+#pragma unroll
+    for (int j = 0; j < 5; ++j) {
+        const int s = (wave * 5 + j) * 64 + lane;
+        const int row = min(s / 10, a.N - 1), c = min(s % 10, 7);
+        xoff2[j] = (row * kFoldD + c * 8) * 2;
+    }
     for (int kc = 0; kc < kFoldChunks; ++kc) {
         if (kc < 4) FOLD_STAMP(1 + 6 * kc);
         asm volatile("s_waitcnt vmcnt(0)" ::: "memory");
@@ -145,8 +168,8 @@
             xa[0] = rd(0);
             xa[1] = rd(1);
 #pragma unroll
-            for (int kb = 0; kb < kFoldKB; ++kb) {
-                if (kb + 2 < kFoldKB && !(FOLD_DBG & 2)) xa[(kb + 2) % 3] = rd(kb + 2);
+            for (int kb = 0; kb < KB; ++kb) {
+                if (kb + 2 < KB && !(FOLD_DBG & 2)) xa[(kb + 2) % 3] = rd(kb + 2);
                 mem_op(kb);
                 __builtin_amdgcn_sched_barrier(0);
 #pragma unroll
@@ -162,27 +185,47 @@
     float rinv[3];
     X8 P[7][3];
 #pragma unroll
+    for (int kb = 0; kb < KB; ++kb) {
+        const bool partial = 16 * kb + 16 > a.N;
+        if constexpr (MASKED) {
+            const float* mrow = a.mask + (int64_t)t * a.m_st;
+            if (partial) {
+#pragma unroll
+                for (int r = 0; r < 4; ++r) {
+                    const int key = 16 * kb + 4 * g + r;
+                    const float mk = mrow[min(key, a.N - 1)];
+#pragma unroll
+                    for (int qb = 0; qb < 3; ++qb)
+                        S[kb][qb][r] = key < a.N ? fmaf(fmaxf(mk, -2.0e38f), 1.4426950408889634f, S[kb][qb][r] * sl) : -INFINITY;
+                }
+            } else {
+#pragma unroll
+                for (int r = 0; r < 4; ++r) {
+                    const float mk = mrow[16 * kb + 4 * g + r];
+#pragma unroll
+                    for (int qb = 0; qb < 3; ++qb) S[kb][qb][r] = fmaf(fmaxf(mk, -2.0e38f), 1.4426950408889634f, S[kb][qb][r] * sl);
+                }
+            }
+        } else if (partial) {
+#pragma unroll
+            for (int qb = 0; qb < 3; ++qb)
+#pragma unroll
+                for (int r = 0; r < 4; ++r) S[kb][qb][r] = 16 * kb + 4 * g + r < a.N ? S[kb][qb][r] : -INFINITY;
+        }
+    }
+#pragma unroll
     for (int qb = 0; qb < 3; ++qb) {
         float m = -INFINITY;
 #pragma unroll
-        for (int kb = 0; kb < kFoldKB; ++kb)
-#pragma unroll
-            for (int r = 0; r < 4; ++r) {
-                const int key = 16 * kb + 4 * g + r;
-                float v = key < a.N ? S[kb][qb][r] : -INFINITY;
-                if constexpr (MASKED) {
-                    const float mk = a.mask[(int64_t)t * a.m_st + min(key, a.N - 1)];
-                    v = key < a.N ? fmaf(fmaxf(mk, -2.0e38f), 1.4426950408889634f, S[kb][qb][r] * sl) : -INFINITY;
-                }
-                S[kb][qb][r] = v;
-                m = fmaxf(m, v);
-            }
+        for (int kb = 0; kb < KB; ++kb)
+#pragma unroll
+            for (int r = 0; r < 4; ++r) m = fmaxf(m, S[kb][qb][r]);
         m = fmaxf(m, __shfl_xor(m, 16, 64));
         m = fmaxf(m, __shfl_xor(m, 32, 64));
         const float ms = MASKED ? m : m * sl;
         float sum = 0.f;
 #pragma unroll
-        for (int kb = 0; kb < kFoldKB; ++kb)
+        for (int kb = 0; kb < KB; ++kb)
 #pragma unroll
             for (int r = 0; r < 4; ++r) {
                 const float p = MASKED ? __builtin_amdgcn_exp2f(S[kb][qb][r] - ms) : __builtin_amdgcn_exp2f(fmaf(S[kb][qb][r], sl, -ms));
@@ -193,7 +236,10 @@
         sum += __shfl_xor(sum, 32, 64);
         rinv[qb] = 1.0f / sum;
 #pragma unroll
-        for (int p = 0; p < 7; ++p) P[p][qb] = pack_acc2<T>(S[2 * p][qb], S[2 * p + 1][qb]);
+        for (int p = 0; p < 7; ++p) {
+            if constexpr (KB == 14) P[p][qb] = pack_acc2<T>(S[2 * p][qb], S[2 * p + 1][qb]);
+            else P[p][qb] = pack_acc2<T>(S[2 * p][qb], p < 6 ? S[min(2 * p + 1, KB - 1)][qb] : f32x4{0.f, 0.f, 0.f, 0.f});
+        }
     }
 
     f32x4 c4[4][3];
@@ -202,21 +248,12 @@
 #pragma unroll
         for (int qb = 0; qb < 3; ++qb) c4[db][qb] = f32x4{0.f, 0.f, 0.f, 0.f};
     X8 wv[4][2];
-    int xoff2[5];
-#pragma unroll
-    for (int j = 0; j < 5; ++j) {
-        const int s = (wave * 5 + j) * 64 + lane;
-        const int row = min(s / 10, a.N - 1), c = min(s % 10, 7);
-        xoff2[j] = (row * kFoldD + c * 8) * 2;
-    }
-    auto stage2 = [&](int chunk, int buf) {
-        char* base = smem + buf * kFoldBuf + wave * 5 * 1024;
-#pragma unroll
-        for (int j = 0; j < 5; ++j) FOLD_DMA(rs_x, xoff2[j], chunk * 128, base + j * 1024);
-    };
     FOLD_STAMP(26);
     __syncthreads();
-    stage2(0, 0);
+#pragma unroll
+    for (int j = 0; j < 5; ++j) FOLD_DMA(rs_x, xoff2[j], 0, smem + (wave * 5 + j) * 1024);
+    const float* bvb = a.bv + b * kFoldD + 4 * g;
+    float4 bias[2][4];
     const int troff = (4 * g + (l16 >> 2)) * kStride2 + (4 * (l16 & 3)) * 2;
     for (int nc = 0; nc < kFoldChunks; ++nc) {
         if (nc < 4) FOLD_STAMP(27 + 6 * nc);
@@ -233,7 +270,7 @@
 #pragma unroll
                 for (int qb = 0; qb < 3; ++qb) a3[fbh][qb] = f32x4{0.f, 0.f, 0.f, 0.f};
             const int cu = 2 * nc + half;
-            const bool more_x = half == 0 && nc + 1 < kFoldChunks && !(FOLD_DBG & 4);
+            const bool more_x = half == 0 && nc + 1 < kFoldChunks && !(FOLD_DBG & 4), last_unit = cu == 2 * kFoldChunks - 1;
             auto mem_op = [&](int j) {
                 if (j < 8) {
                     if (!(FOLD_DBG & 1) || cu == 0) {
@@ -242,6 +279,10 @@
                     }
                 } else if (j < 13) {
                     if (more_x) FOLD_DMA(rs_x, xoff2[j - 8], (nc + 1) * 128, smem + ((nc + 1) & 1) * kFoldBuf + (wave * 5 + j - 8) * 1024);
+                    if (last_unit && j < 12) {
+                        bias[0][j - 8] = *reinterpret_cast<const float4*>(bvb + hA * 64 + 16 * (j - 8));
+                        bias[1][j - 8] = *reinterpret_cast<const float4*>(bvb + hC * 64 + 16 * (j - 8));
+                    }
                 }
             };
             const unsigned xaddr = (unsigned)(size_t)(lptr_t)(xs) + (32 * half) * 2;
@@ -291,21 +332,38 @@
 
     FOLD_STAMP(51);
     T* ob = reinterpret_cast<T*>(a.out) + (int64_t)t * a.o_st + (int64_t)b * a.o_sb;
-    const float* bvb = a.bv + b * kFoldD;
 #pragma unroll
     for (int qb = 0; qb < 3; ++qb) {
         if (tok[qb] >= a.L) continue;
         T* orow = ob + (int64_t)tok[qb] * a.o_sr + hq[qb] * 64 + 4 * g;
-        const float* brow = bvb + hq[qb] * 64 + 4 * g;
 #pragma unroll
         for (int db = 0; db < 4; ++db) {
-            const float4 b4 = *reinterpret_cast<const float4*>(brow + 16 * db);
+            const float4 b4 = bias[qb == 2][db];
+            float r0 = fmaf(c4[db][qb][0], rinv[qb], b4.x), r1 = fmaf(c4[db][qb][1], rinv[qb], b4.y);
+            float r2 = fmaf(c4[db][qb][2], rinv[qb], b4.z), r3 = fmaf(c4[db][qb][3], rinv[qb], b4.w);
+            asm("" : "+v"(r0), "+v"(r1), "+v"(r2), "+v"(r3));
             u32x2 o;
-            o.x = pack2<T>(fmaf(c4[db][qb][0], rinv[qb], b4.x), fmaf(c4[db][qb][1], rinv[qb], b4.y));
-            o.y = pack2<T>(fmaf(c4[db][qb][2], rinv[qb], b4.z), fmaf(c4[db][qb][3], rinv[qb], b4.w));
+            o.x = pack2<T>(r0, r1);
+            o.y = pack2<T>(r2, r3);
             *reinterpret_cast<u32x2*>(orow + 16 * db) = o;
         }
     }
+}
+
+}
+
+namespace cir {
+
+template <typename T>
+static FoldKernel fold_kernel_of(bool masked, bool kb13) {
+    if (kb13) return masked ? xattn_fold_kernel<T, true, 13> : xattn_fold_kernel<T, false, 13>;
+    return masked ? xattn_fold_kernel<T, true, 14> : xattn_fold_kernel<T, false, 14>;
+}
+
+static int launch_fold48(const FoldArgs& a, int dtype, hipStream_t s) {
+    const bool kb13 = a.N <= 16 * 13 && g_tune[CIR_TUNE_FOLD_KB] != 14;
+    const FoldKernel k = dtype == CIR_BF16 ? fold_kernel_of<__bf16>(a.mask != nullptr, kb13) : fold_kernel_of<_Float16>(a.mask != nullptr, kb13);
+    return fold_launch(k, dim3((unsigned)(8 * ((a.T + 3) / 4))), dim3(512), 2 * kFoldBuf + 32 * kStrideQ, s, a);
 }
 
 }
@@ -320,9 +378,22 @@
     if (rc != CIR_OK) return rc;
     hipStream_t s = reinterpret_cast<hipStream_t>(stream);
     if (N > 16 * kFoldKB) return launch_fold16(a, dtype, s);
-    const FoldKernel k = dtype == CIR_BF16 ? (key_mask ? xattn_fold_kernel<__bf16, true> : xattn_fold_kernel<__bf16, false>)
-                                           : (key_mask ? xattn_fold_kernel<_Float16, true> : xattn_fold_kernel<_Float16, false>);
-    return fold_launch(k, dim3((unsigned)(8 * ((T + 3) / 4))), dim3(512), 2 * kFoldBuf + 32 * kStrideQ, s, a);
+    return launch_fold48(a, dtype, s);
+}
+
+extern "C" int cir_cross_attention_folded_indexed(const void* q, int64_t q_sb, int64_t q_rs, const int64_t* q_index, int Q, const void* x, int64_t x_s1,
+                                                  const void* wkt, const void* wvp, int64_t w_sb, const float* bv, const float* key_mask,
+                                                  int64_t mask_stride, void* out, int64_t o_st, int64_t o_sr, int64_t o_sb, int T, int L, int N, int D,
+                                                  int H, float scale, int dtype, void* stream) {
+    using namespace cir;
+    FoldArgs a;
+    CIR_CHECK_PTR(q_index);
+    if (Q <= 0) return CIR_EINVAL;
+    const int rc = fold_args(a, q, q_sb, q_rs, x, x_s1, wkt, wvp, w_sb, bv, key_mask, mask_stride, out, o_st, o_sr, o_sb, T, L, N, D, H, scale, dtype,
+                             32, 16 * kFoldKB, (int64_t)T * 2);
+    if (rc != CIR_OK) return rc;
+    a.q_index = q_index; a.Q = Q;
+    return launch_fold48(a, dtype, reinterpret_cast<hipStream_t>(stream));
 }
 
 #if FOLD_DBG & 8
diff --git a/candidate_reranking_cir_amd/csrc/xattn_fold.hpp b/candidate_reranking_cir_amd/csrc/xattn_fold.hpp
--- a/candidate_reranking_cir_amd/csrc/xattn_fold.hpp
+++ b/candidate_reranking_cir_amd/csrc/xattn_fold.hpp
@@ -13,6 +13,7 @@
     int T, L, N;
     float scale;
     const float* mask = nullptr; int64_t m_st = 0;
+    const int64_t* q_index = nullptr; int Q = 0;
 };
 
 typedef __attribute__((address_space(3))) s16x4* lds_s16x4_ptr_f;
diff --git a/candidate_reranking_cir_amd/engine.py b/candidate_reranking_cir_amd/engine.py
--- a/candidate_reranking_cir_amd/engine.py
+++ b/candidate_reranking_cir_amd/engine.py
@@ -265,6 +265,7 @@
     layers: Tuple[LayerPlan, ...]
     kv_chunk: int
     fallback: bool
+    cls_split: bool = False
 
 
 SCALE = 64 ** -0.5
@@ -280,6 +281,7 @@
         self.split3 = self.split != 0
         self.xdtype = xdt = cross_dtype or dtype
         self.trim_last = True
+        self.trim = True
         self.kv_chunk = 0
         self.fold_cls_kv = xdt != torch.float32
         self.fold_cross_kv = xdt != torch.float32 and geo.hidden_size == 768 and geo.encoder_width == 768 and geo.num_attention_heads == 12
@@ -381,7 +383,8 @@
                 cross = "projected" if bank is None else "bank"
             layers.append(LayerPlan(cls_only, cross, sd(i), sd(i + 1)))
         fallback = last >= 1 and layers[1].cross == "projected" and self.fold_cross_kv and "wkt" in self.layers[1] and l > 32
-        return Plan(tuple(layers), self.kv_chunk, fallback)
+        cls_split = self.trim and layers[-1].cls_only and self.split != 8 and self.dtype != torch.float32
+        return Plan(tuple(layers), self.kv_chunk, fallback, cls_split)
 
     def graph_key(self, ids_shape, cand_shape, cand_dtype) -> tuple:
         return (tuple(ids_shape), tuple(cand_shape), cand_dtype, self.plan(ids_shape[1], cand_shape[1], cand_shape[2], False))
@@ -419,11 +422,16 @@
         graphs[key] = g
         return g(input_ids, attention_mask, z_t32, cand16, qidx)
 
-    def _self_block(self, ly, h32, h16, items, l, smask, sdt, lq=None):
+    def _self_block(self, ly, h32, h16, items, l, smask, sdt, lq=None, cls_split=False):
         d, eps, lq = self.geo.hidden_size, self.geo.layer_norm_eps, lq or l
-        qkv = ops.gemm(h16, ly["wqkv"], ly["bqkv"]).view(2, items, l, 3 * d)
-        ctx_op = _attend(qkv[:, :, :lq, :d], qkv[..., d:2 * d], qkv[..., 2 * d:], SCALE, smask.unsqueeze(0).expand(2, items, l), self.dtype,
-                         self.split == 8, (2, items * lq))
+        if cls_split and lq == 1:
+            q = ops.gemm(h16.view(2, items, l * d)[:, :, :d], ly["wqkv"][:, :d], ly["bqkv"][:, :d]).view(2, items, 1, d)
+            kv = ops.gemm(h16, ly["wqkv"][:, d:], ly["bqkv"][:, d:]).view(2, items, l, 2 * d)
+            k, v = kv[..., :d], kv[..., d:]
+        else:
+            qkv = ops.gemm(h16, ly["wqkv"], ly["bqkv"]).view(2, items, l, 3 * d)
+            q, k, v = qkv[:, :, :lq, :d], qkv[..., d:2 * d], qkv[..., 2 * d:]
+        ctx_op = _attend(q, k, v, SCALE, smask.unsqueeze(0).expand(2, items, l), self.dtype, self.split == 8, (2, items * lq))
         t = ops.gemm(ctx_op, ly["wo"], ly["bo"], residual=h32 if lq == l else h32.view(2, items, l, d)[:, :, 0, :], out_dtype=sdt)
         return _ln(t, ly["g1"], ly["b1"], eps, self.xdtype, sdt)
 
@@ -524,7 +532,7 @@
         for ly, lp, kv in zip(self.layers, plan.layers, kv_bank):
             lq = 1 if lp.cls_only else l
             if h32 is not None:
-                a32, a16 = self._self_block(ly, h32, h16, t_n, l, smask, lp.sdt, lq)
+                a32, a16 = self._self_block(ly, h32, h16, t_n, l, smask, lp.sdt, lq, plan.cls_split)
             ccl = self._cross_block(ly, lp, a16, cc, tok, emask2d, cand_rows, kv, plan.kv_chunk)
             h32, h16 = self._merge_ffn(ly, lp, ccl, a32, t_n * lq)
             if taps is not None:
diff --git a/candidate_reranking_cir_amd/lib.py b/candidate_reranking_cir_amd/lib.py
--- a/candidate_reranking_cir_amd/lib.py
+++ b/candidate_reranking_cir_amd/lib.py
@@ -8,7 +8,7 @@
 LIB_PATH = os.environ.get("CIR_LIB", os.path.join(_HERE, "libcirrank.so"))
 
 CIR_BF16, CIR_F16, CIR_F32 = 0, 1, 2
-TUNE_GEMM_TILE, TUNE_GEMM_GROUP_W, TUNE_ATTN_SHARED_MAX = 0, 1, 2
+TUNE_GEMM_TILE, TUNE_GEMM_GROUP_W, TUNE_ATTN_SHARED_MAX, TUNE_FOLD_KB = 0, 1, 2, 3
 ACT_NONE, ACT_GELU, ACT_RELU = 0, 1, 2
 
 class WgradDesc(ctypes.Structure):
@@ -42,6 +42,8 @@
     "cir_cls_cross_attention": (c_int, [c_void_p, c_int64, c_void_p, c_void_p, c_void_p, c_int, c_int, c_int, c_float, c_int, c_void_p]),
     "cir_cross_attention_folded": (c_int, [c_void_p, c_int64, c_int64, c_void_p, c_int64, c_void_p, c_void_p, c_int64, c_void_p, c_void_p, c_int64, c_void_p, c_int64, c_int64,
                                            c_int64, c_int, c_int, c_int, c_int, c_int, c_float, c_int, c_void_p]),
+    "cir_cross_attention_folded_indexed": (c_int, [c_void_p, c_int64, c_int64, c_void_p, c_int, c_void_p, c_int64, c_void_p, c_void_p, c_int64, c_void_p, c_void_p, c_int64,
+                                                   c_void_p, c_int64, c_int64, c_int64, c_int, c_int, c_int, c_int, c_int, c_float, c_int, c_void_p]),
     "cir_cross_attention_folded_long": (c_int, [c_void_p, c_int64, c_int64, c_void_p, c_int64, c_void_p, c_void_p, c_int64, c_void_p, c_void_p, c_int64, c_void_p, c_int64,
                                                 c_int64, c_int64, c_int, c_int, c_int, c_int, c_int, c_float, c_int, c_void_p]),
     "cir_cross_attention_folded_short": (c_int, [c_void_p, c_int64, c_int64, c_void_p, c_int64, c_void_p, c_void_p, c_int64, c_void_p, c_void_p, c_int64, c_void_p, c_int64,
diff --git a/candidate_reranking_cir_amd/ops.py b/candidate_reranking_cir_amd/ops.py
--- a/candidate_reranking_cir_amd/ops.py
+++ b/candidate_reranking_cir_amd/ops.py
@@ -412,17 +412,23 @@
 
 
 def _cross_attention_folded(entry: str, q: torch.Tensor, x: torch.Tensor, wkt: torch.Tensor, wvp: torch.Tensor, bv: torch.Tensor, out: torch.Tensor, l: int,
-                            scale: float, heads: int, mask: Optional[torch.Tensor]) -> torch.Tensor:
+                            scale: float, heads: int, mask: Optional[torch.Tensor], q_index: Optional[torch.Tensor] = None) -> torch.Tensor:
     _need_cuda(q, x, wkt, wvp, bv, out)
     t_n, n, d = x.shape
-    assert q.shape == (2, t_n * l, d) and q.stride(2) == 1 and x.stride(2) == 1 and x.stride(1) == d
+    q_args = ()
+    if q_index is not None:
+        _need_cuda(q_index)
+        q_index = q_index.to(torch.int64).contiguous()
+        assert q_index.shape == (t_n,) and q.shape[1] % l == 0
+        q_args = (q_index.data_ptr(), q.shape[1] // l)
+    assert q.shape == (2, q.shape[1] if q_index is not None else t_n * l, d) and q.stride(2) == 1 and x.stride(2) == 1 and x.stride(1) == d
     assert wkt.shape == (2, d, d) and wvp.shape == (2, d, d) and wkt.is_contiguous() and wvp.is_contiguous() and bv.shape == (2, d) and bv.is_contiguous()
     assert out.shape == (t_n, l, 2, d) and out.stride(3) == 1 and q.dtype == x.dtype == wkt.dtype == wvp.dtype == out.dtype and bv.dtype == torch.float32
     if mask is not None:
         _need_cuda(mask)
         assert mask.dtype == torch.float32 and mask.shape == (t_n, n) and mask.stride(1) == 1
     ev = _events() if PROFILE_ATTN is not None else None
-    code = getattr(_lib.load(), entry)(q.data_ptr(), q.stride(0), q.stride(1), x.data_ptr(), x.stride(0), wkt.data_ptr(), wvp.data_ptr(), d * d,
+    code = getattr(_lib.load(), entry)(q.data_ptr(), q.stride(0), q.stride(1), *q_args, x.data_ptr(), x.stride(0), wkt.data_ptr(), wvp.data_ptr(), d * d,
                                        bv.data_ptr(), _ptr(mask), mask.stride(0) if mask is not None else 0,
                                        out.data_ptr(), out.stride(0), out.stride(1), out.stride(2), t_n, l, n, d, heads,
                                        float(scale), _DT[x.dtype], _stream())
@@ -434,7 +440,9 @@
 
 
 def cross_attention_folded(q: torch.Tensor, x: torch.Tensor, wkt: torch.Tensor, wvp: torch.Tensor, bv: torch.Tensor, out: torch.Tensor, l: int,
-                           scale: float, heads: int = 12, mask: Optional[torch.Tensor] = None) -> torch.Tensor:
+                           scale: float, heads: int = 12, mask: Optional[torch.Tensor] = None, q_index: Optional[torch.Tensor] = None) -> torch.Tensor:
+    if q_index is not None:
+        return _cross_attention_folded("cir_cross_attention_folded_indexed", q, x, wkt, wvp, bv, out, l, scale, heads, mask, q_index)
     return _cross_attention_folded("cir_cross_attention_folded", q, x, wkt, wvp, bv, out, l, scale, heads, mask)
 
 
diff --git a/include/cirrank.h b/include/cirrank.h
--- a/include/cirrank.h
+++ b/include/cirrank.h
@@ -22,7 +22,7 @@
 int cir_version(void);
 const char* cir_strerror(int code);
 
-enum { CIR_TUNE_GEMM_TILE = 0, CIR_TUNE_GEMM_GROUP_W = 1, CIR_TUNE_ATTN_SHARED_MAX = 2 };
+enum { CIR_TUNE_GEMM_TILE = 0, CIR_TUNE_GEMM_GROUP_W = 1, CIR_TUNE_ATTN_SHARED_MAX = 2, CIR_TUNE_FOLD_KB = 3 };
 int cir_set_tuning(int knob, int value);
 
 int cir_gemm_bias_act(const void* A, int64_t lda, int64_t strideA,
@@ -72,6 +72,11 @@
 int cir_cross_attention_folded(const void* q, int64_t q_sb, int64_t q_rs, const void* x, int64_t x_s1, const void* wkt, const void* wvp, int64_t w_sb,
                                const float* bv, const float* key_mask, int64_t mask_stride, void* out, int64_t o_st, int64_t o_sr, int64_t o_sb,
                                int T, int L, int N, int D, int H, float scale, int dtype, void* stream);
+
+int cir_cross_attention_folded_indexed(const void* q, int64_t q_sb, int64_t q_rs, const int64_t* q_index, int Q, const void* x, int64_t x_s1,
+                                       const void* wkt, const void* wvp, int64_t w_sb, const float* bv, const float* key_mask, int64_t mask_stride,
+                                       void* out, int64_t o_st, int64_t o_sr, int64_t o_sb, int T, int L, int N, int D, int H, float scale,
+                                       int dtype, void* stream);
 
 int cir_cross_attention_folded_long(const void* q, int64_t q_sb, int64_t q_rs, const void* x, int64_t x_s1, const void* wkt, const void* wvp, int64_t w_sb,
                                     const float* bv, const float* key_mask, int64_t mask_stride, void* out, int64_t o_st, int64_t o_sr, int64_t o_sb,
```
